# LSquarzoni/SNN_Event-based_Optical_Flow

Measured on AMD Instinct MI355X. Metric: events/sec (train step) LIFFireNet T=10 128x128, higher is better.
Workload: dtype fp32; 1 GPU; LIFFireNet train step: T=10 x 1000-event windows, 128x128, batch 8/GPU, base_num_channels 8, EventWarping + Adam; global_batch=8, parallelism=dp1, hip_graph=True, launch_order=wavefront

## Files before the change

### include/snnflow.h

```cpp
#ifndef SNNFLOW_H
#define SNNFLOW_H

#include <stdint.h>

#ifdef __cplusplus
extern "C" {
#endif

#define SNNFLOW_ABI_VERSION 41

#define SNNFLOW_E_ARG (-1)
#define SNNFLOW_E_CHANNELS (-2)

#define SNNFLOW_TILE_H 8
#define SNNFLOW_TILE_W 32

typedef struct snnflow_neuron {
    const float* bn_weight;
    const float* bn_bias;
    float* running_mean;
    float* running_var;
    int64_t* num_batches_tracked;
    const float* beta;
    const float* threshold;
    double momentum, eps;
    int bn_train;
    int zero_reset;
} snnflow_neuron;

int snnflow_prep_weights(const float* w, int c, int cin, float* wt_fwd, float* wt_bwd,
                         float* threshold, void* stream);

typedef struct snnflow_prep_desc {
    const float* w; int c, cin; float* wt_fwd; float* wt_bwd;
    float* threshold; int thr_n;
    uint16_t* frag_fwd; uint16_t* frag_bwd;
    double* zero; int64_t zero_n;
} snnflow_prep_desc;
int snnflow_frag_halfs(int c, int cin);
#define SNNFLOW_MAX_BATCH 16
int snnflow_prep_weights_batch(const snnflow_prep_desc* d, int n, void* stream);

#define SNNFLOW_ACC_SHARDS 32
#define SNNFLOW_ACC_STRIDE(n) ((((n) + 15) / 16) * 16)
#define SNNFLOW_ACC_LEN(n) (SNNFLOW_ACC_SHARDS * SNNFLOW_ACC_STRIDE(n))

typedef struct snnflow_conv_fwd_args {
    int B, H, W, cin, c;
    int lif_in;
    const float* x; int64_t xs_b, xs_c, xs_h, xs_w;
    const float* prev_y; const float* prev_mem;
    const double* prev_acc; float* prev_stats;
    snnflow_neuron prev; float* prev_state;
    const float* wt_ff;
    const float* wt_rec;
    const float* wt_ff_t; const float* wt_rec_t;
    const float* s_prev;
    float* y;
    double* acc;
    double* zero0; double* zero1; int zero_n;
    const uint16_t* wf_ff; const uint16_t* wf_rec;
    int state_spk_skip;
    uint8_t* prev_spk_bits; const uint8_t* s_prev_bits;
} snnflow_conv_fwd_args;
int snnflow_conv_fwd(const snnflow_conv_fwd_args* a, void* stream);
int snnflow_conv_blocks(int B, int H, int W);

typedef struct snnflow_lif_fwd_args {
    int B, H, W, c;
    const float* y; const float* mem;
    const double* acc;
    float* stats;
    snnflow_neuron n; float* state;
    const float* pred_w;
    const float* pred_b;
    float* flow;
    double* zero0; double* zero1; int zero_n;
    int state_spk_skip;
} snnflow_lif_fwd_args;
int snnflow_lif_fwd(const snnflow_lif_fwd_args* a, void* stream);

typedef struct snnflow_neuron_grad {
    float* bn_weight; float* bn_bias; float* beta; float* threshold;
} snnflow_neuron_grad;

#define SNNFLOW_SPK_BIT(c, ch) (((ch) % 4) * ((c) / 4) + (ch) / 4)

#define SNNFLOW_BWD_ACC(c) (5 * (c) + 2)

typedef struct snnflow_lif_bwd_args {
    int B, H, W, c;
    const float* y; const float* mem; const float* stats; snnflow_neuron n;
    const float* g_out;
    const float* g_state;
    const float* pred_w; const float* flow; const float* g_flow;
    int64_t gflow_sb, gflow_sc;
    float* g_cur;
    float* g_mem;
    double* acc;
    double* zero0; double* zero1; int zero_n;
    int mem_grad_in;
} snnflow_lif_bwd_args;
int snnflow_lif_bwd(const snnflow_lif_bwd_args* a, void* stream);

typedef struct snnflow_layer_bwd_args {
    int B, H, W, cin, c;
    const float* y; const float* stats; const float* g_cur;
    const double* acc_in;
    snnflow_neuron n;
    snnflow_neuron_grad ng;
    int has_pred; float* g_pred_w; float* g_pred_b;
    int accumulate;
    float* bnc_out;
    const float* wt_bwd_ff;
    const float* wt_bwd_rec;
    const float* wt_fwd_ff; const float* wt_fwd_rec;
    int lif_in;
    float* g_x; int64_t gxs_b, gxs_c, gxs_h, gxs_w;
    float* g_state_prev;
    int zero_mem_half;
    const float* prev_y; const float* prev_mem; const float* prev_stats; snnflow_neuron prev;
    const float* prev_g_state;
    float* prev_g_cur; float* prev_g_mem;
    double* acc_out;
    double* zero0; double* zero1; int zero_n;
    const uint16_t* wd_ff; const uint16_t* wd_rec;
    float* wslab_ff; float* wslab_rec; const float* s_prev; int wslab_accumulate;
    const float* x; int64_t xs_b, xs_c, xs_h, xs_w;
} snnflow_layer_bwd_args;
int snnflow_layer_bwd(const snnflow_layer_bwd_args* a, void* stream);

#define SNNFLOW_MAX_SLOT_TASKS 4
int snnflow_fwd_slot(const snnflow_conv_fwd_args* conv, int nconv, const snnflow_lif_fwd_args* lif,
                     void* stream);
int snnflow_bwd_slot(const snnflow_layer_bwd_args* layer, int nlayer, const snnflow_lif_bwd_args* lif,
                     void* stream);
int snnflow_slot_supported(int c, int cin0);
int snnflow_set_pipe(int fwd_tiles_per_block, int bwd_tiles_per_block);
int snnflow_get_pipe(int which);

#define SNNFLOW_MAX_LAYERS 8

typedef struct snnflow_wgrad_step {
    const float* g_cur;
    const float* y;
    const float* x; int64_t xs_b, xs_c, xs_h, xs_w;
    const float* s_prev;
    const float* stats;
    const float* bnc;
    const uint8_t* x_bits; const uint8_t* s_prev_bits;
} snnflow_wgrad_step;
#define SNNFLOW_MAX_WGRAD_STEPS 32
typedef struct snnflow_wgrad_args {
    int B, H, W, cin, c, nsteps, accumulate, rec;
    int exact_inputs;
    const float* bn_weight;
    float* slab_ff;
    float* slab_rec;
    snnflow_wgrad_step steps[SNNFLOW_MAX_WGRAD_STEPS];
} snnflow_wgrad_args;
int snnflow_wgrad(const snnflow_wgrad_args* a, void* stream);

typedef struct snnflow_convlif_params {
    const float* leak;
    const float* thresh;
    float act_width;
    int hard_reset;
} snnflow_convlif_params;

typedef struct snnflow_convlif_fwd_args {
    int B, H, W, cin, c;
    const float* x; int64_t xs_b, xs_c, xs_h, xs_w;
    const float* prev_state;
    const float* wt_ff;
    const float* wt_rec;
    snnflow_convlif_params p;
    const float* residual; int64_t rs_b, rs_c, rs_h, rs_w;
    float* out;
    float* state;
    float* current;
} snnflow_convlif_fwd_args;
int snnflow_convlif_fwd(const snnflow_convlif_fwd_args* a, void* stream);

typedef struct snnflow_convlif_bwd_args {
    int B, H, W, cin, c;
    const float* g_out; int64_t gs_b, gs_c, gs_h, gs_w;
    const float* g_state;
    const float* state;
    const float* prev_state;
    const float* current;
    const float* wt_bwd_ff;
    const float* wt_bwd_rec;
    snnflow_convlif_params p;
    float* g_x; int64_t gxs_b, gxs_c, gxs_h, gxs_w;
    float* g_prev;
    float* g_current;
    double* acc;
} snnflow_convlif_bwd_args;
int snnflow_convlif_bwd(const snnflow_convlif_bwd_args* a, void* stream);

int snnflow_convlif_param_grads(const double* acc, const float* leak, const float* thresh, int c, int accumulate,
                                float* g_leak, float* g_thresh, void* stream);

typedef struct snnflow_encode_args {
    int B, N, H, W;
    const float* ts; const float* ys; const float* xs; const float* ps;
    int64_t ev_stride, batch_stride;
    int num_bins, round_ts, accumulate;
    float* cnt; float* voxel; float* image; float* mask; float* pol_mask;
} snnflow_encode_args;
int snnflow_encode_events(const snnflow_encode_args* a, void* stream);

#define SNNFLOW_AUG_H 1
#define SNNFLOW_AUG_V 2
#define SNNFLOW_AUG_P 4
typedef struct snnflow_loader_args {
    int B, N;
    int H0, W0;
    int Ht, Wt;
    int num_bins, round_ts;
    int keep_gt_full_res;
    int hot_enabled, hot_max_px, hot_min_obvs;
    float hot_max_rate;
    float scale_y, scale_x;
    const float* xs; const float* ys; const float* ts; const float* ps;
    const int* counts;
    const int* flags;
    const float* gtflow_in;
    float* hot_events;
    int* hot_idx;
    float* event_cnt;
    float* event_voxel;
    float* event_mask;
    float* event_list;
    float* pol_mask;
    float* gtflow;
    float* scratch;
} snnflow_loader_args;
int snnflow_loader_prepare(const snnflow_loader_args* a, void* stream);
int64_t snnflow_loader_scratch_floats(int B, int N, int H0, int W0, int Ht, int Wt, int num_bins, int hot_enabled,
                                      int keep_gt_full_res);

typedef struct snnflow_slab_desc { const float* slab; float* out; int elems; } snnflow_slab_desc;
#define SNNFLOW_MAX_SLABS 16
int snnflow_slab_reduce(const snnflow_slab_desc* d, int n, int nblk, void* stream);

#define SNNFLOW_MAX_WINDOWS 64
typedef struct snnflow_iwe_loss_args {
    int B, M, T, H, W;
    int tf;
    const float* events[SNNFLOW_MAX_WINDOWS]; const float* pol[SNNFLOW_MAX_WINDOWS];
    const float* flows[SNNFLOW_MAX_WINDOWS]; const float* masks[SNNFLOW_MAX_WINDOWS];
    int32_t off[SNNFLOW_MAX_WINDOWS + 1];
    float flow_scaling, weight;
    int smoothing_mask, overwrite_intermediate, loss_scaling;
    float* images;
    double* acc;
    float* persample;
    float* smooth;
    float* loss;
} snnflow_iwe_loss_args;
int snnflow_iwe_loss_fwd(const snnflow_iwe_loss_args* a, void* stream);
int snnflow_iwe_loss_bwd(const snnflow_iwe_loss_args* a, const float* g_loss, float* g_flows, void* stream);
int snnflow_iwe_acc_doubles(int B, int H, int W, int tf);
int snnflow_device_errors(int clear);
int64_t snnflow_iwe_scratch_floats(int B, int M, int T, int tf, int H, int W);

int snnflow_iwe_corners(const float* events, const float* flow_ev, int B, int M, float tref,
                        int H, int W, float flow_scaling, int round_idx, int32_t* idx, float* w,
                        void* stream);
int snnflow_iwe_interpolate(const int32_t* idx, const float* w, const float* pol, int64_t pol_sb,
                            int B, int K, int H, int W, float* img, void* stream);
int snnflow_iwe_corners_bwd(const float* events, const float* flow_ev, int B, int M, float tref,
                            int H, int W, float flow_scaling, const float* g_w, float* g_flow_ev,
                            void* stream);
int snnflow_iwe_interpolate_bwd(const int32_t* idx, const float* pol, int64_t pol_sb, int B, int K,
                                int H, int W, const float* g_img, float* g_w, void* stream);

int snnflow_pol_iwe(const float* events, const float* flow, const float* pol, int64_t pol_stride, int nimg, int B,
                    int N, int H, int W, float tref, float flow_scaling, int round_idx, float* out, void* stream);

typedef struct snnflow_aee_args {
    int B, H, W;
    const float* flow;
    const float* gtflow;
    const float* event_mask;
    const float* dt_ratio;
    float flow_scaling;
    double* acc;
    float* aee; float* percent;
// ... 378 lines not shown
```

### snn_event-based_optical_flow_amd/csrc/lif_layers.hip

```cpp
#include <cmath>
#include <string>
#include <type_traits>

#include "snnflow_dev.h"
#include "snnflow_tile.h"

#ifndef SNNFLOW_PROBE
#define SNNFLOW_PROBE 0
#endif
#define PROBE_OFF(bit) ((SNNFLOW_PROBE & (bit)) != 0)

#ifndef SNNFLOW_SP32
#define SNNFLOW_SP32 2
#endif
#ifndef SNNFLOW_LATE_D_REC8
#define SNNFLOW_LATE_D_REC8 1
#endif
#ifndef SNNFLOW_LATE_D_FF8
#define SNNFLOW_LATE_D_FF8 1
#endif
#ifndef SNNFLOW_EARLY_G_REC8
#define SNNFLOW_EARLY_G_REC8 1
#endif
#ifndef SNNFLOW_L32_WAVES
// ... 1007 lines not shown
        float s = 0.0f;
        for (int k = qq; k < NT; k += Q) {
            const float4 v = lds[k];
            s += j == 0 ? v.x : (j == 1 ? v.y : (j == 2 ? v.z : v.w));
        }
        part[(int64_t)blockIdx.x * C + tid] = s;
    }
}

__global__ __launch_bounds__(64) void k_lif_theta_reduce(const float* __restrict__ part, int nblk, int c,
                                                      float* g_theta) {
    const int ch = threadIdx.x;
    if (ch >= c) return;
    double s = 0.0;
    for (int b = 0; b < nblk; ++b) s += (double)part[(int64_t)b * c + ch];
    g_theta[ch] -= (float)s;
}

struct BnBwdLds { float mean, inv, gm, k, w; };

__device__ inline float4 bn_bwd4(const float4& g, const float4& y, const BnBwdLds* bp) {
    const float gi[4] = {g.x, g.y, g.z, g.w}, yi[4] = {y.x, y.y, y.z, y.w};
    float o[4];
#pragma unroll
    for (int j = 0; j < 4; ++j) {
        const BnBwdLds c = bp[j];
        const float dx = (yi[j] - c.mean) * c.k;
        o[j] = (((gi[j] - c.gm) - dx) * c.inv) * c.w;
    }
    return make_float4(o[0], o[1], o[2], o[3]);
}

template <int CIN, int C, bool LIF_IN, bool REC, int SPLIT, bool BFG = false>
struct LayerBwdLds {
    static constexpr bool BF6 = kMfma<CIN, C> && (C == 8 || BFG);
    static constexpr bool WL = kWlds<CIN, C> && !BF6;
    static constexpr int FR = FragFloats<BF6 && C == 8, C, NT * SPLIT>::v;
    static constexpr int G = BF6 ? (3 * HN * C / 2 + 3) / 4 * 4 : HN * Pad<C>::v;
    static constexpr int WX = WL ? 9 * C * C : FR, WR = REC ? (WL ? 9 * C * C : FR) : 0;
    static constexpr int FLOATS = G + WX + WR;
    static_assert(!BF6 || G >= NT * Pad<CIN>::v, "output staging aliases the gradient tile");
};

typedef short s16x4w __attribute__((ext_vector_type(4)));
typedef __attribute__((address_space(3))) s16x4w lds_s16x4w;
__device__ inline bf16x8 tr8(const __bf16* r0, const __bf16* r1) {
    const s16x4w v0 = __builtin_amdgcn_ds_read_tr16_b64_v4i16((lds_s16x4w*)(r0));
    const s16x4w v1 = __builtin_amdgcn_ds_read_tr16_b64_v4i16((lds_s16x4w*)(r1));
    const short __attribute__((ext_vector_type(8))) v = __builtin_shufflevector(v0, v1, 0, 1, 2, 3, 4, 5, 6, 7);
    return __builtin_bit_cast(bf16x8, v);
}

constexpr int kWgfX = NT * 8 / 2, kWgfR = 8 * 8 * 9, kWgfP = 8 * 64;
constexpr int kWgfFloats = kWgfX + kWgfR + kWgfP;

template <bool REC>
__device__ void fused_wgrad_old(const snnflow_layer_bwd_args& a, const Grid& g, float (&wold)[4]) {
    const int tid = threadIdx.x;
    const bool acc_in = a.wslab_accumulate != 0;
    const bool has_s = REC && a.s_prev != nullptr && a.wslab_rec != nullptr;
    if (acc_in) {
        const float* sf = a.wslab_ff + (int64_t)g.bid * kWgfR;
        wold[0] = sf[tid];
        if (tid + 2 * NT < kWgfR) wold[1] = sf[tid + 2 * NT];
        if constexpr (REC) {
            if (has_s) {
                const float* sr = a.wslab_rec + (int64_t)g.bid * kWgfR;
                wold[2] = sr[tid];
                if (tid + 2 * NT < kWgfR) wold[3] = sr[tid + 2 * NT];
            }
        }
    }
}

template <bool REC>
__device__ void fused_wgrad_stage(const snnflow_layer_bwd_args& a, const float* G, float* wl_x, float* wl_r,
                                  const float (&xsp)[4], const float4& sp, int pt, int ci0) {
    constexpr int C = 8, PART = HN * C;
    const int tid = threadIdx.x;
    const bool has_s = REC && a.s_prev != nullptr && a.wslab_rec != nullptr;
    typedef __bf16 bf16x4 __attribute__((ext_vector_type(4)));
    __bf16* X = reinterpret_cast<__bf16*>(wl_x);
    __bf16* S = reinterpret_cast<__bf16*>(wl_r);
    const bf16x4 xs = {(__bf16)xsp[0], (__bf16)xsp[1], (__bf16)xsp[2], (__bf16)xsp[3]};
    __syncthreads();
    *reinterpret_cast<bf16x4*>(X + pt * C + ci0) = xs;
    if constexpr (REC) {
        if (has_s) *reinterpret_cast<bf16x4*>(S + pt * C + ci0) = bf16x4{(__bf16)sp.x, (__bf16)sp.y, (__bf16)sp.z, (__bf16)sp.w};
    }
    __syncthreads();

    const int lane = tid & 63, wv = __builtin_amdgcn_readfirstlane(tid >> 6);
    const int g4 = lane >> 4, qq = (lane & 15) >> 2, pp = lane & 3;
    const __bf16* G3 = reinterpret_cast<const __bf16*>(G);
    const int j0 = 8 * g4 + qq;
    f32x4 acc = {0.f, 0.f, 0.f, 0.f}, acc8 = acc, accr = acc, acc8r = acc;
    auto kstep = [&](int tap, int row, f32x4& d, f32x4& dr) {
        const int ky = tap / 3, kx = tap - 3 * ky;
        const int hp = (row + 2 - ky) * HWD + (j0 + 2 - kx);
        const __bf16* ga = G3 + hp * C + 4 * pp;
        const bf16x8 ah = tr8(ga, ga + 4 * C);
        const bf16x8 am = tr8(ga + PART, ga + PART + 4 * C);
        const bf16x8 al = tr8(ga + 2 * PART, ga + 2 * PART + 4 * C);
        const int q = row * TW + j0;
        const __bf16* xb = X + q * C + 4 * pp;
        const bf16x8 b = tr8(xb, xb + 4 * C);
        d = __builtin_amdgcn_mfma_f32_16x16x32_bf16(al, b, d, 0, 0, 0);
        d = __builtin_amdgcn_mfma_f32_16x16x32_bf16(am, b, d, 0, 0, 0);
        d = __builtin_amdgcn_mfma_f32_16x16x32_bf16(ah, b, d, 0, 0, 0);
        if constexpr (REC) {
            if (has_s) {
                const __bf16* sb = S + q * C + 4 * pp;
                const bf16x8 bs = tr8(sb, sb + 4 * C);
                dr = __builtin_amdgcn_mfma_f32_16x16x32_bf16(al, bs, dr, 0, 0, 0);
                dr = __builtin_amdgcn_mfma_f32_16x16x32_bf16(am, bs, dr, 0, 0, 0);
                dr = __builtin_amdgcn_mfma_f32_16x16x32_bf16(ah, bs, dr, 0, 0, 0);
            }
        }
    };
#pragma unroll 2
    for (int row = 0; row < TH; ++row) kstep(wv, row, acc, accr);
    kstep(8, wv, acc8, acc8r);
    const int ci = lane & 15;
    if (ci < C && g4 < 2) {
        float* R = wl_x + kWgfX;
        float* P8 = R + kWgfR;
#pragma unroll
        for (int j = 0; j < 4; ++j) {
            const int co = 4 * g4 + j;
            R[(co * C + ci) * 9 + wv] = acc[j];
            P8[wv * 64 + co * C + ci] = acc8[j];
        }
        if constexpr (REC) {
            if (has_s) {
                float* Rr = wl_r + kWgfX;
                float* P8r = Rr + kWgfR;
#pragma unroll
                for (int j = 0; j < 4; ++j) {
                    const int co = 4 * g4 + j;
                    Rr[(co * C + ci) * 9 + wv] = accr[j];
                    P8r[wv * 64 + co * C + ci] = acc8r[j];
                }
            }
        }
    }
}

__device__ inline int pk_slot(int q) { return SNNFLOW_SWZ ? q ^ (((q >> 3) & 1) << 2) : q; }
__device__ inline int pk_quad(int q, int quad) { return SNNFLOW_SWZ ? quad ^ ((q >> 3) & 1) : quad; }

constexpr int kPkRecOff = SNNFLOW_SWZ ? 16 : 0;

__device__ void fused_wgrad_stage_pk(const float* G, float* wl_x, float* wl_r, const float (&xsp)[4], const float4& sp,
                                     int pt, int ci0) {
    constexpr int C = 8, PART = HN * C, XS = 16;
    static_assert(FragFloats<true, 8, 2 * NT>::v >= NT * XS / 2 && FragFloats<true, 8, 2 * NT>::v >= 2 * (kWgfR + kWgfP) + kPkRecOff,
                  "packed x|s tile in wl_x, both result sets in wl_r");
    const int tid = threadIdx.x;
    typedef __bf16 bf16x4 __attribute__((ext_vector_type(4)));
    __bf16* X = reinterpret_cast<__bf16*>(wl_x);
    __syncthreads();
    const int ps = pk_slot(pt);
    *reinterpret_cast<bf16x4*>(X + ps * XS + ci0) = bf16x4{(__bf16)xsp[0], (__bf16)xsp[1], (__bf16)xsp[2], (__bf16)xsp[3]};
    *reinterpret_cast<bf16x4*>(X + ps * XS + C + ci0) = bf16x4{(__bf16)sp.x, (__bf16)sp.y, (__bf16)sp.z, (__bf16)sp.w};
    __syncthreads();

    const int lane = tid & 63, wv = __builtin_amdgcn_readfirstlane(tid >> 6);
    const int g4 = lane >> 4, qq = (lane & 15) >> 2, pp = lane & 3;
    const __bf16* G3 = reinterpret_cast<const __bf16*>(G);
    const int j0 = 8 * g4 + qq;
    f32x4 acc = {0.f, 0.f, 0.f, 0.f}, acc8 = acc;
    auto kstep = [&](int tap, int row, f32x4& d) {
        const int ky = tap / 3, kx = tap - 3 * ky;
        const int hp = (row + 2 - ky) * HWD + (j0 + 2 - kx);
        const __bf16* ga = G3 + hp * C + 4 * pp;
        const bf16x8 ah = tr8(ga, ga + 4 * C);
        const bf16x8 am = tr8(ga + PART, ga + PART + 4 * C);
        const bf16x8 al = tr8(ga + 2 * PART, ga + 2 * PART + 4 * C);
        const int q = row * TW + j0;
        const bf16x8 b = tr8(X + pk_slot(q) * XS + 4 * pp, X + pk_slot(q + 4) * XS + 4 * pp);
        d = __builtin_amdgcn_mfma_f32_16x16x32_bf16(al, b, d, 0, 0, 0);
        d = __builtin_amdgcn_mfma_f32_16x16x32_bf16(am, b, d, 0, 0, 0);
        d = __builtin_amdgcn_mfma_f32_16x16x32_bf16(ah, b, d, 0, 0, 0);
    };
#pragma unroll 2
    for (int row = 0; row < TH; ++row) kstep(wv, row, acc);
    kstep(8, wv, acc8);
    const int n = lane & 15;
    if (g4 < 2) {
        float* R = wl_r + (n < C ? 0 : kWgfR + kWgfP + kPkRecOff);
        float* P8 = R + kWgfR;
        const int ci = n & 7;
#pragma unroll
        for (int j = 0; j < 4; ++j) {
            const int co = 4 * g4 + j;
            R[(co * C + ci) * 9 + wv] = acc[j];
            P8[wv * 64 + co * C + ci] = acc8[j];
        }
    }
}

template <bool REC>
__device__ void fused_wgrad_store(const snnflow_layer_bwd_args& a, const Grid& g, const float* rx,
                                  const float* rr, const float (&wold)[4]) {
    const int tid = threadIdx.x;
    const bool acc_in = a.wslab_accumulate != 0;
    const bool has_s = REC && a.s_prev != nullptr && a.wslab_rec != nullptr;
    auto value = [&](const float* R, int e) {
        const int tap = e % 9;
        if (tap < 8) return R[e];
        const float* P8 = R + kWgfR;
        const int k = e / 9;
        float v = P8[k];
#pragma unroll
        for (int w = 1; w < 8; ++w) v += P8[w * 64 + k];
        return v;
    };
#pragma unroll
    for (int i = 0; i < 2; ++i) {
        const int e = tid + i * 2 * NT;
        if (e < kWgfR) {
            a.wslab_ff[(int64_t)g.bid * kWgfR + e] = acc_in ? wold[i] + value(rx, e) : value(rx, e);
            if constexpr (REC) {
                if (a.wslab_rec) {
                    if (has_s) a.wslab_rec[(int64_t)g.bid * kWgfR + e] = acc_in ? wold[2 + i] + value(rr, e) : value(rr, e);
                    else if (!acc_in) a.wslab_rec[(int64_t)g.bid * kWgfR + e] = 0.0f;
                }
            }
        }
    }
}

template <int CIN, int C, int NTH, int TOFF>
struct WAcc {
    static constexpr int VW = VecW<CIN>::v;
    static constexpr int Q = 9 * (C / 4) * (CIN / VW);
    static constexpr int GR0 = (Q >= NTH) ? 1 : NTH / Q;
    static constexpr int GR = GR0 > 16 ? 16 : GR0;
    static constexpr int NM = (GR > 1) ? 1 : (Q + NTH - 1) / NTH;
    static constexpr int SCRATCH = (GR > 1) ? GR * Q * 4 * VW : 1;
    float acc[NM][4][VW];
    __device__ void zero() {
#pragma unroll
        for (int m = 0; m < NM; ++m)
#pragma unroll
            for (int i = 0; i < 4; ++i)
#pragma unroll
                for (int j = 0; j < VW; ++j) acc[m][i][j] = 0.f;
    }
    template <bool HG = false>
    __device__ void step(const float* Gi, const float* X) {
        constexpr int PC = Pad<C>::v, PX = Pad<CIN>::v;
        const int tid = (int)threadIdx.x - TOFF;
        if (tid < 0 || tid >= NTH) return;
#pragma unroll
        for (int m = 0; m < NM; ++m) {
            const int q = (GR > 1) ? tid % Q : tid + m * NTH;
            const int g = (GR > 1) ? tid / Q : 0;
            if ((GR > 1) ? (g >= GR) : (q >= Q)) continue;
            const int kidx = q % 9, rest = q / 9, cob = rest % (C / 4), cib = rest / (C / 4);
            const int ky = kidx / 3, kx = kidx % 3;
#pragma unroll 4
            for (int p = g; p < NT; p += GR) {
                const int ty = p / TW, tx = p - ty * TW;
                const int gp = HG ? (ty + 1) * HWD + tx + 1 : p;
                const float4 gv4 = *reinterpret_cast<const float4*>(Gi + gp * PC + cob * 4);
                const float gv[4] = {gv4.x, gv4.y, gv4.z, gv4.w};
                const float* xp = X + ((ty + ky) * HWD + tx + kx) * PX + cib * VW;
                float xv[VW];
                if constexpr (VW == 4) {
                    const float4 v = *reinterpret_cast<const float4*>(xp);
                    xv[0] = v.x; xv[1] = v.y; xv[2] = v.z; xv[3] = v.w;
                } else if constexpr (VW == 2) {
                    const float2 v = *reinterpret_cast<const float2*>(xp);
                    xv[0] = v.x; xv[1] = v.y;
                } else {
                    xv[0] = xp[0];
                }
#pragma unroll
                for (int i = 0; i < 4; ++i)
#pragma unroll
                    for (int j = 0; j < VW; ++j) acc[m][i][j] = fmaf(gv[i], xv[j], acc[m][i][j]);
            }
        }
    }
    static __device__ int slab_index(int e) {
        const int qq = e / (4 * VW), ij = e - qq * 4 * VW, i = ij / VW, j = ij - i * VW;
        const int kk = qq % 9, rest = qq / 9, cb = rest % (C / 4), ib = rest / (C / 4);
        return ((cb * 4 + i) * CIN + ib * VW + j) * 9 + kk;
    }
    static constexpr int NOLD = (Q * 4 * VW + NTH - 1) / NTH;
    __device__ void flush_prefetched(float* __restrict__ slab, int accumulate, float* scratch, const float (&old)[NOLD]) {
        static_assert(GR > 1, "group-scratch form");
        const int tid = (int)threadIdx.x - TOFF;
        const bool mine = tid >= 0 && tid < NTH;
        const int q = tid % Q, g = tid / Q;
        if (mine && g < GR) {
#pragma unroll
            for (int i = 0; i < 4; ++i)
#pragma unroll
                for (int j = 0; j < VW; ++j) scratch[((g * Q + q) * 4 + i) * VW + j] = acc[0][i][j];
        }
        __syncthreads();
#pragma unroll
        for (int k = 0; k < NOLD; ++k) {
            const int e = tid + k * NTH;
            if (mine && e < Q * 4 * VW) {
                float sum = 0.f;
                for (int gg = 0; gg < GR; ++gg) sum += scratch[gg * Q * 4 * VW + e];
                slab[slab_index(e)] = accumulate ? old[k] + sum : sum;
            }
        }
    }
    __device__ void flush(float* __restrict__ slab, int accumulate, float* scratch) {
        const int tid = (int)threadIdx.x - TOFF;
        const bool mine = tid >= 0 && tid < NTH;
        if constexpr (GR > 1) {
            const int q = tid % Q, g = tid / Q;
            if (mine && g < GR) {
#pragma unroll
                for (int i = 0; i < 4; ++i)
#pragma unroll
                    for (int j = 0; j < VW; ++j) scratch[((g * Q + q) * 4 + i) * VW + j] = acc[0][i][j];
            }
            __syncthreads();
            for (int e = mine ? tid : Q * 4 * VW; e < Q * 4 * VW; e += NTH) {
                float sum = 0.f;
                for (int gg = 0; gg < GR; ++gg) sum += scratch[gg * Q * 4 * VW + e];
                const int qq = e / (4 * VW), ij = e - qq * 4 * VW, i = ij / VW, j = ij - i * VW;
                const int kk = qq % 9, rest = qq / 9, cb = rest % (C / 4), ib = rest / (C / 4);
                const int idx = ((cb * 4 + i) * CIN + ib * VW + j) * 9 + kk;
                slab[idx] = accumulate ? slab[idx] + sum : sum;
            }
            __syncthreads();
        } else {
#pragma unroll
            for (int m = 0; m < NM; ++m) {
                const int q = tid + m * NTH;
                if (!mine || q >= Q) continue;
                const int kk = q % 9, rest = q / 9, cb = rest % (C / 4), ib = rest / (C / 4);
#pragma unroll
                for (int i = 0; i < 4; ++i)
#pragma unroll
                    for (int j = 0; j < VW; ++j) {
                        const int idx = ((cb * 4 + i) * CIN + ib * VW + j) * 9 + kk;
                        slab[idx] = accumulate ? slab[idx] + acc[m][i][j] : acc[m][i][j];
                    }
            }
        }
    }
};

template <int CIN, int C, bool LIF_IN, bool REC, int SPLIT, bool BFG = false, bool WGF = false, bool HWG = false>
__device__ void layer_bwd_body(const snnflow_layer_bwd_args& a, const Grid g, float* lds) {
    using LB = LayerBwdLds<CIN, C, LIF_IN, REC, SPLIT, BFG>;
    static_assert(!HWG || (!LIF_IN && !REC && !kMfma<CIN, C>), "fused head weight gradient: feed-forward head tasks");
    static_assert(!WGF || (LIF_IN && C == 8 && CIN == 8 && SPLIT == 2 && LB::BF6 && LB::FR >= kWgfFloats),
                  "fused weight gradients: C = 8 LIF-fed layers with LDS weight fragments");
    constexpr int NTB = NT * SPLIT;
    constexpr int CI = CIN / SPLIT, CR = C / SPLIT;
    static_assert(CI * SPLIT == CIN && CR * SPLIT == C, "channel split");
    static_assert(!LIF_IN || CI % 4 == 0, "LIF backward group: multiple of 4 channels");
    constexpr int PC = Pad<C>::v;
    constexpr bool PF = Prefetch<C, NTB>::on;
    constexpr int NVP = LIF_IN ? 3 * CI : 1;
    constexpr int QI = CI / 4 > 0 ? CI / 4 : 1;
    float* G = lds;
    [[maybe_unused]] float* wl_x = lds + LB::G;
    [[maybe_unused]] float* wl_r = wl_x + LB::WX;
    __shared__ BnBwdLds bnp[C];
    __shared__ LifCoef pcoef[LIF_IN ? CIN : 1];
    __shared__ float pmean[LIF_IN ? CIN : 1];

    const int tid = threadIdx.x, pt = tid % NT, ty = pt / TW, tx = pt - ty * TW;
    const int part = thread_part(), ci0 = part * CI, cr0 = part * CR;
    const int H = a.H, W = a.W;
    const Tile tl = block_tile(H, W, g);
    const double N = (double)a.B * H * W;
    const float nf = (float)N;
    const int h = tl.h0 + ty, w = tl.w0 + tx;
    const bool in = (h < H) && (w < W);
    const int64_t pix = ((int64_t)tl.b * H + h) * W + w;
    const float4 z4 = make_float4(0.f, 0.f, 0.f, 0.f);
    [[maybe_unused]] constexpr bool TR = LIF_IN && CIN == C && SNNFLOW_TRACE_LAYER;
    [[maybe_unused]] constexpr int TK = REC ? 3 : 2;
    TRACE_AT(TR, TK, 0);

    constexpr bool EARLY_G = C <= 16 && !(REC && C == 8 && !SNNFLOW_EARLY_G_REC8);
    constexpr int NSUM = SNNFLOW_BWD_ACC(C), NBN = (C <= 16 || SNNFLOW_BWD_GATHER32) ? 2 * C : NSUM;
    const bool lead = g.bid == 0;
    constexpr int NL = NSUM - NBN > 0 ? NSUM - NBN : 1;
    AccGather<NBN> gat;
    AccGather<NL> gat_l;
    if constexpr (EARLY_G) {
        acc_gather_load<NBN>(a.acc_in, NSUM, gat);
        if (NBN < NSUM && lead) acc_gather_load<NL>(a.acc_in + NBN, NSUM, gat_l);
    }
    float st_mean = 0.f, st_inv = 0.f, gamma = 0.f;
    if (tid < C) {
        st_mean = a.stats[tid];
        st_inv = a.stats[C + tid];
        gamma = a.n.bn_weight[tid];
    }
    const NeuronGradRegs ngr =
        load_neuron_grad(a.n, a.stats, C, a.ng, a.accumulate, a.has_pred, a.g_pred_w, a.g_pred_b, g.bid == 0);
    float praw[6] = {0.f, 0.f, 0.f, 0.f, 0.f, 0.f};
    if constexpr (LIF_IN) {
        const int c = tid < CIN ? tid : 0;
        praw[0] = a.prev_stats[c];
        praw[1] = a.prev_stats[CIN + c];
        praw[2] = a.prev.bn_weight[c];
        praw[3] = a.prev.bn_bias[c];
        praw[4] = a.prev.beta[c];
        praw[5] = a.prev.threshold[c];
    }

    constexpr bool WL = LB::WL, BF6 = LB::BF6, FLDS = BF6 && C == 8;
    WStage<WL ? 9 * C * C : 1, NTB> sw_x, sw_r;
    FragStage<FLDS ? C : 8, FLDS ? CIN : 8, FLDS ? NTB : 64> fs_x, fs_r;
    static_assert(!BF6 || PF, "bf16 gradient tile: register-prefetched halo");
    if constexpr (WL) {
        if (a.wt_bwd_ff) sw_x.load(a.wt_fwd_ff);
        if constexpr (REC) {
            if (a.g_state_prev) sw_r.load(a.wt_fwd_rec);
        }
    }
    constexpr bool PKC = FLDS && REC && CIN == 8 && C == 8;
    [[maybe_unused]] const bool pkr = PKC && a.wt_bwd_ff != nullptr && a.g_state_prev != nullptr;
    if constexpr (FLDS) {
        if constexpr (PKC) {
            if (pkr) fs_x.load2(a.wt_fwd_ff, a.wt_fwd_rec);
            else if (a.wt_bwd_ff) fs_x.load(a.wt_fwd_ff);
            if (!pkr && a.g_state_prev) fs_r.load(a.wt_fwd_rec);
        } else {
            if (a.wt_bwd_ff) fs_x.load(a.wt_fwd_ff);
            if constexpr (REC) {
                if (a.g_state_prev) fs_r.load(a.wt_fwd_rec);
            }
        }
    }
    using HAF = WAcc<HWG ? CIN : 4, HWG ? C : 4, NTB, 0>;
    constexpr int HXR = HWG ? (HN * CIN + NTB - 1) / NTB : 1;
    [[maybe_unused]] const bool hwg = HWG && a.wslab_ff != nullptr && a.x != nullptr;
    [[maybe_unused]] float hx[HXR], hold[HAF::NOLD];
    if constexpr (HWG) {
        if (hwg) {
            const float* xb = a.x + (int64_t)tl.b * a.xs_b;
#pragma unroll
            for (int i = 0; i < HXR; ++i) {
                const int e = tid + i * NTB;
                const int ci = e / HN, p = e - ci * HN;
                const int r = p / HWD, cc = p - r * HWD;
                const int hh = tl.h0 + r - 1, ww = tl.w0 + cc - 1;
                hx[i] = (e < HN * CIN && in_image(hh, ww, H, W)) ? xb[ci * a.xs_c + hh * a.xs_h + ww * a.xs_w] : 0.0f;
            }
            const float* srow = a.wslab_ff + (int64_t)g.bid * (C * CIN * 9);
#pragma unroll
            for (int k = 0; k < HAF::NOLD; ++k) {
                const int e = tid + k * NTB;
                hold[k] = (a.wslab_accumulate && e < C * CIN * 9) ? srow[HAF::slab_index(e < C * CIN * 9 ? e : 0)] : 0.0f;
            }
        }
    }
    float4 rg[PF ? Halo4<C, NTB>::R : 1], ry[PF ? Halo4<C, NTB>::R : 1];
    float4 dy[LIF_IN ? QI : 1], dm[LIF_IN ? QI : 1], dg[LIF_IN ? QI : 1];
    if constexpr (PF) {
        halo_load<C, NTB>(a.g_cur, tl, H, W, rg);
        halo_load<C, NTB>(a.y, tl, H, W, ry);
    }
    constexpr bool LATE_D = C >= 32 || (C == 8 && (REC ? SNNFLOW_LATE_D_REC8 : SNNFLOW_LATE_D_FF8));
    [[maybe_unused]] float wold[4] = {0.f, 0.f, 0.f, 0.f};
    [[maybe_unused]] float4 wsp = z4;
    [[maybe_unused]] const bool wgf = WGF && a.wslab_ff != nullptr;
    auto load_prev = [&]() {
        if constexpr (LIF_IN) {
            constexpr int Q4 = CIN / 4;
            const int64_t plane4 = (int64_t)a.B * H * W * Q4;
            const float4* py4 = reinterpret_cast<const float4*>(a.prev_y);
            const float4* pm4 = reinterpret_cast<const float4*>(a.prev_mem);
            const float4* pg4 = reinterpret_cast<const float4*>(a.prev_g_state);
            const int64_t pc = ((int64_t)tl.b * H + (h < H ? h : H - 1)) * W + (w < W ? w : W - 1);
            const int64_t base = pc * Q4 + ci0 / 4;
#pragma unroll
            for (int q = 0; q < QI; ++q) {
                dy[q] = py4[base + q];
                dm[q] = ld4_or_zero(pm4, py4, base + q);
                dg[q] = ld4_or_zero(pg4 ? pg4 + plane4 : nullptr, py4, base + q);
            }
        }
        if constexpr (WGF && REC) {
            if (wgf && a.s_prev && a.wslab_rec && in) wsp = reinterpret_cast<const float4*>(a.s_prev)[pix * 2 + ci0 / 4];
        }
    };
    if constexpr (!LATE_D) load_prev();


    __shared__ double sums[NSUM];
    if constexpr (EARLY_G) {
        acc_gather_reduce<NBN>(gat, sums);
        if (NBN < NSUM && lead) acc_gather_reduce<NL>(gat_l, sums + NBN);
    } else if constexpr (SNNFLOW_BWD_GATHER32) {
        double* red = reinterpret_cast<double*>(lds);
        acc_gather_pool<NBN, NTB>(a.acc_in, NSUM, sums, red);
        if (NBN < NSUM && lead) acc_gather_pool<NL, NTB>(a.acc_in + NBN, NSUM, sums + NBN, red);
    } else {
        acc_gather<NBN>(a.acc_in, NSUM, sums);
        if (NBN < NSUM && lead) acc_gather<NL>(a.acc_in + NBN, NSUM, sums + NBN);
    }
    neuron_grads(ngr, sums, C, a.ng, a.has_pred, a.g_pred_w, a.g_pred_b, lead);
    if (tid < C) {
        const float mean = st_mean, inv = st_inv;
        BnBwdLds c;
        c.mean = mean;
        c.inv = inv;
        c.w = gamma;
        if (a.n.bn_train) {
            c.k = (float)sums[C + tid] * inv * inv / nf;
            c.gm = (float)(sums[tid] / N);
        } else {
            c.k = 0.0f;
            c.gm = 0.0f;
        }
        bnp[tid] = c;
        if (g.bid == 0 && a.bnc_out) {
            a.bnc_out[tid] = c.gm;
            a.bnc_out[C + tid] = c.k;
        }
    }
    if constexpr (LIF_IN) {
        if (tid < CIN) {
            LifCoef pk;
            pk.alpha = praw[1] * praw[2];
            pk.shift = praw[3] - praw[0] * pk.alpha;
            pk.beta = fminf(fmaxf(praw[4], 0.0f), 1.0f);
            pk.theta = praw[5];
            pcoef[tid] = pk;
            pmean[tid] = praw[0];
        }
    }
    __syncthreads();
    TRACE_AT(TR, TK, 1);
    zero_consumed(a.zero0, a.zero1, a.zero_n, g);

    if constexpr (PF) {
        constexpr int Q = C / 4;
        static_assert(NTB % Q == 0, "constant channel quad per thread");
        const int qt = tid % Q;
        const BnBwdLds kb[4] = {bnp[4 * qt], bnp[4 * qt + 1], bnp[4 * qt + 2], bnp[4 * qt + 3]};
#pragma unroll
        for (int i = 0; i < Halo4<C, NTB>::R; ++i) {
            const int e = tid + i * NTB;
            if (e < Halo4<C, NTB>::E) {
                const int p = e / Q;
                const int r = p / HWD, cc = p - r * HWD;
                const bool img = in_image(tl.h0 + r - 1, tl.w0 + cc - 1, H, W);
                const float4 gv = img ? bn_bwd4(rg[i], ry[i], kb) : z4;
                if constexpr (BF6) split3_store4(reinterpret_cast<__bf16*>(G) + p * C + 4 * qt, HN * C, gv);
                else *reinterpret_cast<float4*>(G + p * PC + 4 * qt) = gv;
            }
        }
    } else {
        constexpr int Q = C / 4;
        for (int e = tid; e < Halo4<C>::E; e += NTB) {
            const int p = e / Q, q = e - p * Q;
            const int64_t k = halo_idx4<C>(e, tl, H, W);
            float4 out = z4;
            if (k >= 0)
                out = bn_bwd4(reinterpret_cast<const float4*>(a.g_cur)[k], reinterpret_cast<const float4*>(a.y)[k],
                              bnp + 4 * q);
            *reinterpret_cast<float4*>(G + p * PC + 4 * q) = out;
        }
    }
    if constexpr (WL) {
        if (a.wt_bwd_ff) sw_x.store(wl_x);
        if constexpr (REC) {
            if (a.g_state_prev) sw_r.store(wl_r);
        }
    }
    if constexpr (FLDS) {
        if (a.wt_bwd_ff) fs_x.store(reinterpret_cast<__bf16*>(wl_x));
        if constexpr (REC) {
            if (a.g_state_prev && !pkr) fs_r.store(reinterpret_cast<__bf16*>(wl_r));
        }
    }
    __syncthreads();
    TRACE_AT(TR, TK, 2);

    float gx[CI];
#pragma unroll
    for (int ci = 0; ci < CI; ++ci) gx[ci] = 0.0f;
    if constexpr (kMfma<CIN, C>) {
        constexpr int NW = NTB / 64;
        const bool do_x = a.wt_bwd_ff != nullptr;
        const bool do_r = REC && a.g_state_prev != nullptr;
        constexpr int NG = (C >= 32 && BF6) ? 2 : 1;
        MfmaAcc<C, CIN, NW, NG> ax;
        MfmaAcc<C, C, NW, NG> arr;
        const __bf16* g3 = reinterpret_cast<const __bf16*>(G);
        if (do_x) {
            ax.zero();
            if constexpr (FLDS) {
                if (!PROBE_OFF(1)) mfma_dgrad_bf6<C, CIN, NW>(g3, reinterpret_cast<const __bf16*>(wl_x), ax);
            } else if constexpr (BF6) {
                if (!PROBE_OFF(1)) mfma_dgrad_bf6g<C, CIN, NW, NG>(g3, reinterpret_cast<const __bf16*>(a.wd_ff), ax);
            } else {
                if (!PROBE_OFF(1)) mfma_conv3x3<C, CIN, true, NW, NG>(G, WL ? wl_x : a.wt_fwd_ff, ax);
            }
        }
        if constexpr (REC) {
            if (do_r && !pkr) {
                arr.zero();
                if constexpr (FLDS) {
                    if (!PROBE_OFF(1)) mfma_dgrad_bf6<C, C, NW>(g3, reinterpret_cast<const __bf16*>(wl_r), arr);
                } else if constexpr (BF6) {
                    if (!PROBE_OFF(1)) mfma_dgrad_bf6g<C, C, NW, NG>(g3, reinterpret_cast<const __bf16*>(a.wd_rec), arr);
                } else {
                    if (!PROBE_OFF(1)) mfma_conv3x3<C, C, true, NW, NG>(G, WL ? wl_r : a.wt_fwd_rec, arr);
                }
            }
        }
        if constexpr (LATE_D) load_prev();
        __syncthreads();
        float* const dgo = (WGF && wgf) ? wl_x : G;
        if constexpr (PKC) {
            if (pkr) {
                const int lane = tid & 63, n = lane & 15, g4 = lane >> 4;
                const int wv = __builtin_amdgcn_readfirstlane(tid >> 6);
                float* out = (n < 8 ? wl_x : wl_r + kPkRecOff) + (n & 3);
#pragma unroll
                for (int mt = 0; mt < MfmaAcc<C, CIN, NW, NG>::MT; ++mt) {
                    const int T = MfmaAcc<C, CIN, NW, NG>::mt0(wv) + mt, row = T >> 1, c0 = (T & 1) * 16;
#pragma unroll
                    for (int r = 0; r < 4; ++r) {
                        const int q = row * TW + c0 + g4 * 4 + r;
                        out[q * 8 + 4 * pk_quad(q, (n >> 2) & 1)] = ax.v[mt][0][r];
                    }
                }
                __syncthreads();
                const float4 gv4 = *reinterpret_cast<const float4*>(wl_x + pt * 8 + 4 * pk_quad(pt, ci0 >> 2));
                gx[0] = gv4.x; gx[1] = gv4.y; gx[2] = gv4.z; gx[3] = gv4.w;
                if (in) {
                    const int64_t plane = (int64_t)a.B * H * W * C;
                    float* gsp = a.g_state_prev + pix * C + cr0;
                    if (a.zero_mem_half) *reinterpret_cast<float4*>(gsp) = z4;
                    *reinterpret_cast<float4*>(gsp + plane) =
                        *reinterpret_cast<const float4*>(wl_r + kPkRecOff + pt * 8 + 4 * pk_quad(pt, cr0 >> 2));
                }
            }
        }
        if (do_x && !pkr) {
            mfma_store<false>(ax, ax, dgo);
            __syncthreads();
            const float* gl = dgo + pt * Pad<CIN>::v + ci0;
#pragma unroll
            for (int ci = 0; ci < CI; ++ci) gx[ci] = gl[ci];
        }
        if constexpr (REC) {
            if (do_r && !pkr) {
                __syncthreads();
                mfma_store<false>(arr, arr, dgo);
                __syncthreads();
                if (in) {
                    const float* rl = dgo + pt * PC + cr0;
                    const int64_t plane = (int64_t)a.B * H * W * C;
                    float* gsp = a.g_state_prev + pix * C + cr0;
#pragma unroll
                    for (int c = 0; c < CR; c += 4) {
                        if (a.zero_mem_half) *reinterpret_cast<float4*>(gsp + c) = z4;
                        *reinterpret_cast<float4*>(gsp + plane + c) = *reinterpret_cast<const float4*>(rl + c);
                    }
                }
            }
        }
    } else {
        if (!PROBE_OFF(1) && a.wt_bwd_ff) dgrad_acc<C, CIN, CI>(G, a.wt_bwd_ff, ty, tx, ci0, gx);
        if constexpr (REC) {
            if (a.g_state_prev) {
                float gr[CR];
#pragma unroll
                for (int c = 0; c < CR; ++c) gr[c] = 0.0f;
                if (!PROBE_OFF(1)) dgrad_acc<C, C, CR>(G, a.wt_bwd_rec, ty, tx, cr0, gr);
                pin(gr);
                if (in) {
                    const int64_t plane = (int64_t)a.B * H * W * C;
                    float* gsp = a.g_state_prev + pix * C + cr0;
#pragma unroll
                    for (int c = 0; c < CR; c += 4) {
                        if (a.zero_mem_half) *reinterpret_cast<float4*>(gsp + c) = z4;
                        *reinterpret_cast<float4*>(gsp + plane + c) = make_float4(gr[c], gr[c + 1], gr[c + 2], gr[c + 3]);
                    }
                }
            }
        }
    }

    TRACE_AT(TR, TK, 3);
    if constexpr (LIF_IN) {
        float vd[NVP];
#pragma unroll
        for (int j = 0; j < NVP; ++j) vd[j] = 0.0f;
        [[maybe_unused]] float xsp[4] = {0.f, 0.f, 0.f, 0.f};
        if constexpr (WGF) {
            if (wgf) fused_wgrad_old<REC>(a, g, wold);
        }
        if (in && !PROBE_OFF(8)) {
            const bool zr = a.prev.zero_reset != 0;
            float4* gc4 = reinterpret_cast<float4*>(a.prev_g_cur) + pix * (CIN / 4) + ci0 / 4;
            float4* gm4 = a.prev_g_mem ? reinterpret_cast<float4*>(a.prev_g_mem) + pix * (CIN / 4) + ci0 / 4 : nullptr;
#pragma unroll
            for (int q = 0; q < QI; ++q) {
                const float yi[4] = {dy[q].x, dy[q].y, dy[q].z, dy[q].w};
                const float mi[4] = {dm[q].x, dm[q].y, dm[q].z, dm[q].w};
                const float gi[4] = {dg[q].x, dg[q].y, dg[q].z, dg[q].w};
                float go[4], gmo[4];
#pragma unroll
                for (int j = 0; j < 4; ++j) {
                    const int cl = 4 * q + j, ci = ci0 + cl;
                    const float gs = gx[cl] + gi[j];
                    const LifOut o = lif_step(yi[j], mi[j], pcoef[ci], zr);
                    const float gv = atan_sg(o.v - pcoef[ci].theta) * gs;
                    if constexpr (WGF) xsp[cl & 3] = o.s;
                    go[j] = gv;
                    gmo[j] = mem_grad(gv, mi[j], pcoef[ci], zr);
                    vd[cl] = gv;
                    vd[CI + cl] = (yi[j] - pmean[ci]) * gv;
                    vd[2 * CI + cl] = gv * o.mprime;
                }
                gc4[q] = make_float4(go[0], go[1], go[2], go[3]);
                if (gm4) gm4[q] = make_float4(gmo[0], gmo[1], gmo[2], gmo[3]);
            }
        }
        TRACE_AT(TR, TK, 4);
        double* acc = acc_shard(a.acc_out, SNNFLOW_BWD_ACC(CIN), g.bid);
        if (!PROBE_OFF(4))
            block_atomic_sum_parts<NVP, SPLIT>(vd, [acc](int pp, int j) {
                const int k = j / CI, jj = j - k * CI;
                return acc + k * CIN + pp * CI + jj;
            });
        TRACE_AT(TR, TK, 5);
        if constexpr (WGF) {
            if (wgf) {
                if (REC && a.s_prev != nullptr && a.wslab_rec != nullptr) {
                    fused_wgrad_stage_pk(G, wl_x, wl_r, xsp, wsp, pt, ci0);
                    __syncthreads();
                    fused_wgrad_store<REC>(a, g, wl_r, wl_r + kWgfR + kWgfP + kPkRecOff, wold);
                } else {
                    fused_wgrad_stage<REC>(a, G, wl_x, wl_r, xsp, wsp, pt, ci0);
                    __syncthreads();
                    fused_wgrad_store<REC>(a, g, wl_x + kWgfX, wl_r + kWgfX, wold);
                }
            }
        }
        TRACE_AT(TR, TK, 6);
    } else {
        if (a.g_x && a.wt_bwd_ff && in) {
            float* gb = a.g_x + (int64_t)tl.b * a.gxs_b + h * a.gxs_h + w * a.gxs_w;
#pragma unroll
            for (int ci = 0; ci < CI; ++ci) gb[(ci0 + ci) * a.gxs_c] = gx[ci];
        }
        if constexpr (HWG) {
            if (hwg) {
                float* X = lds + LB::G;
#pragma unroll
                for (int i = 0; i < HXR; ++i) {
                    const int e = tid + i * NTB;
                    if (e < HN * CIN) {
                        const int ci = e / HN, p = e - ci * HN;
                        X[p * Pad<CIN>::v + ci] = hx[i];
                    }
                }
                HAF af;
                af.zero();
                __syncthreads();
                af.template step<true>(G, X);
                __syncthreads();
                af.flush_prefetched(a.wslab_ff + (int64_t)g.bid * (C * CIN * 9), a.wslab_accumulate, lds, hold);
            }
        }
    }
}

template <int CIN, int C, bool LIF_IN, bool REC, int SPLIT, bool BFG = false>
__global__ __launch_bounds__(NT * SPLIT, (C == 32 && LIF_IN && SPLIT == 2) ? SNNFLOW_L32_WAVES : 1)
void k_layer_bwd(snnflow_layer_bwd_args a) {
    __shared__ __attribute__((aligned(16))) float pool[LayerBwdLds<CIN, C, LIF_IN, REC, SPLIT, BFG>::FLOATS];
    layer_bwd_body<CIN, C, LIF_IN, REC, SPLIT, BFG>(a, hw_grid(), pool);
}

typedef const __attribute__((address_space(4))) snnflow_wgrad_args* cwgrad_ptr;

template <int CIN, int C, bool REC, int NW>
struct WgradMfma {
    static constexpr int MTc = (C + 15) / 16, NTF = (CIN + 15) / 16, NTR = (C + 15) / 16;
    static constexpr int NFF = 9 * MTc * NTF, NREC = REC ? 9 * MTc * NTR : 0, NTOT = NFF + NREC;
    static constexpr int J = (NTOT + NW - 1) / NW;
    static_assert(C % 8 == 0 && CIN % 8 == 0, "MFMA wgrad: 8-channel multiples (C = 8 pads the 16-wide tiles)");
    f32x4 acc[J];
    int off[J], mt[J], nt[J], tap[J];
    bool rec[J], live[J];
    __device__ void init() {
        const int wv = __builtin_amdgcn_readfirstlane((int)threadIdx.x >> 6);
#pragma unroll
        for (int j = 0; j < J; ++j) {
            acc[j] = f32x4{0.f, 0.f, 0.f, 0.f};
            const int i = wv + NW * j;
            live[j] = i < NTOT;
            rec[j] = i >= NFF;
            const int ii = rec[j] ? i - NFF : i, ntx = rec[j] ? NTR : NTF;
            tap[j] = live[j] ? ii / (MTc * ntx) : 0;
            const int rem = ii - tap[j] * (MTc * ntx);
            mt[j] = live[j] ? rem / ntx : 0;
            nt[j] = live[j] ? rem - mt[j] * ntx : 0;
            off[j] = (tap[j] / 3) * HWD + (tap[j] % 3);
        }
    }
    __device__ void step(const float* Gi, const float* X, const float* S, bool has_s) {
        constexpr int PC = Pad<C>::v, PX = Pad<CIN>::v;
        const int lane = threadIdx.x & 63, m = lane & 15, g = lane >> 4;
#pragma unroll 8
        for (int s = 0; s < NT / 4; ++s) {
            const int p = 4 * s + g, ty = p / TW, tx = p - ty * TW;
            const int hb = ty * HWD + tx;
            float a[MTc];
#pragma unroll
            for (int q = 0; q < MTc; ++q) a[q] = (q * 16 + m < C) ? Gi[p * PC + q * 16 + m] : 0.0f;
#pragma unroll
            for (int j = 0; j < J; ++j) {
                if (!live[j] || (rec[j] && !has_s)) continue;
                float av = a[0];
#pragma unroll
                for (int q = 1; q < MTc; ++q)
                    if (mt[j] == q) av = a[q];
                const int n = nt[j] * 16 + m;
                float b = 0.0f;
                if (rec[j]) {
                    if (n < C) b = S[(hb + off[j]) * PC + n];
                } else if (n < CIN) {
                    b = X[(hb + off[j]) * PX + n];
                }
                acc[j] = __builtin_amdgcn_mfma_f32_16x16x4f32(av, b, acc[j], 0, 0, 0);
            }
        }
    }
    __device__ void flush(float* __restrict__ slab_ff, float* __restrict__ slab_rec, int accumulate) {
        const int lane = threadIdx.x & 63, m = lane & 15, g = lane >> 4;
#pragma unroll
        for (int j = 0; j < J; ++j) {
            if (!live[j] || (rec[j] && !slab_rec)) continue;
            const int ci = nt[j] * 16 + m, cin = rec[j] ? C : CIN;
            if (ci >= cin) continue;
            float* base = rec[j] ? slab_rec : slab_ff;
#pragma unroll
            for (int r = 0; r < 4; ++r) {
                const int co = mt[j] * 16 + g * 4 + r;
                if (co >= C) continue;
                float* d = base + ((int64_t)co * cin + ci) * 9 + tap[j];
                *d = accumulate ? *d + acc[j][r] : acc[j][r];
            }
        }
    }
};

template <int CH, int NTH>
struct Own4 {
    static constexpr int Q = CH / 4, E = NT * Q, R = (E + NTH - 1) / NTH;
};

template <int CIN, int C, bool REC, int SPLIT>
__global__ __launch_bounds__(NT * SPLIT) void k_wgrad(snnflow_wgrad_args) {
    constexpr int NTB = NT * SPLIT;
    constexpr int PC = Pad<C>::v, PI_ = Pad<CIN>::v;
    constexpr bool XV = CIN % 4 == 0;
    constexpr bool HALVES = REC && SPLIT == 2;
    using AF = WAcc<CIN, C, HALVES ? NT : NTB, 0>;
    using AR = WAcc<C, C, HALVES ? NT : NTB, HALVES ? NT : 0>;
    constexpr bool MF = C >= 16 && CIN % 16 == 0;
    using O = Own4<C, NTB>;
    constexpr int RX = XV ? Halo4<CIN, NTB>::R : 1, RS = REC ? Halo4<C, NTB>::R : 1;
    constexpr int SCR = MF ? 4 : ((REC && AR::SCRATCH > AF::SCRATCH) ? AR::SCRATCH : AF::SCRATCH);
    __shared__ __attribute__((aligned(16))) float Gi[NT * PC];
    __shared__ __attribute__((aligned(16))) float X[HN * PI_];
    __shared__ __attribute__((aligned(16))) float S[REC ? HN * PC : 4];
    __shared__ __attribute__((aligned(16))) float scratch[SCR];
    __shared__ BnBwdLds coef[SNNFLOW_MAX_WGRAD_STEPS][C];

    const cwgrad_ptr ap = (cwgrad_ptr)__builtin_amdgcn_kernarg_segment_ptr();
    const int tid = threadIdx.x;
    const int H = ap->H, W = ap->W, nsteps = ap->nsteps;
    const Tile tl = block_tile(H, W);
    const float4 z4 = make_float4(0.f, 0.f, 0.f, 0.f);

    for (int e = tid; e < nsteps * C; e += NTB) {
        const int t = e / C, c = e - t * C;
        const float* st = ap->steps[t].stats;
        const float* bc = ap->steps[t].bnc;
        BnBwdLds k = {0.f, 1.f, 0.f, 0.f, 1.f};
        if (st) {
            k.mean = st[c];
// ... 862 lines not shown
    const float c = coef_s;
    for (int64_t j = threadIdx.x; j < n; j += 8 * CLIP_NT) {
        float v[8];
#pragma unroll
        for (int k = 0; k < 8; ++k) v[k] = j + k * CLIP_NT < n ? g[j + k * CLIP_NT] : 0.0f;
#pragma unroll
        for (int k = 0; k < 8; ++k)
            if (j + k * CLIP_NT < n) g[j + k * CLIP_NT] = v[k] * c;
    }
}

constexpr int CLIP_PER = 8, CLIP_SLICE = CLIP_PER * CLIP_NT;
static_assert(CLIP_SLICE == SNNFLOW_CLIP_ADAM_ONE_BLOCK, "one-block size");

__device__ inline double clip_sq_slice(const float* g, int64_t n, int64_t i0, int64_t i1) {
    double s = 0.0;
    for (int64_t i = i0 + threadIdx.x; i < i1; i += (int64_t)CLIP_SLICE) {
        float v[CLIP_PER];
#pragma unroll
        for (int k = 0; k < CLIP_PER; ++k) v[k] = i + k * CLIP_NT < i1 ? g[i + k * CLIP_NT] : 0.0f;
#pragma unroll
        for (int k = 0; k < CLIP_PER; ++k) s += (double)v[k] * (double)v[k];
    }
    return s;
}

__device__ inline double clip_block_sum(double s, double* part) {
#pragma unroll
    for (int off = 32; off > 0; off >>= 1) s += __shfl_xor(s, off, 64);
    if ((threadIdx.x & 63) == 0) part[threadIdx.x >> 6] = s;
    __syncthreads();
    double t = 0.0;
    if (threadIdx.x == 0)
        for (int w = 0; w < CLIP_NT / 64; ++w) t += part[w];
    return t;
}

__global__ __launch_bounds__(CLIP_NT) void k_clip_adam_norm(snnflow_clip_adam_args a) {
    __shared__ double part[CLIP_NT / 64];
    const int64_t i0 = (int64_t)blockIdx.x * CLIP_SLICE, i1 = i0 + CLIP_SLICE < a.n ? i0 + CLIP_SLICE : a.n;
    const double t = clip_block_sum(a.max_norm > 0.0f ? clip_sq_slice(a.grad, a.n, i0, i1) : 0.0, part);
    if (threadIdx.x == 0) {
        a.scratch[blockIdx.x] = t;
        if (blockIdx.x == 0) a.step[0] = a.step[0] + 1.0f;
    }
}

__global__ __launch_bounds__(CLIP_NT) void k_clip_adam(snnflow_clip_adam_args a, int nparts) {
    __shared__ double part[CLIP_NT / 64];
    __shared__ float coef_s;
    __shared__ snnflow_adam_tensor tab[SNNFLOW_ADAM_MAX_TENSORS];
    if (threadIdx.x < a.ntensors) tab[threadIdx.x] = a.t[threadIdx.x];
    const bool clip = a.max_norm > 0.0f;
    const float st_in = a.step[0];
    __syncthreads();
    const int64_t lo_i = nparts ? (int64_t)blockIdx.x * CLIP_SLICE : 0;
    const int64_t hi_i = lo_i + CLIP_SLICE < a.n ? lo_i + CLIP_SLICE : a.n;
    float gv[CLIP_PER], pv[CLIP_PER], mv[CLIP_PER], vv[CLIP_PER];
    float *pp[CLIP_PER], *mp[CLIP_PER], *vp[CLIP_PER];
#pragma unroll
    for (int u = 0; u < CLIP_PER; ++u) {
        const int64_t i = lo_i + threadIdx.x + (int64_t)u * CLIP_NT;
        gv[u] = i < hi_i ? a.grad[i] : 0.0f;
    }
#pragma unroll
    for (int u = 0; u < CLIP_PER; ++u) {
        const int64_t i = lo_i + threadIdx.x + (int64_t)u * CLIP_NT;
        pp[u] = nullptr;
        if (i >= hi_i) continue;
        int lo = 0, hi = a.ntensors - 1;
        while (lo < hi) {
            const int mid = (lo + hi + 1) >> 1;
            if (tab[mid].offset <= i) lo = mid;
            else hi = mid - 1;
        }
        const int64_t j = i - tab[lo].offset;
        if (j < 0 || j >= tab[lo].numel) continue;
        pp[u] = tab[lo].param + j;
        mp[u] = a.exp_avg + tab[lo].state_offset + j;
        vp[u] = a.exp_avg_sq + tab[lo].state_offset + j;
        pv[u] = *pp[u];
        mv[u] = *mp[u];
        vv[u] = *vp[u];
    }
    double tot = 0.0;
    if (nparts == 0) {
        double sq = 0.0;
        if (clip) {
#pragma unroll
            for (int u = 0; u < CLIP_PER; ++u) sq += (double)gv[u] * (double)gv[u];
        }
        tot = clip_block_sum(sq, part);
    } else if (threadIdx.x == 0 && clip) {
        for (int j = 0; j < nparts; ++j) tot += a.scratch[j];
    }
    const float st = nparts == 0 ? st_in + 1.0f : st_in;
    if (threadIdx.x == 0) {
        if (clip) {
            const float total = (float)sqrt(tot);
            const float cc = a.max_norm / (total + a.clip_eps);
            coef_s = cc < 1.0f ? cc : 1.0f;
            if (a.total_out && blockIdx.x == 0) a.total_out[0] = total;
        } else {
            coef_s = 1.0f;
        }
        if (nparts == 0) a.step[0] = st;
    }
    const double step = (double)st;
    const double bc1 = 1.0 - pow(a.beta1, step), bc2 = 1.0 - pow(a.beta2, step);
    __syncthreads();
    const float c = coef_s;
    const float neg_step_size = (float)(-(a.lr / bc1));
    const float bc2_sqrt = (float)sqrt(bc2);
    const float w1 = (float)(1.0 - a.beta1), b2 = (float)a.beta2, w2 = (float)(1.0 - a.beta2);
    const float eps = (float)a.eps, wd = (float)a.weight_decay;
#pragma unroll
    for (int u = 0; u < CLIP_PER; ++u) {
        if (!pp[u]) continue;
        float g = gv[u];
        if (clip) {
            g = g * c;
            a.grad[lo_i + threadIdx.x + (int64_t)u * CLIP_NT] = g;
        }
        float p = pv[u];
        if (wd != 0.0f) g = g + wd * p;
        const float m = mv[u] + w1 * (g - mv[u]);
        const float v = vv[u] * b2 + w2 * g * g;
        const float denom = sqrtf(v) / bc2_sqrt + eps;
        p = p + neg_step_size * (m / denom);
        *mp[u] = m;
        *vp[u] = v;
        *pp[u] = p;
    }
}

__global__ void k_lif_export(const float* __restrict__ x, const float* __restrict__ mem, const float* __restrict__ beta,
                             const float* __restrict__ thr, int64_t total, int C, int HW, float* spk, float* mout) {
    for (int64_t i = (int64_t)blockIdx.x * blockDim.x + threadIdx.x; i < total; i += (int64_t)gridDim.x * blockDim.x) {
        const int c = (int)((i / HW) % C);
        const float m = beta[c] * mem[i] + x[i];
        const bool s = m >= thr[c];
        spk[i] = s ? 1.0f : 0.0f;
        mout[i] = s ? 0.0f : m;
    }
}

constexpr int kSlotTasks = SNNFLOW_MAX_SLOT_TASKS;

enum SlotKind : int {
    SK_HEAD1, SK_HEAD2, SK_HEAD4, SK_HEAD5,
    SK_PLAIN, SK_PLAIN_REC,
    SK_LIF, SK_LIF_REC,
    SK_TOP, SK_TOP_PRED,
    SK_LIF_P, SK_LIF_REC_P
};

struct FwdSlotParams {
    snnflow_conv_fwd_args conv[kSlotTasks];
    snnflow_lif_fwd_args lif;
    int kind[kSlotTasks], blk0[kSlotTasks], nblk[kSlotTasks];
    int ntask;
};
struct BwdSlotParams {
    snnflow_layer_bwd_args layer[kSlotTasks];
    snnflow_lif_bwd_args lif;
    int kind[kSlotTasks], blk0[kSlotTasks], nblk[kSlotTasks];
    int ntask;
};

constexpr int cmax(int a, int b) { return a > b ? a : b; }

template <int C>
constexpr bool kSlotAllKinds = C == 8;

constexpr int kFragC8 = 3 * 3 * 256;
constexpr int kPipeRaw = 2 * HN * 16, kPipeSpk = HN * 8 * 2, kPipeFrag = kFragC8 * 2;
template <bool REC>
struct PipeFwdLds {
    static constexpr int RAWY = 0, RAWM = kPipeRaw, SPK = 2 * kPipeRaw, RSPK = SPK + kPipeSpk;
    static constexpr int FF = RSPK + (REC ? kPipeSpk : 0), FR = FF + kPipeFrag;
    static constexpr int BYTES = FR + (REC ? kPipeFrag : 0);
    static constexpr int FLOATS = BYTES / 4;
};

template <int C>
struct SlotLds {
    static constexpr int FWD_ALL = cmax(cmax(ConvFwdLds<1, C, false, false, 2>::FLOATS, ConvFwdLds<5, C, false, false, 2>::FLOATS),
                                        cmax(ConvFwdLds<C, C, false, false, 2>::FLOATS, ConvFwdLds<C, C, false, true, 2>::FLOATS));
    static constexpr int FWD_P = C == 8 ? PipeFwdLds<true>::FLOATS : 0;
    static constexpr int FWD = cmax(cmax(cmax(kSlotAllKinds<C> ? FWD_ALL : 0, kLifQFwdLds<C>), FWD_P),
                                    cmax(cmax(ConvFwdLds<2, C, false, false, 2>::FLOATS, ConvFwdLds<4, C, false, false, 2>::FLOATS),
                                         cmax(ConvFwdLds<C, C, true, false, 2>::FLOATS, ConvFwdLds<C, C, true, true, 2>::FLOATS)));
    static constexpr bool BFG = C >= 16;
    static constexpr int BWD_ALL = cmax(LayerBwdLds<C, C, false, false, 2>::FLOATS, LayerBwdLds<C, C, false, true, 2>::FLOATS);
    static constexpr int BWD = cmax(cmax(cmax(kSlotAllKinds<C> ? BWD_ALL : 0, kLifQBwdLds<C, true>),
                                         cmax(LayerBwdLds<2, C, false, false, 2>::FLOATS, LayerBwdLds<4, C, false, false, 2>::FLOATS)),
                                    cmax(LayerBwdLds<C, C, true, false, 2, BFG>::FLOATS,
                                         LayerBwdLds<C, C, true, true, 2, BFG>::FLOATS));
};

template <typename T>
__device__ inline T kernarg_copy(const __attribute__((address_space(4))) T* p) {
    static_assert(sizeof(T) % 4 == 0, "dword-sized struct");
    T r;
    const __attribute__((address_space(4))) int* src = (const __attribute__((address_space(4))) int*)p;
    int* dst = reinterpret_cast<int*>(&r);
#pragma unroll
    for (int i = 0; i < (int)(sizeof(T) / 4); ++i) dst[i] = src[i];
    return r;
}

template <typename T>
__device__ inline T* as_global_ptr(T* p) {
    __attribute__((address_space(1))) T* g;
    asm("" : "=s"(g) : "0"(p));
    return (T*)g;
}
#define SNN_G(x) (x) = as_global_ptr(x)

__device__ inline void globalize(snnflow_neuron& n) {
    SNN_G(n.bn_weight); SNN_G(n.bn_bias); SNN_G(n.running_mean); SNN_G(n.running_var);
    SNN_G(n.num_batches_tracked); SNN_G(n.beta); SNN_G(n.threshold);
}
__device__ inline void globalize(snnflow_neuron_grad& n) {
    SNN_G(n.bn_weight); SNN_G(n.bn_bias); SNN_G(n.beta); SNN_G(n.threshold);
}
__device__ inline void globalize(snnflow_conv_fwd_args& a) {
    SNN_G(a.x); SNN_G(a.prev_y); SNN_G(a.prev_mem); SNN_G(a.prev_acc); SNN_G(a.prev_stats);
    globalize(a.prev);
    SNN_G(a.prev_state); SNN_G(a.wt_ff); SNN_G(a.wt_rec); SNN_G(a.wt_ff_t); SNN_G(a.wt_rec_t); SNN_G(a.s_prev);
    SNN_G(a.prev_spk_bits); SNN_G(a.s_prev_bits);
    SNN_G(a.y); SNN_G(a.acc); SNN_G(a.zero0); SNN_G(a.zero1); SNN_G(a.wf_ff); SNN_G(a.wf_rec);
}
__device__ inline void globalize(snnflow_lif_fwd_args& a) {
    SNN_G(a.y); SNN_G(a.mem); SNN_G(a.acc); SNN_G(a.stats);
    globalize(a.n);
    SNN_G(a.state); SNN_G(a.pred_w); SNN_G(a.pred_b); SNN_G(a.flow); SNN_G(a.zero0); SNN_G(a.zero1);
}
__device__ inline void globalize(snnflow_lif_bwd_args& a) {
    SNN_G(a.y); SNN_G(a.mem); SNN_G(a.stats);
    globalize(a.n);
    SNN_G(a.g_out); SNN_G(a.g_state); SNN_G(a.pred_w); SNN_G(a.flow); SNN_G(a.g_flow); SNN_G(a.g_cur);
    SNN_G(a.g_mem); SNN_G(a.acc); SNN_G(a.zero0); SNN_G(a.zero1);
}
__device__ inline void globalize(snnflow_layer_bwd_args& a) {
    SNN_G(a.y); SNN_G(a.stats); SNN_G(a.g_cur); SNN_G(a.acc_in);
    globalize(a.n);
    globalize(a.ng);
    SNN_G(a.g_pred_w); SNN_G(a.g_pred_b); SNN_G(a.bnc_out); SNN_G(a.wt_bwd_ff); SNN_G(a.wt_bwd_rec);
    SNN_G(a.wt_fwd_ff); SNN_G(a.wt_fwd_rec); SNN_G(a.g_x); SNN_G(a.g_state_prev); SNN_G(a.prev_y);
    SNN_G(a.prev_mem); SNN_G(a.prev_stats);
    globalize(a.prev);
    SNN_G(a.prev_g_state); SNN_G(a.prev_g_cur); SNN_G(a.prev_g_mem); SNN_G(a.acc_out); SNN_G(a.zero0);
    SNN_G(a.zero1); SNN_G(a.wd_ff); SNN_G(a.wd_rec); SNN_G(a.wslab_ff); SNN_G(a.wslab_rec); SNN_G(a.s_prev);
    SNN_G(a.x);
}
__device__ inline void globalize(snnflow_eval_fwd_args& a) {
    SNN_G(a.x); SNN_G(a.s_in); SNN_G(a.mem_prev); SNN_G(a.s_prev); SNN_G(a.wt_ff); SNN_G(a.wt_rec);
    SNN_G(a.wt_ff_t); SNN_G(a.wt_rec_t);
    globalize(a.n);
    SNN_G(a.state); SNN_G(a.pred_w); SNN_G(a.pred_b); SNN_G(a.flow);
}
#undef SNN_G

template <typename T>
__device__ inline T task_args(const __attribute__((address_space(4))) T* p) {
    T r = kernarg_copy(p);
    globalize(r);
    return r;
}

template <typename P>
__device__ inline int slot_task(const __attribute__((address_space(4))) P* pp, Grid& g) {
    const int bid = blockIdx.x, nt = pp->ntask;
    int k = 0;
#pragma unroll
    for (int i = 1; i < kSlotTasks; ++i)
        if (i < nt && bid >= pp->blk0[i]) k = i;
    g.bid = bid - pp->blk0[k];
    g.nb = pp->nblk[k];
    return k;
}

typedef __attribute__((address_space(3))) void lds_void;

template <int N>
__device__ inline void vm_wait() {
    static_assert(N >= 0 && N < 64, "vmcnt");
    __builtin_amdgcn_s_waitcnt((N & 15) | ((N >> 4) << 14) | (7 << 4) | (15 << 8));
}

__device__ inline int opaque_int(int v) {
    asm volatile("" : "+v"(v));
    return v;
}

struct FragC8 {
    float r[2];
    __device__ inline void load(const float* __restrict__ wB) {
#pragma unroll
        for (int i = 0; i < 2; ++i) {
            const int e = (int)threadIdx.x + i * 2 * NT;
            const int j = e & 7, co = (e >> 3) & 7, g = (e >> 6) & 3, ch = e >> 8, tap = 4 * ch + g;
            r[i] = (e < 768 && tap < 9) ? wB[(tap * 8 + co) * 8 + j] : 0.0f;
        }
    }
    __device__ inline void store(__bf16* f) const {
#pragma unroll
        for (int i = 0; i < 2; ++i) {
            const int e = (int)threadIdx.x + i * 2 * NT;
            if (e < 768) {
                const float w = r[i];
                const __bf16 h = (__bf16)w;
                const float r1 = w - (float)h;
                const __bf16 md = (__bf16)r1;
                __bf16* d = f + (e >> 8) * 3 * 256 + (e & 255);
                d[0] = h;
                d[256] = md;
                d[512] = (__bf16)(r1 - (float)md);
            }
        }
    }
};

__host__ __device__ inline int pipe_tiles(const Grid& g, int ntiles) {
    return g.bid < ntiles ? (ntiles - 1 - g.bid) / g.nb + 1 : 0;
}

__device__ inline int* pipe_slot() {
    __shared__ int slot[4];
    return slot;
}

template <bool REC>
__device__ void fwd_lif8_pipe(const snnflow_conv_fwd_args& a, const Grid g, float* pool) {
    constexpr int C = 8, NTB = 2 * NT, R = Halo4<C, NTB>::R;
    using L = PipeFwdLds<REC>;
    char* const lds = reinterpret_cast<char*>(pool);
    __shared__ LifCoef coef[C];
    __shared__ double sums[2 * C];
    const int tid = threadIdx.x, lane = tid & 63;
    const int wv = __builtin_amdgcn_readfirstlane(tid >> 6);
    const int H = a.H, W = a.W, ntiles = a.B * tiles_per_image(H, W);
    int* const slot = pipe_slot();
    int v_cur = g.bid < ntiles ? g.bid : -1;
    if (v_cur < 0) return;
    const bool lead = g.bid == 0;
    const bool has_mem = a.prev_mem != nullptr;
    const bool has_rec = REC && a.s_prev != nullptr;
    TRACE_AT(true, REC ? 1 : 0, 0);

    AccGather<2 * C> gat;
    if (a.prev.bn_train) acc_gather_load<2 * C>(a.prev_acc, 2 * C, gat);
    const NeuronRegs nr = load_neuron(a.prev, C, lead);
    FragC8 fz_ff, fz_rec;
    fz_ff.load(a.wt_ff_t);
    if (has_rec) fz_rec.load(a.wt_rec_t);

    const uint32_t nbytes = (uint32_t)a.B * H * W * C * 4;
    const __amdgpu_buffer_rsrc_t rs_y = __builtin_amdgcn_make_buffer_rsrc(const_cast<float*>(a.prev_y), (short)0, (int)nbytes, 0x00020000);
    const __amdgpu_buffer_rsrc_t rs_m =
        __builtin_amdgcn_make_buffer_rsrc(const_cast<float*>(has_mem ? a.prev_mem : a.prev_y), (short)0, (int)nbytes, 0x00020000);
    auto issue = [&](const Tile& t, int lane) {
        const int base = ((t.b * H + t.h0 - 1) * W + (t.w0 - 1)) * (C * 4);
#pragma unroll
        for (int j = 0; j < 3; ++j) {
            const int k = wv + 8 * j;
            if (k >= 22) break;
            const bool mem = k >= 11;
            if (mem && !has_mem) continue;
            const int kk = mem ? k - 11 : k, ee = kk * 64 + lane, p = ee >> 1, r = p / HWD, cc = p - r * HWD;
            const bool ok = in_image(t.h0 + r - 1, t.w0 + cc - 1, H, W);
            const uint32_t off = ok ? (uint32_t)(base + (r * W + cc) * (C * 4) + (ee & 1) * 16) : 0x80000000u;
            if (ee < 2 * HN)
                __builtin_amdgcn_raw_ptr_buffer_load_lds(mem ? rs_m : rs_y, (lds_void*)(lds + (mem ? L::RAWM : L::RAWY) + kk * 1024),
                                                         16, off, 0, 0, 0);
        }
    };
    float4 rs[R];
    auto load_sprev = [&](const Tile& t, int tid) {
        const float4* base = reinterpret_cast<const float4*>(a.s_prev) + (((int64_t)t.b * H + (t.h0 - 1)) * W + (t.w0 - 1)) * 2;
#pragma unroll
        for (int i = 0; i < R; ++i) {
            const int e = tid + i * NTB, p = e >> 1, r = p / HWD, cc = p - r * HWD;
            const bool ok = e < 2 * HN && in_image(t.h0 + r - 1, t.w0 + cc - 1, H, W);
            rs[i] = ok ? base[(r * W + cc) * 2 + (e & 1)] : make_float4(0.f, 0.f, 0.f, 0.f);
        }
    };
    Tile tl = block_tile(H, W, Grid{v_cur, ntiles});
    issue(tl, lane);
    if (has_rec) load_sprev(tl, tid);
    if (a.prev.bn_train) acc_gather_reduce<2 * C>(gat, sums);
    TRACE_AT(true, REC ? 1 : 0, 1);
    lif_prologue(a.prev, nr, sums, C, (double)a.B * H * W, a.prev_stats, coef, nullptr, lead);
    TRACE_AT(true, REC ? 1 : 0, 2);
    fz_ff.store(reinterpret_cast<__bf16*>(lds + L::FF));
    if (has_rec) fz_rec.store(reinterpret_cast<__bf16*>(lds + L::FR));
    zero_consumed(a.zero0, a.zero1, a.zero_n, g);
    if (tid == 0) slot[2] = 0;

    const bool zr = a.prev.zero_reset != 0, spk_skip = a.state_spk_skip != 0;
    const int64_t plane4 = (int64_t)a.B * H * W * 2;
    float4* st4 = reinterpret_cast<float4*>(a.prev_state);
    float bs[4] = {0.f, 0.f, 0.f, 0.f}, bq[4] = {0.f, 0.f, 0.f, 0.f};
    const __bf16* spk = reinterpret_cast<const __bf16*>(lds + L::SPK);
    const __bf16* rspk = reinterpret_cast<const __bf16*>(lds + L::RSPK);
    TRACE_AT(true, REC ? 1 : 0, 3);

    for ([[maybe_unused]] int k = 0; v_cur >= 0; ++k) {
        vm_wait<0>();
        __syncthreads();
        TRACE_AT(k < 2, REC ? 1 : 0, 4 + 3 * k);
        const int tid = opaque_int(threadIdx.x), lane = tid & 63, jj = lane & 15, gg = lane >> 4, qt = tid & 1;
        const LifCoef kc[4] = {coef[4 * qt], coef[4 * qt + 1], coef[4 * qt + 2], coef[4 * qt + 3]};
        bool ok = true;
#pragma unroll
        for (int i = 0; i < R; ++i) {
            const int e = tid + i * NTB;
            if (e < 2 * HN) {
                const int p = e >> 1, r = p / HWD, cc = p - r * HWD;
                const int h = tl.h0 + r - 1, w = tl.w0 + cc - 1;
                const float4 yv = *reinterpret_cast<const float4*>(lds + L::RAWY + e * 16);
                const float4 mv = has_mem ? *reinterpret_cast<const float4*>(lds + L::RAWM + e * 16) : make_float4(0.f, 0.f, 0.f, 0.f);
                float4 sv = make_float4(0.f, 0.f, 0.f, 0.f);
                if (in_image(h, w, H, W)) {
                    const Lif4 o = zr ? lif_step4(yv, mv, kc, true) : lif_step4(yv, mv, kc, false);
                    sv = o.s;
                    if (r >= 1 && r <= TH && cc >= 1 && cc <= TW) {
                        const int64_t q = (((int64_t)tl.b * H + h) * W + w) * 2 + qt;
                        st_state4(st4, q, o.mout);
// ... 283 lines not shown
    const int64_t HWp = (int64_t)H * W;

    for (int k = 0; v_cur >= 0; ++k) {
        vm_wait<0>();
        __syncthreads();
        const int tid = opaque_int(threadIdx.x), lane = tid & 63, jj = lane & 15, gg = lane >> 4, qt = tid & 1;
        bool ok = true;
#pragma unroll
        for (int i = 0; i < R; ++i) {
            const int e = tid + i * NTB;
            if (e < 2 * HN) {
                const int p = e >> 1;
                const float4 sv = *reinterpret_cast<const float4*>(lds + L::RAW + e * 16);
                typedef __bf16 bf16x4 __attribute__((ext_vector_type(4)));
                *reinterpret_cast<bf16x4*>(const_cast<__bf16*>(spk) + p * 8 + 4 * qt) =
                    bf16x4{(__bf16)sv.x, (__bf16)sv.y, (__bf16)sv.z, (__bf16)sv.w};
                if (has_rec) {
                    const float4 s = rs[i];
                    ok = ok && exact_bf16(s.x) && exact_bf16(s.y) && exact_bf16(s.z) && exact_bf16(s.w);
                    *reinterpret_cast<bf16x4*>(const_cast<__bf16*>(rspk) + p * 8 + 4 * qt) =
                        bf16x4{(__bf16)s.x, (__bf16)s.y, (__bf16)s.z, (__bf16)s.w};
                }
            }
        }
        if (has_rec && __builtin_amdgcn_ballot_w64(!ok) != 0 && lane == 0) bad[k & 1] = 1;
        if (threadIdx.x == 0) bad[(k + 1) & 1] = 0;
        __syncthreads();
        const bool rec_bf = has_rec && bad[k & 1] == 0;
        const int v_nxt = v_cur + g.nb < ntiles ? v_cur + g.nb : -1;
        const Tile cur = tl;
        if (v_nxt >= 0) {
            tl = block_tile(H, W, Grid{v_nxt, ntiles});
            issue(tl, lane);
            if (has_rec) load_sprev(tl, tid);
        }
        const int qd = (lane >> 4) & 1, h = cur.h0 + wv, w = cur.w0 + (lane >> 5) * 16 + jj;
        const bool in = h < H && w < W;
        const int64_t pix = ((int64_t)cur.b * H + (in ? h : 0)) * W + (in ? w : 0);
        const float4 mv = (has_mem && in) ? mem4[pix * 2 + qd] : make_float4(0.f, 0.f, 0.f, 0.f);

        const bf16x8* fff = reinterpret_cast<const bf16x8*>(lds + L::FF) + gg * 8 + (jj & 7);
        const bf16x8* ffr = reinterpret_cast<const bf16x8*>(lds + L::FR) + gg * 8 + (jj & 7);
        f32x4 af[2] = {{0.f, 0.f, 0.f, 0.f}, {0.f, 0.f, 0.f, 0.f}}, ar[2] = {{0.f, 0.f, 0.f, 0.f}, {0.f, 0.f, 0.f, 0.f}};
#pragma unroll
        for (int ch = 0; ch < 3; ++ch) {
            const int tap = 4 * ch + gg, ky = tap / 3, kx = tap - 3 * ky;
            const bf16x8 fh = fff[ch * 96], fm = fff[ch * 96 + 32], fl = fff[ch * 96 + 64];
#pragma unroll
            for (int mt = 0; mt < 2; ++mt) {
                const int off = ((wv + ky) * HWD + mt * 16 + jj + kx) * 8;
                bf16x8 b = {};
                if (tap < 9) b = *reinterpret_cast<const bf16x8*>(spk + off);
                af[mt] = __builtin_amdgcn_mfma_f32_16x16x32_bf16(fl, b, af[mt], 0, 0, 0);
                af[mt] = __builtin_amdgcn_mfma_f32_16x16x32_bf16(fm, b, af[mt], 0, 0, 0);
                af[mt] = __builtin_amdgcn_mfma_f32_16x16x32_bf16(fh, b, af[mt], 0, 0, 0);
            }
            if (rec_bf) {
                const bf16x8 rh = ffr[ch * 96], rm = ffr[ch * 96 + 32], rl = ffr[ch * 96 + 64];
#pragma unroll
                for (int mt = 0; mt < 2; ++mt) {
                    const int off = ((wv + ky) * HWD + mt * 16 + jj + kx) * 8;
                    bf16x8 b = {};
                    if (tap < 9) b = *reinterpret_cast<const bf16x8*>(rspk + off);
                    ar[mt] = __builtin_amdgcn_mfma_f32_16x16x32_bf16(rl, b, ar[mt], 0, 0, 0);
                    ar[mt] = __builtin_amdgcn_mfma_f32_16x16x32_bf16(rm, b, ar[mt], 0, 0, 0);
                    ar[mt] = __builtin_amdgcn_mfma_f32_16x16x32_bf16(rh, b, ar[mt], 0, 0, 0);
                }
            }
        }
        f32x4 yv;
#pragma unroll
        for (int r = 0; r < 4; ++r) {
            const float y0 = rec_bf ? af[0][r] + ar[0][r] : af[0][r];
            const float y1 = rec_bf ? af[1][r] + ar[1][r] : af[1][r];
            const auto sw = __builtin_amdgcn_permlane32_swap(__builtin_bit_cast(unsigned, y0), __builtin_bit_cast(unsigned, y1),
                                                             false, false);
            yv[r] = __builtin_bit_cast(float, sw[0]);
        }
        if (has_rec && !rec_bf && in) {
            const float* wr = a.wt_rec;
#pragma unroll 1
            for (int tp = 0; tp < 9; ++tp) {
                const int hh = h + tp / 3 - 1, ww = w + tp % 3 - 1;
                if (!in_image(hh, ww, H, W)) continue;
                const float* sp = a.s_prev + (((int64_t)cur.b * H + hh) * W + ww) * C;
                for (int ci = 0; ci < C; ++ci) {
                    const float s = sp[ci];
#pragma unroll
                    for (int r = 0; r < 4; ++r) yv[r] = fmaf(wr[(tp * C + ci) * C + 4 * qd + r], s, yv[r]);
                }
            }
        }
        const LifCoef kc[4] = {coef[4 * qd], coef[4 * qd + 1], coef[4 * qd + 2], coef[4 * qd + 3]};
        const Lif4 o = zr ? lif_step4(make_float4(yv[0], yv[1], yv[2], yv[3]), mv, kc, true)
                          : lif_step4(make_float4(yv[0], yv[1], yv[2], yv[3]), mv, kc, false);
        if (in) {
            st_state4(st4, pix * 2 + qd, o.mout);
            st_state4(st4, plane4 + pix * 2 + qd, o.s);
        }
        if (pred) {
            const float p0 = __shfl_xor(o.s.x, 16, 64), p1 = __shfl_xor(o.s.y, 16, 64);
            const float p2 = __shfl_xor(o.s.z, 16, 64), p3 = __shfl_xor(o.s.w, 16, 64);
            const float s8[8] = {qd ? p0 : o.s.x, qd ? p1 : o.s.y, qd ? p2 : o.s.z, qd ? p3 : o.s.w,
                                 qd ? o.s.x : p0, qd ? o.s.y : p1, qd ? o.s.z : p2, qd ? o.s.w : p3};
            if (in) {
                const float* pw = a.pred_w + qd * C;
                float acc = 0.0f;
#pragma unroll
                for (int c = 0; c < C; ++c) acc = fmaf(pw[c], s8[c], acc);
                a.flow[((int64_t)cur.b * 2 + qd) * HWp + (int64_t)h * W + w] = tanhf(acc + a.pred_b[qd]);
            }
        }
        v_cur = v_nxt;
    }
}

__global__ __launch_bounds__(NT * 2, 6) void k_eval_slot(EvalSlotParams) {
    typedef const __attribute__((address_space(4))) EvalSlotParams* cptr;
    const cptr pp = (cptr)__builtin_amdgcn_kernarg_segment_ptr();
    const int bid = blockIdx.x, nt = pp->ntask;
    int k = 0;
#pragma unroll
    for (int i = 1; i < kEvalTasks; ++i)
        if (i < nt && bid >= pp->blk0[i]) k = i;
    Grid g;
    g.bid = bid - pp->blk0[k];
    g.nb = pp->nblk[k];
    if (g.bid >= g.nb) return;
    __shared__ __attribute__((aligned(16))) float pool[kEvalLdsFloats];
    const snnflow_eval_fwd_args a = task_args(&pp->t[k]);
    switch (pp->kind[k]) {
        case EK_HEAD2: eval_head_body<2>(a, g, pool); break;
        case EK_HEAD4: eval_head_body<4>(a, g, pool); break;
        case EK_FF: eval8_pipe<false>(a, g, pool); break;
        case EK_REC: eval8_pipe<true>(a, g, pool); break;
        default: break;
    }
}

#ifndef SNNFLOW_BWD_SLOT_WAVES
#define SNNFLOW_BWD_SLOT_WAVES 6
#endif
template <int C>
__global__ __launch_bounds__(NT * 2, C == 8 ? SNNFLOW_BWD_SLOT_WAVES : SNNFLOW_L32_WAVES) void k_bwd_slot(BwdSlotParams) {
    static_assert(C != 8 || SlotLds<C>::BWD >= LayerBwdLds<C, C, true, true, 2>::FLOATS, "fused wgrad staging");
    static_assert(C != 8 || 2 * LayerBwdLds<C, C, true, true, 2>::FR >= NT * Pad<C>::v, "dgrad staging size");
    static_assert(SlotLds<C>::BWD >= LayerBwdLds<2, C, false, false, 2>::G + HN * Pad<2>::v &&
                      SlotLds<C>::BWD >= LayerBwdLds<4, C, false, false, 2>::G + HN * Pad<4>::v &&
                      SlotLds<C>::BWD >= WAcc<2, C, 2 * NT, 0>::SCRATCH && SlotLds<C>::BWD >= WAcc<4, C, 2 * NT, 0>::SCRATCH,
                  "fused head weight gradient staging");
    typedef const __attribute__((address_space(4))) BwdSlotParams* cptr;
    const cptr pp = (cptr)__builtin_amdgcn_kernarg_segment_ptr();
    Grid g;
    const int k = slot_task(pp, g);
    if (g.bid >= g.nb) return;
    __shared__ __attribute__((aligned(16))) float pool[SlotLds<C>::BWD];
    switch (pp->kind[k]) {
#define BWD_LAYER(ALL, KIND, ...)                             \
    case KIND: {                                              \
        if constexpr (ALL || kSlotAllKinds<C>) {              \
            const snnflow_layer_bwd_args a = task_args(&pp->layer[k]);       \
            layer_bwd_body<__VA_ARGS__>(a, g, pool);          \
        }                                                     \
        break;                                                \
    }
        BWD_LAYER(true, SK_HEAD2, 2, C, false, false, 2, false, false, true)
        BWD_LAYER(true, SK_HEAD4, 4, C, false, false, 2, false, false, true)
        BWD_LAYER(false, SK_PLAIN, C, C, false, false, 2)
        BWD_LAYER(false, SK_PLAIN_REC, C, C, false, true, 2)
        BWD_LAYER(true, SK_LIF, C, C, true, false, 2, SlotLds<C>::BFG, C == 8)
        BWD_LAYER(true, SK_LIF_REC, C, C, true, true, 2, SlotLds<C>::BFG, C == 8)
#undef BWD_LAYER
        case SK_TOP: {
            if constexpr (kSlotAllKinds<C>) {
                const snnflow_lif_bwd_args a = task_args(&pp->lif);
                lif_bwd_body<C, false, NT * 2>(a, g);
            }
            break;
        }
        case SK_TOP_PRED: {
            const snnflow_lif_bwd_args a = task_args(&pp->lif);
            if constexpr (C >= 16) lif_bwd_q_body<C, true, NT * 2>(a, g, pool);
            else lif_bwd_body<C, true, NT * 2>(a, g);
            break;
        }
        default: break;
    }
}

bool valid_c(int c) { return c == 4 || c == 8 || c == 16 || c == 32; }

template <int C>
int conv_fwd_c(const snnflow_conv_fwd_args& a, hipStream_t s) {
    constexpr int SP = C == 32 ? SNNFLOW_SP32 : ((C == 8 || C == 16) ? 2 : 1);
    const dim3 grid(snnflow_conv_blocks(a.B, a.H, a.W)), block(NT * SP);
    if (a.lif_in) {
        if (a.cin != C) SNN_FAIL(SNNFLOW_E_CHANNELS, "conv_fwd: lif_in requires cin == c");
        if (a.wt_rec) hipLaunchKernelGGL((k_conv_fwd<C, C, true, true, SP>), grid, block, 0, s, a);
        else hipLaunchKernelGGL((k_conv_fwd<C, C, true, false, SP>), grid, block, 0, s, a);
    } else if (a.wt_rec) {
        if (a.cin == C) hipLaunchKernelGGL((k_conv_fwd<C, C, false, true, SP>), grid, block, 0, s, a);
        else if (a.cin == 1) hipLaunchKernelGGL((k_conv_fwd<1, C, false, true, SP>), grid, block, 0, s, a);
        else if (a.cin == 2) hipLaunchKernelGGL((k_conv_fwd<2, C, false, true, SP>), grid, block, 0, s, a);
        else if (a.cin == 4) hipLaunchKernelGGL((k_conv_fwd<4, C, false, true, SP>), grid, block, 0, s, a);
        else if (a.cin == 5) hipLaunchKernelGGL((k_conv_fwd<5, C, false, true, SP>), grid, block, 0, s, a);
        else SNN_FAIL(SNNFLOW_E_CHANNELS, "conv_fwd: recurrent cell with unsupported cin (1, 2, 4, 5 or c)");
    } else {
        if (a.cin == 1) hipLaunchKernelGGL((k_conv_fwd<1, C, false, false, SP>), grid, block, 0, s, a);
        else if (a.cin == 2) hipLaunchKernelGGL((k_conv_fwd<2, C, false, false, SP>), grid, block, 0, s, a);
        else if (a.cin == 4) hipLaunchKernelGGL((k_conv_fwd<4, C, false, false, SP>), grid, block, 0, s, a);
        else if (a.cin == 5) hipLaunchKernelGGL((k_conv_fwd<5, C, false, false, SP>), grid, block, 0, s, a);
        else if (a.cin == C) hipLaunchKernelGGL((k_conv_fwd<C, C, false, false, SP>), grid, block, 0, s, a);
        else SNN_FAIL(SNNFLOW_E_CHANNELS, "conv_fwd: unsupported cin");
    }
    SNN_CHECK_LAUNCH();
    return 0;
}

int layer_bwd_blocks(const snnflow_layer_bwd_args& a) {
    const bool pixels = a.lif_in || (a.g_x && a.wt_bwd_ff) || (a.wt_bwd_rec && a.g_state_prev) || (a.wslab_ff && a.x);
    return pixels ? snnflow_conv_blocks(a.B, a.H, a.W) : 1;
}

template <int C>
int layer_bwd_c(const snnflow_layer_bwd_args& a, hipStream_t s) {
    constexpr int SP = C == 32 ? SNNFLOW_SP32 : ((C == 8 || C == 16) ? 2 : 1);
    const dim3 grid(layer_bwd_blocks(a)), block(NT * SP), block1(NT);
    if (a.lif_in) {
        if (a.cin != C) SNN_FAIL(SNNFLOW_E_CHANNELS, "layer_bwd: lif_in requires cin == c");
        const bool bfg = C >= 16 && a.wd_ff && (!a.wt_bwd_rec || !a.g_state_prev || a.wd_rec);
        if (bfg) {
            if (a.wt_bwd_rec) hipLaunchKernelGGL((k_layer_bwd<C, C, true, true, SP, C >= 16>), grid, block, 0, s, a);
            else hipLaunchKernelGGL((k_layer_bwd<C, C, true, false, SP, C >= 16>), grid, block, 0, s, a);
        } else if (a.wt_bwd_rec) hipLaunchKernelGGL((k_layer_bwd<C, C, true, true, SP>), grid, block, 0, s, a);
        else hipLaunchKernelGGL((k_layer_bwd<C, C, true, false, SP>), grid, block, 0, s, a);
    } else if (a.wt_bwd_rec) {
        if (a.cin == C) hipLaunchKernelGGL((k_layer_bwd<C, C, false, true, SP>), grid, block, 0, s, a);
        else if (a.cin == 1) hipLaunchKernelGGL((k_layer_bwd<1, C, false, true, 1>), grid, block1, 0, s, a);
        else if (a.cin == 2) hipLaunchKernelGGL((k_layer_bwd<2, C, false, true, 1>), grid, block1, 0, s, a);
        else if (a.cin == 4) hipLaunchKernelGGL((k_layer_bwd<4, C, false, true, 1>), grid, block1, 0, s, a);
        else if (a.cin == 5) hipLaunchKernelGGL((k_layer_bwd<5, C, false, true, 1>), grid, block1, 0, s, a);
        else SNN_FAIL(SNNFLOW_E_CHANNELS, "layer_bwd: recurrent cell with unsupported cin (1, 2, 4, 5 or c)");
    } else {
        if (a.cin == 1) hipLaunchKernelGGL((k_layer_bwd<1, C, false, false, 1>), grid, block1, 0, s, a);
        else if (a.cin == 2) hipLaunchKernelGGL((k_layer_bwd<2, C, false, false, 1>), grid, block1, 0, s, a);
        else if (a.cin == 4) hipLaunchKernelGGL((k_layer_bwd<4, C, false, false, 1>), grid, block1, 0, s, a);
        else if (a.cin == 5) hipLaunchKernelGGL((k_layer_bwd<5, C, false, false, 1>), grid, block1, 0, s, a);
        else if (a.cin == C) hipLaunchKernelGGL((k_layer_bwd<C, C, false, false, SP>), grid, block, 0, s, a);
        else SNN_FAIL(SNNFLOW_E_CHANNELS, "layer_bwd: unsupported cin");
    }
    SNN_CHECK_LAUNCH();
    return 0;
}

int elem_grid(int64_t n) {
    int64_t g = (n + NT - 1) / NT;
    return (int)(g < 1 ? 1 : g);
}

}

extern "C" {

int snnflow_abi_version(void) { return SNNFLOW_ABI_VERSION; }

#if SNNFLOW_TRACE
int snnflow_trace_copy(void* host, size_t bytes) {
    return (int)hipMemcpyFromSymbol(host, HIP_SYMBOL(g_trace), bytes < sizeof(g_trace) ? bytes : sizeof(g_trace), 0,
                                    hipMemcpyDeviceToHost);
}
#endif
const char* snnflow_last_error(void) { return g_err.c_str(); }

int snnflow_conv_blocks(int B, int H, int W) { return B * tiles_per_image(H, W); }

int snnflow_frag_halfs(int c, int cin) {
    if (cin != c || c <= 0 || c % 8 != 0 || c > 64) return 0;
    return FragGeo(c, c).halfs();
}

int snnflow_prep_weights_batch(const snnflow_prep_desc* d, int n, void* stream) {
    if (!d || n <= 0 || n > SNNFLOW_MAX_BATCH) SNN_FAIL(SNNFLOW_E_ARG, "prep_weights_batch: bad count");
    DescBatch<snnflow_prep_desc> batch = {};
    int maxe = 1;
    for (int i = 0; i < n; ++i) {
        const snnflow_prep_desc& x = d[i];
        if ((x.w && (x.c <= 0 || x.cin <= 0 || !x.wt_fwd || !x.wt_bwd)) || (!x.w && !x.threshold && !x.zero) ||
            (x.threshold && x.thr_n <= 0) || (x.zero && x.zero_n < 0))
            SNN_FAIL(SNNFLOW_E_ARG, "prep_weights_batch: bad descriptor");
        if ((x.frag_fwd || x.frag_bwd) && (!x.w || snnflow_frag_halfs(x.c, x.cin) == 0))
            SNN_FAIL(SNNFLOW_E_ARG, "prep_weights_batch: fragments need cin == c, c % 8 == 0");
        batch.d[i] = x;
        if (x.w && x.c * x.cin * 9 > maxe) maxe = x.c * x.cin * 9;
        if (x.frag_fwd || x.frag_bwd) {
            const int fe = snnflow_frag_halfs(x.c, x.cin) / 3;
            if (fe > maxe) maxe = fe;
        }
        if (x.threshold && x.thr_n > maxe) maxe = x.thr_n;
        if (x.zero) maxe = std::max(maxe, (int)std::min<int64_t>(x.zero_n, 65536));
    }
    hipLaunchKernelGGL(k_prep_weights, dim3((maxe + 255) / 256, n), dim3(256), 0, (hipStream_t)stream, batch);
    SNN_CHECK_LAUNCH();
    return 0;
}

int snnflow_prep_weights(const float* w, int c, int cin, float* wt_fwd, float* wt_bwd, float* threshold,
                         void* stream) {
    if (c <= 0 || cin <= 0 || (w && (!wt_fwd || !wt_bwd)) || (!w && !threshold))
        SNN_FAIL(SNNFLOW_E_ARG, "prep_weights: bad args");
    snnflow_prep_desc d = {w, c, cin, wt_fwd, wt_bwd, threshold, c, nullptr, nullptr, nullptr, 0};
    return snnflow_prep_weights_batch(&d, 1, stream);
}

static int conv_fwd_check(const snnflow_conv_fwd_args* a) {
    if (!a || a->B <= 0 || a->H <= 0 || a->W <= 0 || !a->wt_ff || !a->y)
        SNN_FAIL(SNNFLOW_E_ARG, "conv_fwd: bad args");
    if (a->cin == a->c && a->c % 8 == 0 && (!a->wt_ff_t || (a->wt_rec && !a->wt_rec_t)))
        SNN_FAIL(SNNFLOW_E_ARG, "conv_fwd: cin == c needs the backward-layout weights wt_ff_t / wt_rec_t");
    if (a->lif_in ? (!a->prev_y || !a->prev_state || (a->prev.bn_train && !a->prev_acc)) : !a->x)
        SNN_FAIL(SNNFLOW_E_ARG, "conv_fwd: missing input");
    const bool bits_ok = a->cin == a->c && (a->c == 8 || a->c == 16 || a->c == 32);
    if ((a->prev_spk_bits && !(bits_ok && a->lif_in)) || (a->s_prev_bits && !(bits_ok && a->wt_rec)))
        SNN_FAIL(SNNFLOW_E_ARG, "conv_fwd: spike bit planes need cin == c in {8, 16, 32} (and lif_in / a recurrent conv)");
    return 0;
}
// ... 136 lines not shown
        case SK_LIF_REC: case SK_PLAIN_REC: return 0;
        case SK_LIF: case SK_PLAIN: return 1;
        default: return 2;
    }
}

#ifndef SNNFLOW_SLOT_ORDER8
#define SNNFLOW_SLOT_ORDER8 0
#endif
extern "C++" template <typename A>
static void slot_sort(A* args, int* kind, int* nblk, int n, bool reverse = false) {
    if (!SNNFLOW_SLOT_ORDER) return;
    const int sg = reverse ? -1 : 1;
    for (int i = 1; i < n; ++i)
        for (int j = i; j > 0 && sg * slot_rank(kind[j]) < sg * slot_rank(kind[j - 1]); --j) {
            const A ta = args[j]; args[j] = args[j - 1]; args[j - 1] = ta;
            const int tk = kind[j]; kind[j] = kind[j - 1]; kind[j - 1] = tk;
            const int tn = nblk[j]; nblk[j] = nblk[j - 1]; nblk[j - 1] = tn;
        }
}

static int slot_top_blocks(int c, int B, int H, int W) {
    const int64_t npix = (int64_t)B * H * W;
    if (c < 16) return (int)((npix + 2 * NT - 1) / (2 * NT));
    const int64_t ppb = 2 * NT / (c / 4), target = snnflow_conv_blocks(B, H, W);
    const int64_t items = (npix + ppb * target - 1) / (ppb * target);
    return (int)((npix + ppb * items - 1) / (ppb * items));
}

static int env_int(const char* name, int dflt) {
    const char* v = getenv(name);
    return v && *v ? atoi(v) : dflt;
}
static int g_pipe_fwd = env_int("SNNFLOW_PIPE_FWD", 2);
static int g_pipe_order = env_int("SNNFLOW_PIPE_ORDER", 1);

static int pipe_blocks(int ntiles, int tpb) {
    const int nb = (ntiles + tpb - 1) / tpb;
    return (nb + 7) / 8 * 8;
}
static bool pipe_fits(int B, int H, int W, int c) { return (int64_t)B * H * W * c * 4 < ((int64_t)1 << 31); }

int snnflow_slot_supported(int c, int cin0) { return slot_c(c) && (cin0 == 2 || cin0 == 4) ? 1 : 0; }

static int slot_ranges(const int* nblk, int n, int* blk0) {
    int b = 0;
    for (int i = 0; i < n; ++i) {
        blk0[i] = b;
        b += (nblk[i] + 7) / 8 * 8;
    }
    return b;
}

int snnflow_fwd_slot(const snnflow_conv_fwd_args* conv, int nconv, const snnflow_lif_fwd_args* lif, void* stream) {
    const int nt = nconv + (lif ? 1 : 0);
    if (nconv < 0 || nt <= 0 || nt > kSlotTasks || (nconv && !conv)) SNN_FAIL(SNNFLOW_E_ARG, "fwd_slot: task count");
    FwdSlotParams p = {};
    const int c = nconv ? conv[0].c : lif->c;
    const int B = nconv ? conv[0].B : lif->B, H = nconv ? conv[0].H : lif->H, W = nconv ? conv[0].W : lif->W;
    if (!slot_c(c)) SNN_FAIL(SNNFLOW_E_CHANNELS, "fwd_slot: c must be 8, 16 or 32");
    for (int i = 0; i < nconv; ++i) {
        const snnflow_conv_fwd_args& a = conv[i];
        if (const int e = conv_fwd_check(&a)) return e;
        if (a.c != c || a.B != B || a.H != H || a.W != W) SNN_FAIL(SNNFLOW_E_ARG, "fwd_slot: tasks of different shapes");
        int kind;
        if (a.lif_in) {
            if (a.cin != c) SNN_FAIL(SNNFLOW_E_CHANNELS, "fwd_slot: lif_in requires cin == c");
            kind = a.wt_rec ? SK_LIF_REC : SK_LIF;
        } else if (a.wt_rec) {
            if (a.cin != c) SNN_FAIL(SNNFLOW_E_CHANNELS, "fwd_slot: recurrent cell requires cin == c");
            kind = SK_PLAIN_REC;
        } else if (a.cin == c) {
            kind = SK_PLAIN;
        } else if (a.cin == 1 || a.cin == 2 || a.cin == 4 || a.cin == 5) {
            kind = a.cin == 1 ? SK_HEAD1 : a.cin == 2 ? SK_HEAD2 : a.cin == 4 ? SK_HEAD4 : SK_HEAD5;
        } else {
            SNN_FAIL(SNNFLOW_E_CHANNELS, "fwd_slot: unsupported cin");
        }
        if (c != 8 && !(kind == SK_HEAD2 || kind == SK_HEAD4 || kind == SK_LIF || kind == SK_LIF_REC))
            SNN_FAIL(SNNFLOW_E_CHANNELS, "fwd_slot: c = 16 / 32 runs the LIFFireNet task kinds only");
        p.conv[i] = a;
        p.nblk[i] = snnflow_conv_blocks(B, H, W);
        if (c == 8 && g_pipe_fwd > 0 && (kind == SK_LIF || kind == SK_LIF_REC) && pipe_fits(B, H, W, c) &&
            !a.prev_spk_bits && !a.s_prev_bits)
            kind = kind == SK_LIF ? SK_LIF_P : SK_LIF_REC_P;
        p.kind[i] = kind;
    }
    const int tpb = g_pipe_fwd;
    for (int i = 0; i < nconv; ++i) {
        if (p.kind[i] != SK_LIF_P && p.kind[i] != SK_LIF_REC_P) continue;
        const int nt = p.nblk[i];
        p.nblk[i] = pipe_blocks(nt, tpb);
        if (p.nblk[i] > (nt + 7) / 8 * 8) p.nblk[i] = (nt + 7) / 8 * 8;
    }
    if (lif) {
        if (const int e = lif_fwd_check(lif)) return e;
        if (lif->c != c || lif->B != B || lif->H != H || lif->W != W)
            SNN_FAIL(SNNFLOW_E_ARG, "fwd_slot: tasks of different shapes");
        if (c != 8 && !lif->pred_w) SNN_FAIL(SNNFLOW_E_CHANNELS, "fwd_slot: c = 16 / 32 top task needs the prediction");
        p.lif = *lif;
        p.kind[nconv] = lif->pred_w ? SK_TOP_PRED : SK_TOP;
        p.nblk[nconv] = slot_top_blocks(c, B, H, W);
    }
    if (c != 8) slot_sort(p.conv, p.kind, p.nblk, nconv);
    else if (SNNFLOW_SLOT_ORDER8) slot_sort(p.conv, p.kind, p.nblk, nconv, SNNFLOW_SLOT_ORDER8 == 2);
    else if (g_pipe_fwd > 0 && g_pipe_order) slot_sort(p.conv, p.kind, p.nblk, nconv, g_pipe_order == 2);
    p.ntask = nt;
    const int nb = slot_ranges(p.nblk, nt, p.blk0);
    const hipStream_t s = (hipStream_t)stream;
    if (c == 8) hipLaunchKernelGGL(k_fwd_slot<8>, dim3(nb), dim3(2 * NT), 0, s, p);
    else if (c == 16) hipLaunchKernelGGL(k_fwd_slot<16>, dim3(nb), dim3(2 * NT), 0, s, p);
    else hipLaunchKernelGGL(k_fwd_slot<32>, dim3(nb), dim3(2 * NT), 0, s, p);
    SNN_CHECK_LAUNCH();
    return 0;
}

int snnflow_eval_slot(const snnflow_eval_fwd_args* tasks, int n, void* stream) {
    if (!tasks || n <= 0 || n > kEvalTasks) SNN_FAIL(SNNFLOW_E_ARG, "eval_slot: task count");
    EvalSlotParams p = {};
    const int B = tasks[0].B, H = tasks[0].H, W = tasks[0].W;
    for (int i = 0; i < n; ++i) {
        const snnflow_eval_fwd_args& a = tasks[i];
        if (a.c != 8) SNN_FAIL(SNNFLOW_E_CHANNELS, "eval_slot: c must be 8");
        if (a.B != B || a.H != H || a.W != W || B <= 0 || H <= 0 || W <= 0)
            SNN_FAIL(SNNFLOW_E_ARG, "eval_slot: tasks of different or empty shapes");
        if (a.n.bn_train) SNN_FAIL(SNNFLOW_E_ARG, "eval_slot: BatchNorm in train mode needs batch statistics (snnflow_fwd_slot)");
        if (!a.state || !a.wt_ff || !a.n.bn_weight || !a.n.bn_bias || !a.n.running_mean || !a.n.running_var ||
            !a.n.beta || !a.n.threshold)
            SNN_FAIL(SNNFLOW_E_ARG, "eval_slot: missing state, weights or neuron parameters");
        if (a.flow && (!a.pred_w || !a.pred_b)) SNN_FAIL(SNNFLOW_E_ARG, "eval_slot: prediction without weights");
        if (!pipe_fits(B, H, W, 8)) SNN_FAIL(SNNFLOW_E_ARG, "eval_slot: tensors of 2^31 bytes or more");
        const int ntiles = snnflow_conv_blocks(B, H, W);
        if (a.cin == a.c) {
            if (!a.s_in || !a.wt_ff_t) SNN_FAIL(SNNFLOW_E_ARG, "eval_slot: spike input / fragment weights missing");
            if (a.s_prev && (!a.wt_rec || !a.wt_rec_t)) SNN_FAIL(SNNFLOW_E_ARG, "eval_slot: recurrent weights missing");
            p.kind[i] = a.s_prev ? EK_REC : EK_FF;
            p.nblk[i] = pipe_blocks(ntiles, 2);
        } else if (a.cin == 2 || a.cin == 4) {
            if (!a.x || a.s_prev || a.flow) SNN_FAIL(SNNFLOW_E_ARG, "eval_slot: head task takes the event tensor only");
            p.kind[i] = a.cin == 2 ? EK_HEAD2 : EK_HEAD4;
            p.nblk[i] = ntiles;
        } else {
            SNN_FAIL(SNNFLOW_E_CHANNELS, "eval_slot: cin must be 2, 4 or c");
        }
        p.t[i] = a;
    }
    p.ntask = n;
    const int nb = slot_ranges(p.nblk, n, p.blk0);
    hipLaunchKernelGGL(k_eval_slot, dim3(nb), dim3(2 * NT), 0, (hipStream_t)stream, p);
    SNN_CHECK_LAUNCH();
    return 0;
}

int snnflow_bwd_slot(const snnflow_layer_bwd_args* layer, int nlayer, const snnflow_lif_bwd_args* lif,
                     void* stream) {
    const int nt = nlayer + (lif ? 1 : 0);
    if (nlayer < 0 || nt <= 0 || nt > kSlotTasks || (nlayer && !layer)) SNN_FAIL(SNNFLOW_E_ARG, "bwd_slot: task count");
    BwdSlotParams p = {};
    const int c = nlayer ? layer[0].c : lif->c;
    const int B = nlayer ? layer[0].B : lif->B, H = nlayer ? layer[0].H : lif->H, W = nlayer ? layer[0].W : lif->W;
    if (!slot_c(c)) SNN_FAIL(SNNFLOW_E_CHANNELS, "bwd_slot: c must be 8, 16 or 32");
    for (int i = 0; i < nlayer; ++i) {
        const snnflow_layer_bwd_args& a = layer[i];
        if (const int e = layer_bwd_check(&a)) return e;
        if (a.c != c || a.B != B || a.H != H || a.W != W) SNN_FAIL(SNNFLOW_E_ARG, "bwd_slot: tasks of different shapes");
        int kind;
        if (a.lif_in) {
            if (a.cin != c) SNN_FAIL(SNNFLOW_E_CHANNELS, "bwd_slot: lif_in requires cin == c");
            if (c >= 16 && (!a.wd_ff || (a.wt_bwd_rec && a.g_state_prev && !a.wd_rec)))
                SNN_FAIL(SNNFLOW_E_ARG, "bwd_slot: c >= 16 needs the pre-split input-gradient fragments wd_ff / wd_rec");
            kind = a.wt_bwd_rec ? SK_LIF_REC : SK_LIF;
        } else if (a.wt_bwd_rec) {
            if (a.cin != c) SNN_FAIL(SNNFLOW_E_CHANNELS, "bwd_slot: recurrent cell requires cin == c");
            kind = SK_PLAIN_REC;
        } else if (a.cin == c) {
            kind = SK_PLAIN;
        } else if (a.cin == 2 || a.cin == 4) {
            kind = a.cin == 2 ? SK_HEAD2 : SK_HEAD4;
        } else {
            SNN_FAIL(SNNFLOW_E_CHANNELS, "bwd_slot: unsupported cin (2, 4 or c)");
        }
        if (c != 8 && !(kind == SK_HEAD2 || kind == SK_HEAD4 || kind == SK_LIF || kind == SK_LIF_REC))
            SNN_FAIL(SNNFLOW_E_CHANNELS, "bwd_slot: c = 16 / 32 runs the LIFFireNet task kinds only");
        const bool head_wg = (kind == SK_HEAD2 || kind == SK_HEAD4) && a.x != nullptr && !a.wslab_rec && !a.wt_bwd_rec;
        if ((a.wslab_ff || a.wslab_rec) && !(c == 8 && (kind == SK_LIF || kind == SK_LIF_REC)) && !head_wg)
            SNN_FAIL(SNNFLOW_E_ARG, "bwd_slot: wslab_ff / wslab_rec need a c = 8 LIF-fed task or a head task with x");
        p.layer[i] = a;
        p.kind[i] = kind;
        p.nblk[i] = layer_bwd_blocks(a);
    }
    if (lif) {
        if (const int e = lif_bwd_check(lif)) return e;
        if (lif->c != c || lif->B != B || lif->H != H || lif->W != W)
            SNN_FAIL(SNNFLOW_E_ARG, "bwd_slot: tasks of different shapes");
        if (lif->mem_grad_in) SNN_FAIL(SNNFLOW_E_ARG, "bwd_slot: mem_grad_in is a standalone-cell option");
        if (c != 8 && !lif->pred_w) SNN_FAIL(SNNFLOW_E_CHANNELS, "bwd_slot: c = 16 / 32 top task needs the prediction");
        p.lif = *lif;
        p.kind[nlayer] = lif->pred_w ? SK_TOP_PRED : SK_TOP;
        p.nblk[nlayer] = slot_top_blocks(c, B, H, W);
    }
    if (c != 8) {
        slot_sort(p.layer, p.kind, p.nblk, nlayer);
    } else if (SNNFLOW_SLOT_ORDER8) {
        slot_sort(p.layer, p.kind, p.nblk, nlayer, SNNFLOW_SLOT_ORDER8 == 2);
    }
    p.ntask = nt;
    const int nb = slot_ranges(p.nblk, nt, p.blk0);
    const hipStream_t s = (hipStream_t)stream;
    if (c == 8) hipLaunchKernelGGL(k_bwd_slot<8>, dim3(nb), dim3(2 * NT), 0, s, p);
    else if (c == 16) hipLaunchKernelGGL(k_bwd_slot<16>, dim3(nb), dim3(2 * NT), 0, s, p);
    else hipLaunchKernelGGL(k_bwd_slot<32>, dim3(nb), dim3(2 * NT), 0, s, p);
    SNN_CHECK_LAUNCH();
    return 0;
}

int snnflow_set_pipe(int fwd_tiles_per_block, int bwd_tiles_per_block) {
    if (fwd_tiles_per_block < 0) SNN_FAIL(SNNFLOW_E_ARG, "set_pipe: negative tiles per block");
    if (bwd_tiles_per_block != 0) SNN_FAIL(SNNFLOW_E_ARG, "set_pipe: the backward runs one tile per block (ABI 38)");
    g_pipe_fwd = fwd_tiles_per_block;
    return 0;
}
int snnflow_get_pipe(int which) { return which == 0 ? g_pipe_fwd : 0; }

static int g_wg_bits = env_int("SNNFLOW_WG_BITS", 1);
static int g_wg_head_sp2 = env_int("SNNFLOW_WG_HEAD_SP2", 1);
static bool wgrad_all_x_bits(const snnflow_wgrad_args* a) {
    for (int t = 0; t < a->nsteps; ++t)
        if (!a->steps[t].x_bits) return false;
    return true;
}

int snnflow_wgrad(const snnflow_wgrad_args* a, void* stream) {
    if (!a || a->B <= 0 || a->H <= 0 || a->W <= 0 || a->nsteps <= 0 || a->nsteps > SNNFLOW_MAX_WGRAD_STEPS ||
        !a->slab_ff || (a->rec && !a->slab_rec))
        SNN_FAIL(SNNFLOW_E_ARG, "wgrad: bad args");
    for (int t = 0; t < a->nsteps; ++t) {
        const snnflow_wgrad_step& st = a->steps[t];
        if (!st.g_cur || !st.y || !(st.x || st.x_bits) || (st.stats && !st.bnc)) SNN_FAIL(SNNFLOW_E_ARG, "wgrad: incomplete step");
        if ((st.x_bits || st.s_prev_bits) && !(a->exact_inputs && a->cin == a->c && (a->c == 8 || a->c == 16 || a->c == 32)))
            SNN_FAIL(SNNFLOW_E_ARG, "wgrad: spike bit planes need exact_inputs and cin == c in {8, 16, 32}");
        if (st.stats && !a->bn_weight) SNN_FAIL(SNNFLOW_E_ARG, "wgrad: BatchNorm step needs bn_weight");
    }
    const hipStream_t s = (hipStream_t)stream;
    const dim3 grid(snnflow_conv_blocks(a->B, a->H, a->W));
    const int c = a->c, cin = a->cin;
    if (!valid_c(c)) SNN_FAIL(SNNFLOW_E_CHANNELS, "wgrad: c must be 4, 8, 16 or 32");
#define WG_LAUNCH(CI_, CC_, REC_)                                                                          \
    do {                                                                                                   \
        constexpr int SP_ = (CC_ == 8 || CC_ == 16 || (CC_ == 32 && CI_ % 16 == 0)) ? 2 : 1;              \
        constexpr int SP2_ = (CC_ == 32 && CI_ == 2 && !REC_) ? 2 : SP_;                                  \
        if (SP2_ != SP_ && !g_wg_head_sp2)                                                                \
            hipLaunchKernelGGL((k_wgrad<CI_, CC_, REC_, SP_>), grid, dim3(NT * SP_), 0, s, *a);           \
        else                                                                                              \
            hipLaunchKernelGGL((k_wgrad<CI_, CC_, REC_, SP2_>), grid, dim3(NT * SP2_), 0, s, *a);         \
    } while (0)
#define WG_PICK(CI_, CC_)                                                                                  \
    do {                                                                                                   \
        if (a->rec) WG_LAUNCH(CI_, CC_, true);                                                             \
        else WG_LAUNCH(CI_, CC_, false);                                                                   \
    } while (0)
#define WG_CASE(CC_)                                                                                       \
    case CC_:                                                                                              \
        if (cin == CC_) WG_PICK(CC_, CC_);                                                                 \
        else if (cin == 1) WG_PICK(1, CC_);                                                                \
        else if (cin == 2) WG_PICK(2, CC_);                                                                \
        else if (cin == 3) WG_PICK(3, CC_);                                                                \
        else if (cin == 4) WG_PICK(4, CC_);                                                                \
        else if (cin == 5) WG_PICK(5, CC_);                                                                \
        else SNN_FAIL(SNNFLOW_E_CHANNELS, "wgrad: unsupported cin");                                       \
        break;
    if (a->exact_inputs && cin == c && (c == 8 || c == 16 || c == 32)) {
        const dim3 blk(NT * 2);
        if (c == 8) {
            if (a->rec) hipLaunchKernelGGL((k_wgrad_bf<8, true>), grid, blk, 0, s, *a);
            else hipLaunchKernelGGL((k_wgrad_bf<8, false>), grid, blk, 0, s, *a);
        } else if (c == 16) {
            if (a->rec) hipLaunchKernelGGL((k_wgrad_bf<16, true>), grid, blk, 0, s, *a);
            else hipLaunchKernelGGL((k_wgrad_bf<16, false>), grid, blk, 0, s, *a);
        } else if (g_wg_bits && wgrad_all_x_bits(a)) {
            hipLaunchKernelGGL(k_wgrad_b32, dim3(a->rec ? 2 * ((grid.x + 7) / 8 * 8) : grid.x), blk, 0, s, *a);
        } else {
            if (a->rec) {
                if (SNNFLOW_WG32_SPLIT > 1) hipLaunchKernelGGL((k_wgrad_bf32<true>), grid, blk, 0, s, *a);
                else hipLaunchKernelGGL((k_wgrad_bf<32, true>), grid, blk, 0, s, *a);
            } else if (SNNFLOW_WG32_SPLIT) {
                hipLaunchKernelGGL((k_wgrad_bf32<false>), grid, blk, 0, s, *a);
            } else {
                hipLaunchKernelGGL((k_wgrad_bf<32, false>), grid, blk, 0, s, *a);
            }
        }
        SNN_CHECK_LAUNCH();
        return 0;
    }
    switch (c) {
        WG_CASE(4) WG_CASE(8) WG_CASE(16) WG_CASE(32)
        default: break;
    }
#undef WG_CASE
#undef WG_PICK
#undef WG_LAUNCH
    SNN_CHECK_LAUNCH();
    return 0;
}

int snnflow_slab_reduce(const snnflow_slab_desc* d, int n, int nblk, void* stream) {
    if (!d || n <= 0 || n > SNNFLOW_MAX_SLABS || nblk <= 0) SNN_FAIL(SNNFLOW_E_ARG, "slab_reduce: bad args");
    DescBatch<snnflow_slab_desc> batch = {};
    int maxe = 0;
    for (int i = 0; i < n; ++i) {
        batch.d[i] = d[i];
        if (!d[i].slab || !d[i].out || d[i].elems <= 0) SNN_FAIL(SNNFLOW_E_ARG, "slab_reduce: bad descriptor");
        maxe = d[i].elems > maxe ? d[i].elems : maxe;
    }
    hipLaunchKernelGGL(k_slab_reduce, dim3((maxe + SR_E - 1) / SR_E, n), dim3(SR_E * SR_G), 0, (hipStream_t)stream,
                       batch, nblk);
    SNN_CHECK_LAUNCH();
    return 0;
}

}

namespace {
constexpr int CLIP2_NB = 512;

__global__ __launch_bounds__(256) void k_clip_partial(const float* __restrict__ g, int64_t n, double* partials) {
    __shared__ double part[4];
    double s = 0.0;
    for (int64_t i = (int64_t)blockIdx.x * 256 + threadIdx.x; i < n; i += (int64_t)gridDim.x * 256) {
        const double v = g[i];
        s += v * v;
    }
#pragma unroll
    for (int off = 32; off > 0; off >>= 1) s += __shfl_xor(s, off, 64);
    if ((threadIdx.x & 63) == 0) part[threadIdx.x >> 6] = s;
    __syncthreads();
    if (threadIdx.x == 0) partials[blockIdx.x] = (part[0] + part[1]) + (part[2] + part[3]);
}

__global__ void k_clip_coef(const double* partials, int nb, float max_norm, float eps, float* total_out, float* coef) {
    if (threadIdx.x != 0) return;
    double t = 0.0;
    for (int i = 0; i < nb; ++i) t += partials[i];
    const float total = (float)sqrt(t);
    const float c = max_norm / (total + eps);
    coef[0] = c < 1.0f ? c : 1.0f;
    if (total_out) total_out[0] = total;
}

__global__ __launch_bounds__(256) void k_clip_scale(float* __restrict__ g, int64_t n, const float* coef) {
    const float c = coef[0];
    for (int64_t i = (int64_t)blockIdx.x * 256 + threadIdx.x; i < n; i += (int64_t)gridDim.x * 256) g[i] = g[i] * c;
}
}

extern "C" {

int snnflow_clip_grad_norm_large(float* g, int64_t n, float max_norm, float eps, float* total_out, double* scratch,
                                 void* stream) {
    if (!g || n < 0 || !scratch) SNN_FAIL(SNNFLOW_E_ARG, "clip_grad_norm_large: bad args");
    const hipStream_t s = (hipStream_t)stream;
    int64_t nb = (n + 255) / 256;
    if (nb > CLIP2_NB) nb = CLIP2_NB;
    if (nb < 1) nb = 1;
    float* coef = reinterpret_cast<float*>(scratch + CLIP2_NB);
    hipLaunchKernelGGL(k_clip_partial, dim3((unsigned)nb), dim3(256), 0, s, g, n, scratch);
    hipLaunchKernelGGL(k_clip_coef, dim3(1), dim3(64), 0, s, scratch, (int)nb, max_norm, eps, total_out, coef);
// ... 55 lines not shown
```

### snn_event-based_optical_flow_amd/snnflow/_lib.py

```python
import ctypes
import os

import torch

_HERE = os.path.dirname(os.path.abspath(__file__))
LIB_PATH = os.environ.get("SNNFLOW_LIB", os.path.join(_HERE, "libsnnflow.so"))

P = ctypes.c_void_p
I32 = ctypes.c_int
I64 = ctypes.c_int64
F32 = ctypes.c_float
F64 = ctypes.c_double

TILE_H, TILE_W = 8, 32
ABI_VERSION = 41
THETA_SCRATCH = 1024 * 32


class Neuron(ctypes.Structure):
    _fields_ = [("bn_weight", P), ("bn_bias", P), ("running_mean", P), ("running_var", P),
                ("num_batches_tracked", P), ("beta", P), ("threshold", P),
                ("momentum", F64), ("eps", F64), ("bn_train", I32), ("zero_reset", I32)]


# ... 192 lines not shown

class IweLossArgs(ctypes.Structure):
    _fields_ = [("B", I32), ("M", I32), ("T", I32), ("H", I32), ("W", I32), ("tf", I32),
                ("events", P * MAX_WINDOWS), ("pol", P * MAX_WINDOWS), ("flows", P * MAX_WINDOWS),
                ("masks", P * MAX_WINDOWS), ("off", ctypes.c_int32 * (MAX_WINDOWS + 1)),
                ("flow_scaling", F32), ("weight", F32),
                ("smoothing_mask", I32), ("overwrite_intermediate", I32), ("loss_scaling", I32),
                ("images", P), ("acc", P), ("persample", P), ("smooth", P), ("loss", P)]


UNET_MAX_SEGS = 4
UNET_MODE_S1, UNET_MODE_S2, UNET_MODE_T2 = 0, 1, 2
UNET_EPI_STORE, UNET_EPI_LIF = 0, 1
SURROGATES = {"arctanspike": 0, "superspike": 1, "mgspike": 2, "trianglespike": 3}


class UNetSeg(ctypes.Structure):
    _fields_ = [("x", P), ("H", I32), ("W", I32), ("cpitch", I32), ("mode", I32), ("kc0", I32), ("nparts", I32)]


class UNetConvArgs(ctypes.Structure):
    _fields_ = [("B", I32), ("Ho", I32), ("Wo", I32), ("M", I32), ("ksize", I32), ("nseg", I32),
                ("seg", UNetSeg * UNET_MAX_SEGS), ("w", P), ("kct", I32), ("mpad", I32), ("xparts", I32),
                ("xpart", I64), ("pclass", I32), ("epi", I32),
                ("out", P), ("ld", I32), ("accumulate", I32),
                ("leak", P), ("thresh", P), ("hard_reset", I32), ("prev_state", P), ("residual", P),
                ("res_pitch", I32), ("state", P), ("current", P), ("act", P), ("act_pitch", I32),
                ("ksplit", I32), ("partial", P)]


class UNetWgradArgs(ctypes.Structure):
    _fields_ = [("B", I32), ("Ho", I32), ("Wo", I32), ("M", I32), ("ksize", I32),
                ("g3", P), ("gpitch", I32), ("gpart", I64), ("seg", UNetSeg), ("k0", I32), ("ktot", I32),
                ("dwk", P), ("partial", P)]


class UNetLifBwdArgs(ctypes.Structure):
    _fields_ = [("P", I32), ("C", I32), ("leak", P), ("thresh", P), ("width", F32), ("hard_reset", I32),
                ("detach", I32), ("surrogate", I32), ("g_out", P), ("g_pitch", I32), ("g_state", P),
                ("state", P), ("prev_state", P), ("current", P), ("g_cur3", P), ("gc_pitch", I32),
                ("gc_part", I64), ("g_prev", P), ("g_res", P), ("gres_pitch", I32), ("acc", P), ("partial", P),
                ("res_assign", I32)]


MAX_LAYERS = 8
PL = P * MAX_LAYERS


class FireNetPlan(ctypes.Structure):
    _fields_ = [("L", I32), ("B", I32), ("H", I32), ("W", I32), ("c", I32), ("cin0", I32),
                ("rec", I32 * MAX_LAYERS), ("train", I32 * MAX_LAYERS), ("n", Neuron * MAX_LAYERS),
                ("wt_fwd_ff", PL), ("wt_fwd_rec", PL), ("wt_bwd_ff", PL), ("wt_bwd_rec", PL),
                ("wf_ff", PL), ("wf_rec", PL), ("wd_ff", PL), ("wd_rec", PL),
                ("fwd_acc", P), ("fwd_acc_stride", I64), ("bwd_acc", P), ("bwd_acc_stride", I64),
                ("pred_w", P), ("pred_b", P), ("slab_ff", PL), ("slab_rec", PL), ("nblk", I32)]


class FireNetFwdIo(ctypes.Structure):
    _fields_ = [("x", P), ("xs", I64 * 4), ("ys", P), ("stats", P), ("states", P), ("flow", P),
                ("mem_in", PL), ("s_prev", PL)]


class FireNetBwdIo(ctypes.Structure):
    _fields_ = [("ys", P), ("stats", P), ("flow", P), ("mem_in", PL), ("g_state", PL),
                ("g_flow", P), ("gflow_sb", I64), ("gflow_sc", I64), ("g_cur", P), ("bnc", P),
                ("g_prev", PL), ("ext", I32 * MAX_LAYERS), ("g_x", P), ("gxs", I64 * 4),
                ("ng", NeuronGrad * MAX_LAYERS), ("g_pred_w", P), ("g_pred_b", P), ("accumulate", I32)]


class FireNetSeqBwd(ctypes.Structure):
    _fields_ = [("T", I32), ("fresh", I32), ("fused", I32),
                ("ys", P * MAX_WINDOWS), ("stats", P * MAX_WINDOWS), ("flow", P * MAX_WINDOWS),
                ("states", P * MAX_WINDOWS), ("g_flow", P * MAX_WINDOWS),
                ("gflow_sb", I64 * MAX_WINDOWS), ("gflow_sc", I64 * MAX_WINDOWS),
                ("mem_in0", PL), ("s_prev0", PL), ("g_prev0", PL), ("ext0", I32 * MAX_LAYERS), ("g_state_last", PL),
                ("g_out", P), ("g_cur", P), ("bnc", P), ("bwd_acc", P), ("acc_stride", I64),
                ("ng", NeuronGrad * MAX_LAYERS), ("g_pred_w", P), ("g_pred_b", P),
                ("fuse_head", I32), ("x", P * MAX_WINDOWS), ("xs", (I64 * 4) * MAX_WINDOWS)]


class FireNetWgradStep(ctypes.Structure):
    _fields_ = [("g_cur", P), ("bnc", P), ("ys", P), ("stats", P), ("x", P), ("xs", I64 * 4), ("states", P),
                ("s_prev", PL)]


BN_PARTS = 256
ACT = {None: 0, "tanh": 1, "relu": 2, "sigmoid": 3}
PW_MAX_CIN, PW_MAX_COUT = 256, 4


class BnFwdArgs(ctypes.Structure):
    _fields_ = [("P", I64), ("C", I32), ("train", I32), ("x", P), ("y", P), ("weight", P), ("bias", P),
                ("running_mean", P), ("running_var", P), ("num_batches_tracked", P), ("momentum", F32), ("eps", F32),
                ("save_mean", P), ("save_invstd", P), ("scratch", P)]


class BnBwdArgs(ctypes.Structure):
    _fields_ = [("P", I64), ("C", I32), ("train", I32), ("x", P), ("g", P), ("weight", P), ("save_mean", P),
                ("save_invstd", P), ("g_x", P), ("g_weight", P), ("g_bias", P), ("scratch", P)]


class PointwiseArgs(ctypes.Structure):
    _fields_ = [("B", I32), ("H", I32), ("W", I32), ("cin", I32), ("cout", I32), ("act", I32), ("x", P),
                ("xs", I64 * 4), ("w", P), ("b", P), ("out", P), ("g_x", P), ("gxs", I64 * 4)]


EXPORTS = {
    "snnflow_abi_version": (I32, []),
    "snnflow_last_error": (ctypes.c_char_p, []),
    "snnflow_conv_blocks": (I32, [I32, I32, I32]),
    "snnflow_prep_weights": (I32, [P, I32, I32, P, P, P, P]),
    "snnflow_prep_weights_batch": (I32, [ctypes.POINTER(PrepDesc), I32, P]),
    "snnflow_conv_fwd": (I32, [ctypes.POINTER(ConvFwdArgs), P]),
    "snnflow_lif_fwd": (I32, [ctypes.POINTER(LifFwdArgs), P]),
    "snnflow_lif_bwd": (I32, [ctypes.POINTER(LifBwdArgs), P]),
    "snnflow_layer_bwd": (I32, [ctypes.POINTER(LayerBwdArgs), P]),
    "snnflow_wgrad": (I32, [ctypes.POINTER(WgradArgs), P]),
    "snnflow_convlif_fwd": (I32, [ctypes.POINTER(ConvLifFwdArgs), P]),
    "snnflow_encode_events": (I32, [ctypes.POINTER(EncodeArgs), P]),
    "snnflow_loader_prepare": (I32, [ctypes.POINTER(LoaderArgs), P]),
    "snnflow_loader_scratch_floats": (I64, [I32, I32, I32, I32, I32, I32, I32, I32, I32]),
    "snnflow_pol_iwe":(I32, [P, P, P, I64, I32, I32, I32, I32, I32, F32, F32, I32, P, P]),
    "snnflow_aee": (I32, [ctypes.POINTER(AeeArgs), P]),
    "snnflow_aee_acc_doubles": (I32, [I32, I32, I32]),
    "snnflow_flow_metrics": (I32, [ctypes.POINTER(FlowMetricsArgs), P]),
    "snnflow_flow_metrics_rows": (I32, [I32, I32, I32]),
    "snnflow_percentiles": (I32, [ctypes.POINTER(PercentilesArgs), P]),
    "snnflow_flow_to_image": (I32, [ctypes.POINTER(FlowToImageArgs), P]),
    "snnflow_events_to_image": (I32, [ctypes.POINTER(EventsToImageArgs), P]),
    "snnflow_minmax_norm": (I32, [ctypes.POINTER(MinmaxNormArgs), P]),
    "snnflow_error_to_image": (I32, [P, I64, P, P]),
    "snnflow_error_maps": (I32, [ctypes.POINTER(ErrorMapsArgs), P]),
    "snnflow_convlif_bwd": (I32, [ctypes.POINTER(ConvLifBwdArgs), P]),
    "snnflow_convlif_param_grads": (I32, [P, P, P, I32, I32, P, P, P]),
    "snnflow_slab_reduce": (I32, [ctypes.POINTER(SlabDesc), I32, I32, P]),
    "snnflow_iwe_loss_fwd": (I32, [ctypes.POINTER(IweLossArgs), P]),
    "snnflow_iwe_loss_bwd": (I32, [ctypes.POINTER(IweLossArgs), P, P, P]),
    "snnflow_device_errors": (I32, [I32]),
    "snnflow_iwe_scratch_floats": (I64, [I32, I32, I32, I32, I32, I32]),
    "snnflow_iwe_acc_doubles": (I32, [I32, I32, I32, I32]),
    "snnflow_iwe_corners": (I32, [P, P, I32, I32, F32, I32, I32, F32, I32, P, P, P]),
    "snnflow_iwe_interpolate": (I32, [P, P, P, I64, I32, I32, I32, I32, P, P]),
    "snnflow_iwe_corners_bwd": (I32, [P, P, I32, I32, F32, I32, I32, F32, P, P, P]),
    "snnflow_iwe_interpolate_bwd": (I32, [P, P, I64, I32, I32, I32, I32, P, P, P]),
    "snnflow_lif_export": (I32, [P, P, P, P, I32, I32, I32, P, P, P]),
    "snnflow_lif_theta_subtract": (I32, [P, P, P, I64, I32, P, P, P]),
    "snnflow_clip_grad_norm": (I32, [P, I64, F32, F32, P, P]),
    "snnflow_clip_grad_norm_large": (I32, [P, I64, F32, F32, P, P, P]),
    "snnflow_clip_adam": (I32, [P, P]),
    "snnflow_eval_slot": (I32, [P, I32, P]),
    "snnflow_count_nonzero": (I32, [P, P, I32, P, P]),
    "snnflow_fwd_slot": (I32, [ctypes.POINTER(ConvFwdArgs), I32, ctypes.POINTER(LifFwdArgs), P]),
    "snnflow_bwd_slot": (I32, [ctypes.POINTER(LayerBwdArgs), I32, ctypes.POINTER(LifBwdArgs), P]),
    "snnflow_slot_supported": (I32, [I32, I32]),
    "snnflow_set_pipe": (I32, [I32, I32]),
    "snnflow_get_pipe": (I32, [I32]),
    "snnflow_frag_halfs": (I32, [I32, I32]),
    "snnflow_unet_conv": (I32, [ctypes.POINTER(UNetConvArgs), P]),
    "snnflow_unet_conv_ksplit": (I32, [ctypes.POINTER(UNetConvArgs)]),
    "snnflow_unet_prep_weights": (I32, [P, I32, I32, I32, P, I32, I32, I32, I32, I32, I32, I32, P, P]),
    "snnflow_unet_wgrad": (I32, [ctypes.POINTER(UNetWgradArgs), P]),
    "snnflow_unet_wgrad_partial_floats": (I64, [ctypes.POINTER(UNetWgradArgs)]),
    "snnflow_unet_wgrad_finalize": (I32, [P, I32, P, I32, I32, I32, I32, I32, I32, P, P]),
    "snnflow_unet_lif_bwd": (I32, [ctypes.POINTER(UNetLifBwdArgs), P]),
    "snnflow_unet_lif_bwd_partial_doubles": (I32, [I32, I32, I32]),
    "snnflow_unet_cell_param_grads": (I32, [P, P, P, I32, I32, P, P, P]),
    "snnflow_unet_pack": (I32, [P, I32, I32, I32, I32, I64, I64, I64, I64, I32, P, I32, P]),
    "snnflow_unet_dec_in": (I32, [P, I32, I32, P, I32, I32, P, I32, I32, I32, P, I32, P]),
    "snnflow_unet_dec_in_bwd": (I32, [P, I32, I32, I32, I32, I32, I32, I32, P, I32, P, I32, P, I32, P]),
    "snnflow_unet_pred_fwd": (I32, [P, I32, I32, P, P, I32, I32, I32, I32, P, P, P]),
    "snnflow_unet_pred_bwd": (I32, [P, I32, I32, P, P, P, P, I32, I32, I32, I32, P, P, I32, P, I32, P, P]),
    "snnflow_unet_pred_bwd_partial_doubles": (I32, [I32, I32, I32, I32]),
    "snnflow_unet_pred_param_grads": (I32, [P, I32, I32, P, P, P]),
    "snnflow_firenet_fwd": (I32, [ctypes.POINTER(FireNetPlan), ctypes.POINTER(FireNetFwdIo), P]),
    "snnflow_firenet_bwd": (I32, [ctypes.POINTER(FireNetPlan), ctypes.POINTER(FireNetBwdIo), P]),
    "snnflow_firenet_bwd_seq": (I32, [ctypes.POINTER(FireNetPlan), ctypes.POINTER(FireNetSeqBwd), ctypes.POINTER(I32), P]),
    "snnflow_firenet_wgrad": (I32, [ctypes.POINTER(FireNetPlan), ctypes.POINTER(FireNetWgradStep), I32, P, P, P]),
    "snnflow_bn_fwd": (I32, [ctypes.POINTER(BnFwdArgs), P]),
    "snnflow_bn_bwd": (I32, [ctypes.POINTER(BnBwdArgs), P]),
    "snnflow_bn_scratch_doubles": (I32, [I32]),
    "snnflow_pointwise_fwd": (I32, [ctypes.POINTER(PointwiseArgs), P]),
    "snnflow_pointwise_bwd": (I32, [ctypes.POINTER(PointwiseArgs), P, I64, I64, P, P, P, P]),
}
MAX_SLOT_TASKS = 4
MAX_COUNT_TENSORS = 16


def _load():
    if not os.path.exists(LIB_PATH):
        raise ImportError(
            f"snnflow HIP library not found at {LIB_PATH}; build it with "
            "`make -C snn_event-based_optical_flow_amd/csrc` (or __graft_entry__.build()). "
            "There is no CPU fallback.")
    lib = ctypes.CDLL(LIB_PATH)
    for name, (res, args) in EXPORTS.items():
        fn = getattr(lib, name)
        fn.restype = res
        fn.argtypes = args
    if lib.snnflow_abi_version() != ABI_VERSION:
        raise ImportError("snnflow ABI version mismatch; rebuild libsnnflow.so")
    return lib


lib = _load()


class SnnflowError(RuntimeError):
    pass


def check(rc, what):
    if rc != 0:
        raise SnnflowError(f"{what} failed ({rc}): {lib.snnflow_last_error().decode(errors='replace')}")


_DEVICE_FAULTS = {1: "event-warping forward: a bin segment outside its window's records (k_iwe_splat)",
                  2: "event-warping backward: a bin segment outside its window's records (k_iwe_bwd_band)"}


def check_device_errors(clear=True):
    rc = lib.snnflow_device_errors(1 if clear else 0)
    if rc < 0 or rc > 0xFFFF:
        check(rc, "device_errors")
    if rc:
        what = "; ".join(v for k, v in _DEVICE_FAULTS.items() if rc & k) or f"flags {rc:#x}"
        raise SnnflowError(f"device-side fault detected and skipped: {what}")


class KernelTimer:

    GROUPED = ("fwd_slot", "bwd_slot")

    def __init__(self):
        self.records = []
        self.open = None

    def close(self):
        if self.open is not None:
            name, a, n, work = self.open
            b = torch.cuda.Event(enable_timing=True)
            b.record()
            self.records.append((name, a, b, work, n))
            self.open = None

    def summary(self):
        self.close()
        torch.cuda.synchronize()
        out = {}
        for name, a, b, work, cnt in self.records:
            ms = a.elapsed_time(b)
            n, tot, w = out.get(name, (0, 0.0, 0.0))
            out[name] = (n + cnt, tot + ms, w + (work or 0.0))
        return {k: {"launches": n, "total_ms": tot, "avg_us": 1000.0 * tot / n, "work": w}
                for k, (n, tot, w) in out.items()}


TIMER = None


def timer_close():
    if TIMER is not None:
        TIMER.close()


def call(name, fn, *args, work=None):
    if TIMER is None:
        check(fn(*args), name)
        return
    if name in TIMER.GROUPED:
        if TIMER.open is None or TIMER.open[0] != name:
            TIMER.close()
            a = torch.cuda.Event(enable_timing=True)
            a.record()
            TIMER.open = [name, a, 0, 0.0]
        check(fn(*args), name)
        TIMER.open[2] += 1
        TIMER.open[3] += work or 0.0
        return
    TIMER.close()
    a = torch.cuda.Event(enable_timing=True)
    b = torch.cuda.Event(enable_timing=True)
    a.record()
    check(fn(*args), name)
    b.record()
    TIMER.records.append((name, a, b, work, 1))


def ptr(t):
    if t is None:
        return None
    return t.data_ptr()


_HIP_SEEN = False


def stream_ptr(device=None):
    global _HIP_SEEN
    if not _HIP_SEEN:
        if not torch.cuda.is_available():
            raise SnnflowError("snnflow kernels need a HIP device (none visible); there is no CPU fallback")
        _HIP_SEEN = True
    if isinstance(device, str):
        device = torch.device(device)
    idx = device.index if isinstance(device, torch.device) else device
    if idx is None:
        idx = torch.cuda.current_device()
    return torch._C._cuda_getCurrentRawStream(idx)


def require_device(t, name):
    if not t.is_cuda:
        raise SnnflowError(f"{name} must be a HIP device tensor (got {t.device}); there is no CPU fallback")
    if t.dtype != torch.float32:
        raise SnnflowError(f"{name} must be float32 (got {t.dtype})")
```

### snn_event-based_optical_flow_amd/snnflow/engine.py

```python
import ctypes
import operator
import os

import torch

from . import _lib
from ._lib import check, lib, ptr



def nhwc_state_strides(B, C, H, W):
    return (B * H * W * C, H * W * C, 1, W * C, C)


def empty_state(B, C, H, W, device):
    return torch.empty_strided((2, B, C, H, W), nhwc_state_strides(B, C, H, W), device=device, dtype=torch.float32)


def as_nhwc_state(s):
    two, B, C, H, W = s.shape
    if s.stride() == nhwc_state_strides(B, C, H, W) and s.dtype == torch.float32:
        return s
    out = empty_state(B, C, H, W, s.device)
    out.copy_(s)
    return out


def as_nhwc(t):
    B, C, H, W = t.shape
    if t.stride() == (H * W * C, 1, W * C, C) and t.dtype == torch.float32:
        return t
    return t.contiguous(memory_format=torch.channels_last).float()


def neuron_struct(cell, weight=None, bias=None):
    bn, lif = getattr(cell, "batch_norm", cell.bn), cell.lif
    train = bn.training or not bn.track_running_stats
    return _lib.Neuron(
        ptr(bn.weight if weight is None else weight), ptr(bn.bias if bias is None else bias),
        ptr(bn.running_mean) if bn.track_running_stats else None,
        ptr(bn.running_var) if bn.track_running_stats else None,
        ptr(bn.num_batches_tracked) if (bn.training and bn.track_running_stats) else None,
        ptr(lif.beta), ptr(lif.threshold),
        float(bn.momentum if bn.momentum is not None else 0.0), float(bn.eps),
        1 if train else 0, 1 if cell.hard_reset else 0)


class Workspace:

    def __init__(self, B, H, W, C, layers, device):
        self.key = (B, H, W, C, device)
        self.B, self.H, self.W, self.C = B, H, W, C
        self.nblk = lib.snnflow_conv_blocks(B, H, W)
        self.fwd_acc = torch.zeros(max(layers, 1), _lib.acc_storage(2 * C), dtype=torch.float64, device=device)
        self.bwd_acc = torch.zeros(max(layers, 1), _lib.acc_storage(_lib.bwd_acc_len(C)), dtype=torch.float64,
                                   device=device)
        self.slab_ff = []
        self.slab_rec = []
        self.device = device

    def reset_acc(self):
        self.fwd_acc.zero_()
        self.bwd_acc.zero_()

    def slabs(self, layer_shapes):
        if len(self.slab_ff) != len(layer_shapes):
            dev = self.device
            self.slab_ff = [torch.empty(self.nblk, self.C * cin * 9, device=dev) for cin, _ in layer_shapes]
            self.slab_rec = [torch.empty(self.nblk, self.C * self.C * 9, device=dev) if rec else None
                             for _, rec in layer_shapes]
        return self.slab_ff, self.slab_rec


class PreppedWeights:

    def __init__(self):
        self.fwd = {}
        self.bwd = {}
        self.frag = {}
        self.fragb = {}
        self.key = None
        self.gen = 0

    def weight_version(self):
        src = self.__dict__.get("src")
        if src is None:
            return -1
        return sum(w._version for w in src) + sum(t._version for t in self.__dict__.get("th", ()))

    def ensure(self, weights, thresholds, stream, refresh=True, zero=None):
        ver = sum(w._version for w in weights) + sum(t._version for t in thresholds)
        same = self.__dict__.get("src") is weights
        if not same:
            key = tuple((w.data_ptr(), w._version) for w in weights) + tuple((t.data_ptr(), t._version) for t in thresholds)
            if key != self.key:
                refresh = True
            self.key = key
            self.src = weights
            self.th = thresholds
        elif ver != self.__dict__.get("ver"):
            refresh = True
        self.ver = ver
        fresh = False
        shapes = tuple((w.data_ptr(), w.numel()) for w in weights) if not same else self.shapes
        for i, w in enumerate(weights if shapes != self.__dict__.get("shapes") else ()):
            f = self.fwd.get(i)
            if f is None or f.numel() != w.numel() or f.device != w.device:
                self.fwd[i] = torch.empty(w.numel(), device=w.device)
                self.bwd[i] = torch.empty(w.numel(), device=w.device)
                c, cin = w.shape[0], w.shape[1]
                nf = lib.snnflow_frag_halfs(c, cin) if c >= 16 else 0
                self.frag[i] = torch.empty(nf, dtype=torch.int16, device=w.device) if nf else None
                self.fragb[i] = torch.empty(nf, dtype=torch.int16, device=w.device) if nf else None
                fresh = True
        self.shapes = shapes
        if fresh:
            self.gen += 1
        if not (refresh or fresh):
            if zero is not None:
                d = _lib.PrepDesc()
                d.zero, d.zero_n = zero.data_ptr(), zero.numel()
                _lib.call("prep_weights", lib.snnflow_prep_weights_batch, (_lib.PrepDesc * 1)(d), 1, stream)
            return
        descs = []
        for i, w in enumerate(weights):
            c, cin = w.shape[0], w.shape[1]
            if not w.is_contiguous():
                raise _lib.SnnflowError("conv weight must be contiguous")
            descs.append(_lib.PrepDesc(ptr(w), c, cin, ptr(self.fwd[i]), ptr(self.bwd[i]), None, 0,
                                       _ptr_t(self.frag.get(i)), _ptr_t(self.fragb.get(i))))
        for i, t in enumerate(thresholds):
            if i < len(descs):
                descs[i].threshold, descs[i].thr_n = ptr(t), t.numel()
            else:
                descs.append(_lib.PrepDesc(None, 0, 0, None, None, ptr(t), t.numel()))
        if zero is not None:
            if not descs:
                descs.append(_lib.PrepDesc())
            descs[0].zero, descs[0].zero_n = zero.data_ptr(), zero.numel()
        for i0 in range(0, len(descs), _lib.MAX_BATCH):
            chunk = descs[i0:i0 + _lib.MAX_BATCH]
            _lib.call("prep_weights", lib.snnflow_prep_weights_batch, (_lib.PrepDesc * len(chunk))(*chunk),
                      len(chunk), stream)


class FireNetEngine:

    def __init__(self, model):
        self.cells = [getattr(model, name) for name, _ in model.layer_spec]
        self.rec = [rec for _, rec in model.layer_spec]
        self.pred = model.pred.conv2d
        self.L = len(self.cells)
        self.C = self.cells[0].hidden_size
        self.ws = None
        self.prep = PreppedWeights()
        self.bwd_open = False
        self.flat = None
        self.flat_views = None
        self.pending = []
        self.pending_layers = []
        self.slab_live = [False] * self.L
        self.fuse_wgrad = self.C == 8
        fh = os.environ.get("SNNFLOW_FUSE_HEAD")
        self.fuse_head = (self.C >= 16) if fh is None else fh != "0"
        self.spk_bits = os.environ.get("SNNFLOW_SPK_BITS", "1") != "0"
        self.defer_backward = os.environ.get("SNNFLOW_DEFER_BWD", "1") != "0"
        self.keep_seq_states = False
        self.capture_states = False
        self.final_state_out = None
        self.seq_states = None
        self.prep_stale = True
        self.lifs = [c.lif for c in self.cells]
        self.bns = [getattr(c, "batch_norm", c.bn) for c in self.cells]
        self._plist = None
        self._neurons = None
        self._gen = 0

    def __deepcopy__(self, memo):
        import copy
        new = self.__class__.__new__(self.__class__)
        memo[id(self)] = new
        for k, v in self.__dict__.items():
            new.__dict__[k] = None if k in ("_neurons", "_nk_src", "_plist", "_prep_ws", "_prep_map", "_plan", "_gviews", "_layout",
                                            "_anchor") \
                else copy.deepcopy(v, memo)
        return new

    def invalidate(self):
        self._plist = None
        self._neurons = None
        self._prep_ws = None
        self._prep_map = None
        self._plan = None
        self._gen = self.__dict__.get("_gen", 0) + 1

    def _neuron_key(self):
        src = self.__dict__.get("_nk_src")
        if src is None:
            src = [(c, bn, bn._parameters, bn._buffers, lif._parameters, lif._buffers)
                   for c, bn, lif in zip(self.cells, self.bns, self.lifs)]
            self._nk_src = src
        tens, scal = [], []
        for c, bn, bp, bb, lp, lb in src:
            tens += (bp.get("weight"), bp.get("bias"), bb.get("running_mean"), bb.get("running_var"),
                     bb.get("num_batches_tracked"), lp["beta"] if "beta" in lp else lb.get("beta"),
                     lp["threshold"] if "threshold" in lp else lb.get("threshold"))
            scal += (bn.training, bn.track_running_stats, bn.momentum, bn.eps, c.hard_reset)
        return tens, scal

    def neurons(self):
        tens, scal = self._neuron_key()
        n = self._neurons
        if n is None or n[1] != scal or not all(map(operator.is_, n[0], tens)):
            self._neurons = (tens, scal, [neuron_struct(c) for c in self.cells])
            self._gen = self.__dict__.get("_gen", 0) + 1
        return self._neurons[2]

    def any_subtract(self):
        return any(lif.reset_mechanism == "subtract" for lif in self.lifs)

    def sequence_ok(self, cin0):
        return bool(lib.snnflow_slot_supported(self.C, cin0))

    def param_list(self):
        pl = self._plist
        if pl is not None and all(d.get(k) is v for d, k, v in pl[1]):
            return pl[0]
        ps = self._param_list()
        checks = []
        for cell, rec in zip(self.cells, self.rec):
            checks.append((cell.ff._parameters, "weight", cell.ff.weight))
            if rec:
                checks.append((cell.rec._parameters, "weight", cell.rec.weight))
            bn = getattr(cell, "batch_norm", cell.bn)
            checks += [(bn._parameters, "weight", bn.weight), (bn._parameters, "bias", bn.bias),
                       (cell.lif._parameters, "beta", cell.lif._parameters.get("beta")),
                       (cell.lif._parameters, "threshold", cell.lif._parameters.get("threshold"))]
        checks += [(self.pred._parameters, "weight", self.pred.weight), (self.pred._parameters, "bias", self.pred.bias)]
        self._plist = (tuple(ps), checks)
        self._neurons = None
        self._prep_ws = None
        return self._plist[0]

    def _param_list(self):
        ps = []
        for cell, rec in zip(self.cells, self.rec):
            ps.append(cell.ff.weight)
            if rec:
                ps.append(cell.rec.weight)
            ps += [cell.bn.weight, cell.bn.bias, cell.lif.beta, cell.lif.threshold]
        ps += [self.pred.weight, self.pred.bias]
        return ps

    def workspace(self, B, H, W, device):
        key = (B, H, W, self.C, device)
        if self.ws is None or self.ws.key != key:
            self.ws = Workspace(B, H, W, self.C, self.L, device)
            self.ws.slabs([(c.input_size, r) for c, r in zip(self.cells, self.rec)])
        return self.ws

    def prep_weights(self, stream, refresh=True, zero=None):
        ws = self.__dict__.get("_prep_ws")
        if ws is None or self._plist is None:
            ws = []
            for cell, rec in zip(self.cells, self.rec):
                ws.append(cell.ff.weight)
                if rec:
                    ws.append(cell.rec.weight)
            self._prep_ws = ws
            self._prep_th = [c.lif.threshold for c in self.cells]
            self._prep_map = None
        self.prep.ensure(ws, self._prep_th, stream, refresh, zero)
        m = self._prep_map
        if m is not None and m[0] == self.prep.gen:
            return m[1], m[2]
        fwd, bwd, frag, fragb, i = [], [], [], [], 0
        for rec in self.rec:
            ff = (self.prep.fwd[i], self.prep.bwd[i], self.prep.frag.get(i), self.prep.fragb.get(i))
            i += 1
            rc = (None, None, None, None)
            if rec:
                rc = (self.prep.fwd[i], self.prep.bwd[i], self.prep.frag.get(i), self.prep.fragb.get(i))
                i += 1
            fwd.append((ff[0], rc[0]))
            bwd.append((ff[1], rc[1]))
            frag.append((ff[2], rc[2]))
            fragb.append((ff[3], rc[3]))
        self.frags, self.fragsb = frag, fragb
        self._prep_map = (self.prep.gen, fwd, bwd)
        return fwd, bwd

    def flat_layout_for(self, params):
        layout = self.__dict__.get("_layout")
        if layout is None or layout[0] != [id(p) for p in params]:
            lay, off = [], 0
            for p in params:
                lay.append((off, p.numel(), p.shape))
                off += p.numel()
            layout = ([id(p) for p in params], lay, off)
            self._layout = layout
        return layout[1]

    def anchor(self, states):
        params = self.param_list()
        if not torch.is_grad_enabled() or not any(p.requires_grad for p in params):
            return None
        cont = False
        for p, rec in zip(states, self.rec):
            if rec and p is not None and p.requires_grad and getattr(p.grad_fn, "eng", None) is self:
                cont = True
                break
        a = self.__dict__.get("_anchor")
        if not cont or a is None or a[0] is not params:
            self._anchor = (params, ParamAnchor.apply(self, *params))
        return self._anchor[1]

    def prepped(self):
# ... 530 lines not shown
    gl = [as_nhwc_state(g) if g is not None else None for g in steps[-1].g_states]
    for l in range(L):
        q.mem_in0[l], q.s_prev0[l], q.g_prev0[l] = mem0[l], sp0[l], _ptr_t(g0[l])
        q.ext0[l] = 1 if first.ext[l] else 0
        q.g_state_last[l] = _ptr_t(gl[l])
        q.ng[l] = glayers[l][2]
    q.g_out = buf.data_ptr() + 4 * (ng_ + nb_) if no_ else None
    q.g_cur, q.bnc = gcur.data_ptr(), bnc.data_ptr()
    q.bwd_acc, q.acc_stride = bacc.data_ptr(), nacc
    q.g_pred_w, q.g_pred_b = gpw, gpb
    live = (ctypes.c_int * L)(*[1 if v else 0 for v in eng.slab_live])
    try:
        _lib.call("firenet_bwd_seq", lib.snnflow_firenet_bwd_seq, ctypes.byref(plan), ctypes.byref(q), live, s)
        eng.slab_live = [bool(v) for v in live]
        if eng.any_subtract():
            for t, st in enumerate(steps):
                for l in range(L):
                    theta_subtract(eng.cells[l], gcur[t][l].data_ptr(), st.ptrs[0][l], B * H * W,
                                   glayers[l][2].threshold, s)
        for t in range(T - 1, -1, -1):
            st = steps[t]
            x, ys, stats = st.saved[:3]
            eng.pending.append((_Rows(gcur[t]), _Rows(bnc[t]), _Rows(ys), _Rows(stats), x, st.saved[4:4 + L],
                                st.ptrs[1], (st.saved, buf), None))
            eng.pending_layers.append(tuple(l for l in range(L) if not ((fuse and l > 0) or (fuse_head and l == 0))))
        eng.flush_weight_grads(B, H, W, cin0, ws, glayers, s, plan)
    except Exception:
        eng.ws.reset_acc()
        eng.bwd_open = False
        eng.pending, eng.pending_layers = [], []
        eng.prep_stale = True
        raise
    g_anchor = eng.flat if first.needs[2 + L] else None
    eng.flat_views = None
    eng.bwd_open = False
    eng.last_flat = eng.flat
    eng.prep_stale = True
    del gfl
    return (None, None, *g0, g_anchor)


def _step_backward(eng, ctx, g_states=None):
    g_flow = ctx.g_flow
    if g_states is None:
        g_states = ctx.g_states
    L, C = eng.L, eng.C
    B, H, W, cin0 = ctx.shape
    saved = ctx.saved
    x, ys, stats, flow = saved[:4]
    states = saved[4:4 + L]
    keep = saved[4 + L:]
    mem_in, s_prev = ctx.ptrs

    dev = x.device
    s = _lib.stream_ptr(dev)
    ws = eng.workspace(B, H, W, dev)
    wfwd, wbwd = eng.prepped()
    if not eng.bwd_open:
        eng.open_chain(dev)
        acc = 0
    else:
        acc = 1
    glayers, gpw, gpb = eng.grad_views()
    neurons = eng.neurons()
    bacc = _Rows(ws.bwd_acc)
    zn = ws.bwd_acc.shape[1]
    gst = [as_nhwc_state(g) if g is not None else None for g in g_states]
    g_prev = [None] * L
    for l in range(L):
        if not (ctx.has_prev[l] and ctx.needs[2 + l]):
            continue
        if ctx.ext[l]:
            g_prev[l] = torch.zeros((2, B, C, H, W), device=dev).as_strided(
                (2, B, C, H, W), (B * H * W * C, H * W * C, 1, W * C, C))
        elif eng.rec[l]:
            g_prev[l] = empty_state(B, C, H, W, dev)
    gmem = [g_prev[l] if (g_prev[l] is not None and ctx.ext[l]) else None for l in range(L)]

    gcur_t = torch.empty(L, B, H, W, C, device=dev)
    bnc_t = torch.empty(L, 2, C, device=dev)
    gcur, bnc, ys, stats = _Rows(gcur_t), _Rows(bnc_t), _Rows(ys), _Rows(stats)
    eng.pending.append((gcur, bnc, ys, stats, x, states, s_prev, (keep, gcur_t, bnc_t, saved), None))
    eng.pending_layers.append(tuple(range(L)))
    try:
        if g_flow is not None and (g_flow.stride(3) != 1 or g_flow.stride(2) != W or g_flow.dtype != torch.float32):
            g_flow = g_flow.contiguous().float()
        gx = None
        if ctx.needs[1]:
            gx = torch.empty_like(x)
        plan = None if _lib.TIMER is not None else eng.plan(B, H, W, cin0, ws, wfwd, wbwd)
        if plan is not None:
            io = _lib.FireNetBwdIo()
            io.ys, io.stats, io.flow = ys.base, stats.base, flow.data_ptr()
            for l in range(L):
                io.mem_in[l] = mem_in[l]
                io.g_state[l] = _ptr_t(gst[l])
                io.g_prev[l] = _ptr_t(g_prev[l])
                io.ext[l] = 1 if ctx.ext[l] else 0
                io.ng[l] = glayers[l][2]
            if g_flow is not None:
                io.g_flow, io.gflow_sb, io.gflow_sc = g_flow.data_ptr(), g_flow.stride(0), g_flow.stride(1)
            io.g_cur, io.bnc = gcur.base, bnc.base
            if gx is not None:
                io.g_x = gx.data_ptr()
                io.gxs[0], io.gxs[1], io.gxs[2], io.gxs[3] = gx.stride()
            io.g_pred_w, io.g_pred_b, io.accumulate = gpw, gpb, acc
            _lib.call("firenet_bwd", lib.snnflow_firenet_bwd, ctypes.byref(plan), ctypes.byref(io), s)
        else:
            b = _bwd_top_args(eng, B, H, W, ys, stats, mem_in, neurons, gst, g_flow, flow, gcur, gmem, bacc)
            b.zero0, b.zero_n = bacc[0], zn
            _lib.call("lif_bwd", lib.snnflow_lif_bwd, ctypes.byref(b), s)
            for l in range(L - 1, -1, -1):
                a = _bwd_layer_args(eng, l, B, H, W, cin0, ys, stats, mem_in, neurons, gst, gcur, gmem, bacc, bnc,
                                    glayers, gpw, gpb, acc, wfwd, wbwd, g_prev, ctx.ext, gx)
                if l + 1 <= L - 1:
                    a.zero0, a.zero_n = bacc[l + 1], zn
                _lib.call(f"layer_bwd[{l}]", lib.snnflow_layer_bwd, ctypes.byref(a), s)
        if eng.any_subtract():
            for l in range(L):
                theta_subtract(eng.cells[l], gcur[l], mem_in[l], B * H * W, glayers[l][2].threshold, s)
        if ctx.root:
            eng.flush_weight_grads(B, H, W, cin0, ws, glayers, s, plan)
    except Exception:
        ws.reset_acc()
        eng.bwd_open = False
        eng.pending, eng.pending_layers = [], []
        eng.prep_stale = True
        raise

    g_anchor = None
    if ctx.root:
        g_anchor = eng.flat if ctx.needs[2 + L] else None
        eng.flat_views = None
        eng.bwd_open = False
        eng.last_flat = eng.flat
        eng.prep_stale = True
    return (None, gx, *g_prev, g_anchor)


def _ptr_t(t):
    if t is None or isinstance(t, int):
        return t
    return t.data_ptr()


def wavefront_slots(T, K):
    slots = [[] for _ in range(K + 2 * (T - 1))]
    for t in range(T):
        for k in range(K):
            slots[k + 2 * t].append((k, t))
    return slots


def _state_rows(st_all, fin, T):
    rows = [st_all[t] for t in range(st_all.shape[0])]
    return rows + [fin] if fin is not None else rows


class FireNetSequence(torch.autograd.Function):

    @staticmethod
    def forward(ctx, eng, T, *rest):
        L, C = eng.L, eng.C
        xs = list(rest[:T])
        prev = list(rest[T:T + L])
        B, cin0, H, W = xs[0].shape
        dev = xs[0].device
        for x in xs:
            _lib.require_device(x, "event tensor")
            if tuple(x.shape) != (B, cin0, H, W):
                raise _lib.SnnflowError("forward_sequence: every step's input must have the same shape")
        s = _lib.stream_ptr(dev)
        ws = eng.workspace(B, H, W, dev)
        nf, nb = T * L * _lib.acc_storage(2 * C), T * L * _lib.acc_storage(_lib.bwd_acc_len(C))
        accs = torch.empty(nf + nb, dtype=torch.float64, device=dev)
        facc = accs[:nf].view(T, L, -1)
        ctx.bacc = accs[nf:].view(T, L, -1)
        wfwd, wbwd = eng.prep_weights(s, refresh=eng.prep_stale, zero=accs)
        eng.prep_stale = False
        cells = eng.cells

        ys = torch.empty(T, L, B, H, W, C, device=dev)
        stats = torch.empty(T, L, 2, C, device=dev)
        n1 = 2 * B * H * W * C
        fin = eng.final_state_out
        eng.final_state_out = None
        if fin is not None:
            if (fin.device != dev or fin.dtype != torch.float32 or fin.numel() != L * n1 or not fin.is_contiguous()
                    or any(p is not None and p.untyped_storage().data_ptr() == fin.untyped_storage().data_ptr()
                           for p in prev)):
                raise _lib.SnnflowError("final_state_out: a contiguous fp32 buffer of L*2*B*H*W*C floats on the "
                                        "input's device, not aliasing the initial states")
            fin = fin.view(L * n1)
        st_all = torch.empty(T - (fin is not None), L * n1, device=dev)
        rows = _state_rows(st_all, fin, T)
        states = [[rows[t][l * n1:(l + 1) * n1].as_strided((2, B, C, H, W), nhwc_state_strides(B, C, H, W))
                   for l in range(L)] for t in range(T)]
        flows = [torch.empty(B, 2, H, W, device=dev) for _ in range(T)]

        mem0, sprev0 = [], []
        root = True
        ext = [False] * L
        for l in range(L):
            p = prev[l]
            if p is None:
                cache = cells[l].lif.mem
                mem0.append(cache if (cache is not None and tuple(cache.shape) == (B, C, H, W)
                                      and cache.device == dev) else None)
                sprev0.append(None)
            else:
                pn = as_nhwc_state(p)
                mem0.append(pn[0])
                sprev0.append(pn[1] if eng.rec[l] else None)
                ours = getattr(p.grad_fn, "eng", None) is eng
                if eng.rec[l] and p.requires_grad and ours:
                    root = False
                ext[l] = p.requires_grad and not ours
        mem_in = [mem0] + [[states[t - 1][l][0] for l in range(L)] for t in range(1, T)]
        s_prev = [sprev0] + [[states[t - 1][l][1] if eng.rec[l] else None for l in range(L)] for t in range(1, T)]
        neurons = eng.neurons()
        train = [bn.training or not bn.track_running_stats for bn in eng.bns]

        fuse = bool(eng.fuse_wgrad)

        bits_on = eng.spk_bits and C in (16, 32) and not fuse
        need_bits = [bits_on and l < L - 1 for l in range(L)]
        bits = (torch.empty(T, L, B * H * W * C // 8, dtype=torch.uint8, device=dev) if any(need_bits)
                else None)
        bptr = [[bits[t, l].data_ptr() if need_bits[l] else None for l in range(L)] for t in range(T)]

        def spk_skip(l, t):
            return t < T - 1 and not eng.keep_seq_states and ((fuse and not eng.rec[l]) or need_bits[l])
        for tasks in wavefront_slots(T, L + 1):
            convs, top = [], None
            for k, t in tasks:
                if k < L:
                    a = _fwd_conv_args(eng, k, B, H, W, cin0, xs[t], ys[t], stats[t], states[t], mem_in[t],
                                       s_prev[t], facc[t], neurons, train, wfwd, wbwd)
                    if k >= 1 and spk_skip(k - 1, t):
                        a.state_spk_skip = 1
                    if k >= 1 and need_bits[k - 1]:
                        a.prev_spk_bits = bptr[t][k - 1]
                    if eng.rec[k] and t >= 1 and need_bits[k]:
                        a.s_prev_bits, a.s_prev = bptr[t - 1][k], None
                    convs.append(a)
                else:
                    top = _fwd_top_args(eng, B, H, W, ys[t], stats[t], states[t], mem_in[t], facc[t], neurons,
                                        flows[t])
                    if spk_skip(L - 1, t):
                        top.state_spk_skip = 1
            arr = (_lib.ConvFwdArgs * max(len(convs), 1))(*convs)
            _lib.call("fwd_slot", lib.snnflow_fwd_slot, arr, len(convs), ctypes.byref(top) if top is not None else None,
                      s)
        _lib.timer_close()

        if eng.capture_states:
            eng.seq_debug = (ys, stats, facc)
        for l in range(L):
            cells[l].lif.mem = states[T - 1][l][0].detach()
        eng.seq_states = [[st.detach() for st in sts] for sts in states] if eng.keep_seq_states else None

        ctx.eng = eng
        ctx.T = T
        ctx.fuse = fuse
        ctx.bptr = bptr
        ctx.bits = bits
        ctx.root = root
        ctx.ext = ext
        ctx.shape = (B, H, W, cin0)
        ctx.has_prev = [p is not None for p in prev]
        ctx.has_mem = [m is not None for m in mem0]
        saved = xs + flows + [ys, stats, st_all]
        ctx.has_fin = fin is not None
        if fin is not None:
            saved.append(fin)
        saved += [m for m in mem0 if m is not None]
        saved += [sp for sp in sprev0 if sp is not None]
        ctx.save_for_backward(*saved)
        ctx.set_materialize_grads(False)
        return (*flows, *states[T - 1])

    @staticmethod
    def backward(ctx, *grads):
        eng, T = ctx.eng, ctx.T
        L, C = eng.L, eng.C
        B, H, W, cin0 = ctx.shape
        g_flows, g_final = list(grads[:T]), list(grads[T:T + L])
        saved = list(ctx.saved_tensors)
        xs, flows = saved[:T], saved[T:2 * T]
        ys, stats, st_all = saved[2 * T:2 * T + 3]
        rest = saved[2 * T + 3:]
        fin = rest.pop(0) if ctx.has_fin else None
        rows = _state_rows(st_all, fin, T)
        n1 = 2 * B * H * W * C
        states = [[rows[t][l * n1:(l + 1) * n1].as_strided((2, B, C, H, W), nhwc_state_strides(B, C, H, W))
                   for l in range(L)] for t in range(T)]
        mem0 = [rest.pop(0) if ctx.has_mem[l] else None for l in range(L)]
        sprev0 = [rest.pop(0) if (ctx.has_prev[l] and eng.rec[l]) else None for l in range(L)]
        mem_in = [mem0] + [[states[t - 1][l][0] for l in range(L)] for t in range(1, T)]
        s_prev = [sprev0] + [[states[t - 1][l][1] if eng.rec[l] else None for l in range(L)] for t in range(1, T)]

        dev = xs[0].device
        s = _lib.stream_ptr(dev)
        eng.drop_stale_chain()
        eng.workspace(B, H, W, dev)
        ws = eng.ws
        wfwd, wbwd = eng.prep_weights(s, refresh=False)
        fresh = not eng.bwd_open
        if fresh:
            eng.open_chain(dev)
        glayers, gpw, gpb = eng.grad_views()
        neurons = eng.neurons()
        bacc = ctx.bacc
        ctx.bacc = None
        if bacc is None:
            bacc = torch.zeros(T, L, _lib.acc_storage(_lib.bwd_acc_len(C)), dtype=torch.float64, device=dev)
        gcur = torch.empty(T, L, B, H, W, C, device=dev)
        bnc = torch.empty(T, L, 2, C, device=dev)

        g_into = [None] * T
        g_into[T - 1] = [as_nhwc_state(g) if g is not None else None for g in g_final]
        g_out = [None] * T
        for t in range(T - 1, 0, -1):
            g_out[t] = [empty_state(B, C, H, W, dev) if eng.rec[l] else None for l in range(L)]
            g_into[t - 1] = g_out[t]
        g0 = [None] * L
        for l in range(L):
            if not (ctx.has_prev[l] and ctx.needs_input_grad[2 + T + l]):
                continue
            if ctx.ext[l]:
                g0[l] = torch.zeros((2, B, C, H, W), device=dev).as_strided(
                    (2, B, C, H, W), (B * H * W * C, H * W * C, 1, W * C, C))
            elif eng.rec[l]:
                g0[l] = empty_state(B, C, H, W, dev)
        g_out[0] = g0
        ext = [list(ctx.ext)] + [[False] * L for _ in range(T - 1)]
        gmem = [[None] * L for _ in range(T)]
        gmem[0] = [g0[l] if (g0[l] is not None and ctx.ext[l]) else None for l in range(L)]
        gxs = [torch.empty_like(xs[t]) if ctx.needs_input_grad[2 + t] else None for t in range(T)]
        gfl = []
        for g in g_flows:
            if g is not None and (g.stride(3) != 1 or g.stride(2) != W or g.dtype != torch.float32):
                g = g.contiguous().float()
            gfl.append(g)

        fuse = ctx.fuse
        fuse_head = (bool(eng.fuse_head) and not eng.rec[0] and cin0 in (2, 4)
                     and all(x.dim() == 4 and x.dtype == torch.float32 for x in xs))
        bptr = ctx.bptr
        for t in range(T - 1, -1, -1):
            eng.pending.append((_Rows(gcur[t]), _Rows(bnc[t]), _Rows(ys[t]), _Rows(stats[t]), xs[t], states[t], s_prev[t],
                                (gcur, bnc, ys, stats, ctx.bits), (bptr[t], bptr[t - 1] if t >= 1 else [None] * L)))
            eng.pending_layers.append(tuple(l for l in range(L) if not ((fuse and l > 0) or (fuse_head and l == 0))))
        try:
            for tasks in wavefront_slots(T, L + 1):
                layers, top = [], None
                for j, tau in tasks:
                    t = T - 1 - tau
                    acc = 0 if (fresh and t == T - 1) else 1
                    if j == 0:
                        top = _bwd_top_args(eng, B, H, W, ys[t], stats[t], mem_in[t], neurons, g_into[t], gfl[t],
                                            flows[t], gcur[t], gmem[t], bacc[t])
                    else:
                        l = L - j
                        a = _bwd_layer_args(eng, l, B, H, W, cin0, ys[t], stats[t], mem_in[t], neurons,
                                            g_into[t], gcur[t], gmem[t], bacc[t], bnc[t], glayers, gpw, gpb,
                                            acc, wfwd, wbwd, g_out[t], ext[t], gxs[t] if l == 0 else None)
                        if t > 0:
                            a.zero_mem_half = 0
                        if fuse_head and l == 0:
                            a.x = xs[t].data_ptr()
                            a.xs_b, a.xs_c, a.xs_h, a.xs_w = _x_strides(xs[t])
                            a.wslab_ff = ws.slab_ff[0].data_ptr()
                            a.wslab_accumulate = 1 if eng.slab_live[0] else 0
                            eng.slab_live[0] = True
                        if fuse and l > 0:
                            a.wslab_ff = ws.slab_ff[l].data_ptr()
                            if eng.rec[l]:
                                a.wslab_rec = ws.slab_rec[l].data_ptr()
                                a.s_prev = _ptr_t(s_prev[t][l])
                            a.wslab_accumulate = 1 if eng.slab_live[l] else 0
                            eng.slab_live[l] = True
                        layers.append(a)
                arr = (_lib.LayerBwdArgs * max(len(layers), 1))(*layers)
                _lib.call("bwd_slot", lib.snnflow_bwd_slot, arr, len(layers),
                          ctypes.byref(top) if top is not None else None, s)
            _lib.timer_close()
            for l in range(L):
                for t in range(T):
                    theta_subtract(eng.cells[l], gcur[t][l], mem_in[t][l], B * H * W, glayers[l][2].threshold, s)
            if ctx.root:
                eng.flush_weight_grads(B, H, W, cin0, ws, glayers, s)
        except Exception:
            ws.reset_acc()
            eng.bwd_open = False
            eng.pending, eng.pending_layers = [], []
            eng.prep_stale = True
            raise

        pgrads = [None] * len(eng.flat_layout)
        if ctx.root:
            pgrads = [eng.flat[o:o + n].view(shp) for o, n, shp in eng.flat_layout]
            eng.flat_views = None
            eng.bwd_open = False
            eng.last_flat = eng.flat
            eng.prep_stale = True
        return (None, None, *gxs, *g0, *pgrads)


def eval_fused_ok(eng, xs, prev=()):
    import os
    x = xs[0]
    if os.environ.get("SNNFLOW_EVAL_FUSED", "1") == "0" or eng.C != 8 or not x.is_cuda or x.shape[1] not in (2, 4):
        return False
    if any(bn.training or not bn.track_running_stats for bn in eng.bns):
        return False
    if not torch.is_grad_enabled():
        return True
    return not (any(p.requires_grad for p in eng.param_list()) or any(t.requires_grad for t in xs)
                or any(p is not None and p.requires_grad for p in prev))


def eval_sequence(eng, xs, prev):
    L, C = eng.L, eng.C
    T = len(xs)
    B, cin0, H, W = xs[0].shape
    dev = xs[0].device
    for x in xs:
        _lib.require_device(x, "event tensor")
        if tuple(x.shape) != (B, cin0, H, W):
            raise _lib.SnnflowError("forward_sequence: every step's input must have the same shape")
    s = _lib.stream_ptr(dev)
    wfwd, wbwd = eng.prep_weights(s, refresh=eng.prep_stale)
    eng.prep_stale = False
    neurons = eng.neurons()
    n1 = 2 * B * H * W * C
    fin = eng.final_state_out
    eng.final_state_out = None
    if fin is not None:
        if (fin.device != dev or fin.dtype != torch.float32 or fin.numel() != L * n1 or not fin.is_contiguous()
                or any(p is not None and p.untyped_storage().data_ptr() == fin.untyped_storage().data_ptr()
                       for p in prev)):
            raise _lib.SnnflowError("final_state_out: a contiguous fp32 buffer of L*2*B*H*W*C floats on the "
                                    "input's device, not aliasing the initial states")
        fin = fin.view(L * n1)
    st_all = torch.empty(T - (fin is not None), L * n1, device=dev)
    rows = _state_rows(st_all, fin, T)
    sst = nhwc_state_strides(B, C, H, W)
    states = [[rows[t][l * n1:(l + 1) * n1].as_strided((2, B, C, H, W), sst) for l in range(L)] for t in range(T)]
    flows = [torch.empty(B, 2, H, W, device=dev) for _ in range(T)]
    half = 4 * (n1 // 2)
    keep, mem0, sp0 = [], [], []
    for l in range(L):
        p = prev[l]
        if p is None:
            cache = eng.lifs[l].mem
            ok = cache is not None and tuple(cache.shape) == (B, C, H, W) and cache.device == dev
            if ok and cache.stride() != (H * W * C, 1, W * C, C):
                cache = cache.permute(0, 2, 3, 1).contiguous().permute(0, 3, 1, 2)
            mem0.append(cache.data_ptr() if ok else None)
            sp0.append(None)
            keep.append(cache if ok else None)
        else:
            pn = as_nhwc_state(p.detach())
            mem0.append(pn.data_ptr())
            sp0.append(pn.data_ptr() + half if eng.rec[l] else None)
            keep.append(pn)
    base = [r.data_ptr() for r in rows]

    def targs(l, t):
        a = _lib.EvalFwdArgs()
        a.B, a.H, a.W, a.c = B, H, W, C
        if l == 0:
            x = xs[t]
            a.cin, a.x = cin0, x.data_ptr()
            a.xs_b, a.xs_c, a.xs_h, a.xs_w = _x_strides(x)
        else:
            a.cin, a.s_in = C, base[t] + 4 * (l - 1) * n1 + half
        a.mem_prev = mem0[l] if t == 0 else base[t - 1] + 4 * l * n1
        if eng.rec[l]:
            a.s_prev = sp0[l] if t == 0 else base[t - 1] + 4 * l * n1 + half
        a.wt_ff, a.wt_rec = ptr(wfwd[l][0]), _ptr_t(wfwd[l][1])
        a.wt_ff_t, a.wt_rec_t = ptr(wbwd[l][0]), _ptr_t(wbwd[l][1])
        a.n = neurons[l]
        a.state = base[t] + 4 * l * n1
        if l == L - 1:
            a.pred_w, a.pred_b, a.flow = ptr(eng.pred.weight), ptr(eng.pred.bias), flows[t].data_ptr()
        return a

    for d in range(T + L - 1):
        tasks = [(l, d - l) for l in range(L) if 0 <= d - l < T]
        for i0 in range(0, len(tasks), _lib.EVAL_MAX_TASKS):
            chunk = [targs(l, t) for l, t in tasks[i0:i0 + _lib.EVAL_MAX_TASKS]]
            _lib.call("eval_slot", lib.snnflow_eval_slot, (_lib.EvalFwdArgs * len(chunk))(*chunk), len(chunk), s)
    _lib.timer_close()
    del keep
    for l in range(L):
        eng.cells[l].lif.mem = states[T - 1][l][0]
    eng.seq_states = [list(sts) for sts in states] if eng.keep_seq_states else None
    return flows, states[T - 1]
```

Before: 65.70 million events/s.

## Chain recurrent and following feed-forward backward layer tasks in one block via LDS handoff

Adds a chained backward path in which a recurrent LIF layer's backward task at step t and the following feed-forward layer's task at step t-1 run back-to-back in the same thread block. The recurrent-state gradient is passed through LDS instead of a global g_state buffer. A new dependency-aware scheduler packs up to 7 tasks per launch instead of 4, and the kernel argument struct is compacted to fit. This removes a global round trip and reduces the number of wavefront launches, at the cost of serializing the two halves within a block and adding argument unpacking and extra syncs.

```diff
diff --git a/include/snnflow.h b/include/snnflow.h
--- a/include/snnflow.h
+++ b/include/snnflow.h
@@ -136,6 +136,9 @@
 int snnflow_bwd_slot(const snnflow_layer_bwd_args* layer, int nlayer, const snnflow_lif_bwd_args* lif,
                      void* stream);
 int snnflow_slot_supported(int c, int cin0);
+#define SNNFLOW_MAX_CHAIN_TASKS 7
+int snnflow_bwd_chain(const snnflow_layer_bwd_args* layer, int nlayer, const unsigned char* pair,
+                      const snnflow_lif_bwd_args* lif, void* stream);
 int snnflow_set_pipe(int fwd_tiles_per_block, int bwd_tiles_per_block);
 int snnflow_get_pipe(int which);
 
diff --git a/snn_event-based_optical_flow_amd/csrc/lif_layers.hip b/snn_event-based_optical_flow_amd/csrc/lif_layers.hip
--- a/snn_event-based_optical_flow_amd/csrc/lif_layers.hip
+++ b/snn_event-based_optical_flow_amd/csrc/lif_layers.hip
@@ -1183,7 +1183,7 @@
 constexpr int kPkRecOff = SNNFLOW_SWZ ? 16 : 0;
 
 __device__ void fused_wgrad_stage_pk(const float* G, float* wl_x, float* wl_r, const float (&xsp)[4], const float4& sp,
-                                     int pt, int ci0) {
+                                     int pt, int ci0, bool over_x = false) {
     constexpr int C = 8, PART = HN * C, XS = 16;
     static_assert(FragFloats<true, 8, 2 * NT>::v >= NT * XS / 2 && FragFloats<true, 8, 2 * NT>::v >= 2 * (kWgfR + kWgfP) + kPkRecOff,
                   "packed x|s tile in wl_x, both result sets in wl_r");
@@ -1217,6 +1217,7 @@
 #pragma unroll 2
     for (int row = 0; row < TH; ++row) kstep(wv, row, acc);
     kstep(8, wv, acc8);
+    if (over_x) __syncthreads();
     const int n = lane & 15;
     if (g4 < 2) {
         float* R = wl_r + (n < C ? 0 : kWgfR + kWgfP + kPkRecOff);
@@ -1383,7 +1384,7 @@
 };
 
 template <int CIN, int C, bool LIF_IN, bool REC, int SPLIT, bool BFG = false, bool WGF = false, bool HWG = false>
-__device__ void layer_bwd_body(const snnflow_layer_bwd_args& a, const Grid g, float* lds) {
+__device__ void layer_bwd_body(const snnflow_layer_bwd_args& a, const Grid g, float* lds, const int chain = 0) {
     using LB = LayerBwdLds<CIN, C, LIF_IN, REC, SPLIT, BFG>;
     static_assert(!HWG || (!LIF_IN && !REC && !kMfma<CIN, C>), "fused head weight gradient: feed-forward head tasks");
     static_assert(!WGF || (LIF_IN && C == 8 && CIN == 8 && SPLIT == 2 && LB::BF6 && LB::FR >= kWgfFloats),
@@ -1409,10 +1410,12 @@
     const Tile tl = block_tile(H, W, g);
     const double N = (double)a.B * H * W;
     const float nf = (float)N;
+    constexpr bool CHAIN2 = WGF && !REC && QI == 1;
     const int h = tl.h0 + ty, w = tl.w0 + tx;
     const bool in = (h < H) && (w < W);
     const int64_t pix = ((int64_t)tl.b * H + h) * W + w;
     const float4 z4 = make_float4(0.f, 0.f, 0.f, 0.f);
+    [[maybe_unused]] const bool has_gsp = REC && (a.g_state_prev != nullptr || (WGF && chain == 1));
     [[maybe_unused]] constexpr bool TR = LIF_IN && CIN == C && SNNFLOW_TRACE_LAYER;
     [[maybe_unused]] constexpr int TK = REC ? 3 : 2;
     TRACE_AT(TR, TK, 0);
@@ -1453,20 +1456,20 @@
     if constexpr (WL) {
         if (a.wt_bwd_ff) sw_x.load(a.wt_fwd_ff);
         if constexpr (REC) {
-            if (a.g_state_prev) sw_r.load(a.wt_fwd_rec);
+            if (has_gsp) sw_r.load(a.wt_fwd_rec);
         }
     }
     constexpr bool PKC = FLDS && REC && CIN == 8 && C == 8;
-    [[maybe_unused]] const bool pkr = PKC && a.wt_bwd_ff != nullptr && a.g_state_prev != nullptr;
+    [[maybe_unused]] const bool pkr = PKC && a.wt_bwd_ff != nullptr && has_gsp;
     if constexpr (FLDS) {
         if constexpr (PKC) {
             if (pkr) fs_x.load2(a.wt_fwd_ff, a.wt_fwd_rec);
             else if (a.wt_bwd_ff) fs_x.load(a.wt_fwd_ff);
-            if (!pkr && a.g_state_prev) fs_r.load(a.wt_fwd_rec);
+            if (!pkr && has_gsp) fs_r.load(a.wt_fwd_rec);
         } else {
             if (a.wt_bwd_ff) fs_x.load(a.wt_fwd_ff);
             if constexpr (REC) {
-                if (a.g_state_prev) fs_r.load(a.wt_fwd_rec);
+                if (has_gsp) fs_r.load(a.wt_fwd_rec);
             }
         }
     }
@@ -1518,6 +1521,10 @@
                 dm[q] = ld4_or_zero(pm4, py4, base + q);
                 dg[q] = ld4_or_zero(pg4 ? pg4 + plane4 : nullptr, py4, base + q);
             }
+            if constexpr (CHAIN2) {
+                if (chain == 2)
+                    dg[0] = *reinterpret_cast<const float4*>(wl_r + kPkRecOff + pt * 8 + 4 * pk_quad(pt, ci0 >> 2));
+            }
         }
         if constexpr (WGF && REC) {
             if (wgf && a.s_prev && a.wslab_rec && in) wsp = reinterpret_cast<const float4*>(a.s_prev)[pix * 2 + ci0 / 4];
@@ -1605,13 +1612,13 @@
     if constexpr (WL) {
         if (a.wt_bwd_ff) sw_x.store(wl_x);
         if constexpr (REC) {
-            if (a.g_state_prev) sw_r.store(wl_r);
+            if (has_gsp) sw_r.store(wl_r);
         }
     }
     if constexpr (FLDS) {
         if (a.wt_bwd_ff) fs_x.store(reinterpret_cast<__bf16*>(wl_x));
         if constexpr (REC) {
-            if (a.g_state_prev && !pkr) fs_r.store(reinterpret_cast<__bf16*>(wl_r));
+            if (has_gsp && !pkr) fs_r.store(reinterpret_cast<__bf16*>(wl_r));
         }
     }
     __syncthreads();
@@ -1623,7 +1630,7 @@
     if constexpr (kMfma<CIN, C>) {
         constexpr int NW = NTB / 64;
         const bool do_x = a.wt_bwd_ff != nullptr;
-        const bool do_r = REC && a.g_state_prev != nullptr;
+        const bool do_r = has_gsp;
         constexpr int NG = (C >= 32 && BF6) ? 2 : 1;
         MfmaAcc<C, CIN, NW, NG> ax;
         MfmaAcc<C, C, NW, NG> arr;
@@ -1670,7 +1677,8 @@
                 __syncthreads();
                 const float4 gv4 = *reinterpret_cast<const float4*>(wl_x + pt * 8 + 4 * pk_quad(pt, ci0 >> 2));
                 gx[0] = gv4.x; gx[1] = gv4.y; gx[2] = gv4.z; gx[3] = gv4.w;
-                if (in) {
+                if (WGF && chain == 1) {
+                } else if (in) {
                     const int64_t plane = (int64_t)a.B * H * W * C;
                     float* gsp = a.g_state_prev + pix * C + cr0;
                     if (a.zero_mem_half) *reinterpret_cast<float4*>(gsp) = z4;
@@ -1772,9 +1780,10 @@
         if constexpr (WGF) {
             if (wgf) {
                 if (REC && a.s_prev != nullptr && a.wslab_rec != nullptr) {
-                    fused_wgrad_stage_pk(G, wl_x, wl_r, xsp, wsp, pt, ci0);
+                    float* const res = chain == 1 ? wl_x : wl_r;
+                    fused_wgrad_stage_pk(G, wl_x, res, xsp, wsp, pt, ci0, chain == 1);
                     __syncthreads();
-                    fused_wgrad_store<REC>(a, g, wl_r, wl_r + kWgfR + kWgfP + kPkRecOff, wold);
+                    fused_wgrad_store<REC>(a, g, res, res + kWgfR + kWgfP + kPkRecOff, wold);
                 } else {
                     fused_wgrad_stage<REC>(a, G, wl_x, wl_r, xsp, wsp, pt, ci0);
                     __syncthreads();
@@ -2943,7 +2952,8 @@
     SK_PLAIN, SK_PLAIN_REC,
     SK_LIF, SK_LIF_REC,
     SK_TOP, SK_TOP_PRED,
-    SK_LIF_P, SK_LIF_REC_P
+    SK_LIF_P, SK_LIF_REC_P,
+    SK_CHAIN
 };
 
 struct FwdSlotParams {
@@ -2952,12 +2962,39 @@
     int kind[kSlotTasks], blk0[kSlotTasks], nblk[kSlotTasks];
     int ntask;
 };
+constexpr int kBwdTasks = SNNFLOW_MAX_CHAIN_TASKS, kBwdNodes = kBwdTasks + 1;
+struct ByteRange { int off, len; };
+constexpr int kNrnA0 = offsetof(snnflow_neuron, running_mean), kNrnA1 = offsetof(snnflow_neuron, beta);
+constexpr int kNrnB0 = offsetof(snnflow_neuron, momentum), kNrnB1 = offsetof(snnflow_neuron, bn_train);
+constexpr int kBwdOffN = offsetof(snnflow_layer_bwd_args, n), kBwdOffP = offsetof(snnflow_layer_bwd_args, prev);
+constexpr int kBwdKeepN = 5;
+constexpr ByteRange kBwdKeep[kBwdKeepN] = {
+    {0, kBwdOffN + kNrnA0},
+    {kBwdOffN + kNrnA1, kNrnB0 - kNrnA1},
+    {kBwdOffN + kNrnB1, kBwdOffP + kNrnA0 - (kBwdOffN + kNrnB1)},
+    {kBwdOffP + kNrnA1, kNrnB0 - kNrnA1},
+    {kBwdOffP + kNrnB1, (int)sizeof(snnflow_layer_bwd_args) - (kBwdOffP + kNrnB1)}};
+constexpr int bwd_keep_bytes(int n) { return n == 0 ? 0 : bwd_keep_bytes(n - 1) + kBwdKeep[n - 1].len; }
+constexpr bool bwd_keep_aligned(int n) {
+    return n == 0 || (kBwdKeep[n - 1].off % 8 == 0 && kBwdKeep[n - 1].len % 8 == 0 && kBwdKeep[n - 1].len > 0 && bwd_keep_aligned(n - 1));
+}
+constexpr int kBwdTaskBytes = bwd_keep_bytes(kBwdKeepN);
+static_assert(bwd_keep_aligned(kBwdKeepN), "8-byte pieces (pointers stay aligned)");
+struct BwdTask { int64_t w[kBwdTaskBytes / 8]; };
 struct BwdSlotParams {
-    snnflow_layer_bwd_args layer[kSlotTasks];
+    BwdTask layer[kBwdTasks];
     snnflow_lif_bwd_args lif;
-    int kind[kSlotTasks], blk0[kSlotTasks], nblk[kSlotTasks];
+    int kind[kBwdNodes], blk0[kBwdNodes], nblk[kBwdNodes], first[kBwdNodes];
     int ntask;
 };
+static_assert(sizeof(BwdSlotParams) + 256 <= 4096, "kernel arguments: 4 KB with the hidden ones");
+
+static void bwd_task_pack(const snnflow_layer_bwd_args& a, BwdTask& t) {
+    const int64_t* src = reinterpret_cast<const int64_t*>(&a);
+    int n = 0;
+    for (const ByteRange& r : kBwdKeep)
+        for (int i = 0; i < r.len / 8; ++i) t.w[n++] = src[r.off / 8 + i];
+}
 
 constexpr int cmax(int a, int b) { return a > b ? a : b; }
 
@@ -3061,12 +3098,27 @@
     return r;
 }
 
-template <typename P>
+__device__ inline snnflow_layer_bwd_args bwd_task_args(const __attribute__((address_space(4))) BwdTask* p) {
+    snnflow_layer_bwd_args r = {};
+    const __attribute__((address_space(4))) int* src = (const __attribute__((address_space(4))) int*)p;
+    int* dst = reinterpret_cast<int*>(&r);
+    int s = 0;
+#pragma unroll
+    for (int k = 0; k < kBwdKeepN; ++k) {
+#pragma unroll
+        for (int i = 0; i < kBwdKeep[k].len / 4; ++i) dst[kBwdKeep[k].off / 4 + i] = src[s + i];
+        s += kBwdKeep[k].len / 4;
+    }
+    globalize(r);
+    return r;
+}
+
+template <int NMAX = kSlotTasks, typename P>
 __device__ inline int slot_task(const __attribute__((address_space(4))) P* pp, Grid& g) {
     const int bid = blockIdx.x, nt = pp->ntask;
     int k = 0;
 #pragma unroll
-    for (int i = 1; i < kSlotTasks; ++i)
+    for (int i = 1; i < NMAX; ++i)
         if (i < nt && bid >= pp->blk0[i]) k = i;
     g.bid = bid - pp->blk0[k];
     g.nb = pp->nblk[k];
@@ -3656,14 +3708,28 @@
     typedef const __attribute__((address_space(4))) BwdSlotParams* cptr;
     const cptr pp = (cptr)__builtin_amdgcn_kernarg_segment_ptr();
     Grid g;
-    const int k = slot_task(pp, g);
+    const int k = slot_task<kBwdNodes>(pp, g);
     if (g.bid >= g.nb) return;
     __shared__ __attribute__((aligned(16))) float pool[SlotLds<C>::BWD];
-    switch (pp->kind[k]) {
+    int kind = pp->kind[k], ti = pp->first[k];
+    int chain = 0;
+    if (kind == SK_LIF_REC || kind == SK_CHAIN) {
+        const int ch1 = (C == 8 && kind == SK_CHAIN) ? 1 : 0;
+        {
+            const snnflow_layer_bwd_args a = bwd_task_args(&pp->layer[ti]);
+            layer_bwd_body<C, C, true, true, 2, SlotLds<C>::BFG, C == 8>(a, g, pool, ch1);
+        }
+        if (!ch1) return;
+        __syncthreads();
+        kind = SK_LIF;
+        ti += 1;
+        chain = 2;
+    }
+    switch (kind) {
 #define BWD_LAYER(ALL, KIND, ...)                             \
     case KIND: {                                              \
         if constexpr (ALL || kSlotAllKinds<C>) {              \
-            const snnflow_layer_bwd_args a = task_args(&pp->layer[k]);       \
+            const snnflow_layer_bwd_args a = bwd_task_args(&pp->layer[ti]);  \
             layer_bwd_body<__VA_ARGS__>(a, g, pool);          \
         }                                                     \
         break;                                                \
@@ -3672,9 +3738,12 @@
         BWD_LAYER(true, SK_HEAD4, 4, C, false, false, 2, false, false, true)
         BWD_LAYER(false, SK_PLAIN, C, C, false, false, 2)
         BWD_LAYER(false, SK_PLAIN_REC, C, C, false, true, 2)
-        BWD_LAYER(true, SK_LIF, C, C, true, false, 2, SlotLds<C>::BFG, C == 8)
-        BWD_LAYER(true, SK_LIF_REC, C, C, true, true, 2, SlotLds<C>::BFG, C == 8)
 #undef BWD_LAYER
+        case SK_LIF: {
+            const snnflow_layer_bwd_args a = bwd_task_args(&pp->layer[ti]);
+            layer_bwd_body<C, C, true, false, 2, SlotLds<C>::BFG, C == 8>(a, g, pool, chain);
+            break;
+        }
         case SK_TOP: {
             if constexpr (kSlotAllKinds<C>) {
                 const snnflow_lif_bwd_args a = task_args(&pp->lif);
@@ -4117,11 +4186,10 @@
     return 0;
 }
 
-int snnflow_bwd_slot(const snnflow_layer_bwd_args* layer, int nlayer, const snnflow_lif_bwd_args* lif,
-                     void* stream) {
-    const int nt = nlayer + (lif ? 1 : 0);
-    if (nlayer < 0 || nt <= 0 || nt > kSlotTasks || (nlayer && !layer)) SNN_FAIL(SNNFLOW_E_ARG, "bwd_slot: task count");
+static int bwd_launch(const snnflow_layer_bwd_args* layer, int nlayer, const unsigned char* pair,
+                      const snnflow_lif_bwd_args* lif, void* stream) {
     BwdSlotParams p = {};
+    int taskkind[kBwdTasks];
     const int c = nlayer ? layer[0].c : lif->c;
     const int B = nlayer ? layer[0].B : lif->B, H = nlayer ? layer[0].H : lif->H, W = nlayer ? layer[0].W : lif->W;
     if (!slot_c(c)) SNN_FAIL(SNNFLOW_E_CHANNELS, "bwd_slot: c must be 8, 16 or 32");
@@ -4150,9 +4218,17 @@
         const bool head_wg = (kind == SK_HEAD2 || kind == SK_HEAD4) && a.x != nullptr && !a.wslab_rec && !a.wt_bwd_rec;
         if ((a.wslab_ff || a.wslab_rec) && !(c == 8 && (kind == SK_LIF || kind == SK_LIF_REC)) && !head_wg)
             SNN_FAIL(SNNFLOW_E_ARG, "bwd_slot: wslab_ff / wslab_rec need a c = 8 LIF-fed task or a head task with x");
-        p.layer[i] = a;
-        p.kind[i] = kind;
-        p.nblk[i] = layer_bwd_blocks(a);
+        bwd_task_pack(a, p.layer[i]);
+        taskkind[i] = kind;
+    }
+    int nn = 0;
+    for (int i = 0; i < nlayer; ++i) {
+        const bool ch = pair && pair[i];
+        p.first[nn] = i;
+        p.kind[nn] = ch ? SK_CHAIN : taskkind[i];
+        p.nblk[nn] = layer_bwd_blocks(layer[i]);
+        ++nn;
+        if (ch) ++i;
     }
     if (lif) {
         if (const int e = lif_bwd_check(lif)) return e;
@@ -4161,22 +4237,60 @@
         if (lif->mem_grad_in) SNN_FAIL(SNNFLOW_E_ARG, "bwd_slot: mem_grad_in is a standalone-cell option");
         if (c != 8 && !lif->pred_w) SNN_FAIL(SNNFLOW_E_CHANNELS, "bwd_slot: c = 16 / 32 top task needs the prediction");
         p.lif = *lif;
-        p.kind[nlayer] = lif->pred_w ? SK_TOP_PRED : SK_TOP;
-        p.nblk[nlayer] = slot_top_blocks(c, B, H, W);
+        p.kind[nn] = lif->pred_w ? SK_TOP_PRED : SK_TOP;
+        p.nblk[nn] = slot_top_blocks(c, B, H, W);
     }
     if (c != 8) {
-        slot_sort(p.layer, p.kind, p.nblk, nlayer);
+        slot_sort(p.first, p.kind, p.nblk, nn);
+    } else if (pair) {
+        for (int i = 1; i < nn; ++i)
+            for (int j = i; j > 0 && p.kind[j] == SK_CHAIN && p.kind[j - 1] != SK_CHAIN; --j) {
+                const int tf = p.first[j]; p.first[j] = p.first[j - 1]; p.first[j - 1] = tf;
+                const int tk = p.kind[j]; p.kind[j] = p.kind[j - 1]; p.kind[j - 1] = tk;
+                const int tn = p.nblk[j]; p.nblk[j] = p.nblk[j - 1]; p.nblk[j - 1] = tn;
+            }
     } else if (SNNFLOW_SLOT_ORDER8) {
-        slot_sort(p.layer, p.kind, p.nblk, nlayer, SNNFLOW_SLOT_ORDER8 == 2);
-    }
-    p.ntask = nt;
-    const int nb = slot_ranges(p.nblk, nt, p.blk0);
+        slot_sort(p.first, p.kind, p.nblk, nn, SNNFLOW_SLOT_ORDER8 == 2);
+    }
+    p.ntask = nn + (lif ? 1 : 0);
+    const int nb = slot_ranges(p.nblk, p.ntask, p.blk0);
     const hipStream_t s = (hipStream_t)stream;
     if (c == 8) hipLaunchKernelGGL(k_bwd_slot<8>, dim3(nb), dim3(2 * NT), 0, s, p);
     else if (c == 16) hipLaunchKernelGGL(k_bwd_slot<16>, dim3(nb), dim3(2 * NT), 0, s, p);
     else hipLaunchKernelGGL(k_bwd_slot<32>, dim3(nb), dim3(2 * NT), 0, s, p);
     SNN_CHECK_LAUNCH();
     return 0;
+}
+
+int snnflow_bwd_slot(const snnflow_layer_bwd_args* layer, int nlayer, const snnflow_lif_bwd_args* lif,
+                     void* stream) {
+    const int nt = nlayer + (lif ? 1 : 0);
+    if (nlayer < 0 || nt <= 0 || nt > kSlotTasks || (nlayer && !layer)) SNN_FAIL(SNNFLOW_E_ARG, "bwd_slot: task count");
+    return bwd_launch(layer, nlayer, nullptr, lif, stream);
+}
+
+int snnflow_bwd_chain(const snnflow_layer_bwd_args* layer, int nlayer, const unsigned char* pair,
+                      const snnflow_lif_bwd_args* lif, void* stream) {
+    if (nlayer < 0 || nlayer > kBwdTasks || nlayer + (lif ? 1 : 0) <= 0 || (nlayer && !layer))
+        SNN_FAIL(SNNFLOW_E_ARG, "bwd_chain: task count");
+    for (int i = 0; pair && i < nlayer; ++i) {
+        if (!pair[i]) continue;
+        if (i + 1 >= nlayer || pair[i + 1]) SNN_FAIL(SNNFLOW_E_ARG, "bwd_chain: a pair is two consecutive tasks");
+        const snnflow_layer_bwd_args& r = layer[i];
+        const snnflow_layer_bwd_args& f = layer[i + 1];
+        if (r.c != 8 || r.cin != 8 || f.c != 8 || f.cin != 8 || !r.lif_in || !f.lif_in)
+            SNN_FAIL(SNNFLOW_E_CHANNELS, "bwd_chain: pairs are c = cin = 8 LIF-fed tasks");
+        if (r.B != f.B || r.H != f.H || r.W != f.W) SNN_FAIL(SNNFLOW_E_ARG, "bwd_chain: pair of different shapes");
+        if (!r.wt_bwd_rec || !r.wt_fwd_rec || f.wt_bwd_rec)
+            SNN_FAIL(SNNFLOW_E_ARG, "bwd_chain: a pair is (recurrent task, feed-forward task)");
+        if (!r.wslab_ff || !r.wslab_rec || !r.s_prev || !f.wslab_ff)
+            SNN_FAIL(SNNFLOW_E_ARG, "bwd_chain: both halves carry the fused weight gradients (wslab_*, s_prev)");
+        if (r.g_state_prev || f.prev_g_state || f.prev.bn_weight != r.n.bn_weight || f.prev.threshold != r.n.threshold)
+            SNN_FAIL(SNNFLOW_E_ARG, "bwd_chain: the first half's g_state_prev is handed to the second half's prev_g_state "
+                                    "(both NULL; second half's layer l-1 = first half's layer)");
+        ++i;
+    }
+    return bwd_launch(layer, nlayer, pair, lif, stream);
 }
 
 int snnflow_set_pipe(int fwd_tiles_per_block, int bwd_tiles_per_block) {
diff --git a/snn_event-based_optical_flow_amd/snnflow/_lib.py b/snn_event-based_optical_flow_amd/snnflow/_lib.py
--- a/snn_event-based_optical_flow_amd/snnflow/_lib.py
+++ b/snn_event-based_optical_flow_amd/snnflow/_lib.py
@@ -368,6 +368,8 @@
     "snnflow_count_nonzero": (I32, [P, P, I32, P, P]),
     "snnflow_fwd_slot": (I32, [ctypes.POINTER(ConvFwdArgs), I32, ctypes.POINTER(LifFwdArgs), P]),
     "snnflow_bwd_slot": (I32, [ctypes.POINTER(LayerBwdArgs), I32, ctypes.POINTER(LifBwdArgs), P]),
+    "snnflow_bwd_chain": (I32, [ctypes.POINTER(LayerBwdArgs), I32, ctypes.POINTER(ctypes.c_ubyte),
+                                ctypes.POINTER(LifBwdArgs), P]),
     "snnflow_slot_supported": (I32, [I32, I32]),
     "snnflow_set_pipe": (I32, [I32, I32]),
     "snnflow_get_pipe": (I32, [I32]),
@@ -399,6 +401,7 @@
     "snnflow_pointwise_bwd": (I32, [ctypes.POINTER(PointwiseArgs), P, I64, I64, P, P, P, P]),
 }
 MAX_SLOT_TASKS = 4
+MAX_CHAIN_TASKS = 7
 MAX_COUNT_TENSORS = 16
 
 
diff --git a/snn_event-based_optical_flow_amd/snnflow/engine.py b/snn_event-based_optical_flow_amd/snnflow/engine.py
--- a/snn_event-based_optical_flow_amd/snnflow/engine.py
+++ b/snn_event-based_optical_flow_amd/snnflow/engine.py
@@ -163,6 +163,8 @@
         self.fuse_wgrad = self.C == 8
         fh = os.environ.get("SNNFLOW_FUSE_HEAD")
         self.fuse_head = (self.C >= 16) if fh is None else fh != "0"
+        bc = os.environ.get("SNNFLOW_BWD_CHAIN")
+        self.bwd_chain = True if bc is None else bc != "0"
         self.spk_bits = os.environ.get("SNNFLOW_SPK_BITS", "1") != "0"
         self.defer_backward = os.environ.get("SNNFLOW_DEFER_BWD", "1") != "0"
         self.keep_seq_states = False
@@ -999,6 +1001,63 @@
     return slots
 
 
+def chainable_layers(rec):
+    L = len(rec)
+    return [r for r in range(1, L - 1) if rec[r] and not rec[r + 1]]
+
+
+def chained_bwd_slots(T, rec, chain=(), max_tasks=_lib.MAX_CHAIN_TASKS):
+    L = len(rec)
+    chain = set(chain)
+    if not all(1 <= r < L - 1 and rec[r] and not rec[r + 1] for r in chain):
+        raise ValueError("chained_bwd_slots: a chained layer is recurrent, LIF-fed and followed by a feed-forward layer")
+    node_of = {}
+    for k in range(L + 1):
+        for t in range(T):
+            if k in chain and t >= 1:
+                node = ((k, t), (k + 1, t - 1))
+            elif k - 1 in chain and t <= T - 2:
+                node = ((k - 1, t + 1), (k, t))
+            else:
+                node = ((k, t),)
+            node_of[(k, t)] = node
+
+    def deps(node):
+        out = set()
+        for k, t in node:
+            if k < L:
+                out.add((k + 1, t))
+            if t + 1 < T:
+                out.add((k, t + 1))
+                if k >= 1 and rec[k - 1]:
+                    out.add((k - 1, t + 1))
+        return {node_of[d] for d in out if d not in node}
+
+    level = {}
+
+    def lvl(node):
+        if node not in level:
+            level[node] = 1 + max((lvl(d) for d in deps(node)), default=-1)
+        return level[node]
+
+    nodes = sorted(set(node_of.values()), key=lambda n: (lvl(n), -n[0][0], -n[0][1]))
+    slot, fill, launches = {}, [], []
+    for n in nodes:
+        s = 1 + max((slot[d] for d in deps(n)), default=-1)
+        nl = sum(1 for k, _ in n if k < L)
+        while s < len(fill) and fill[s] + nl > max_tasks:
+            s += 1
+        while len(launches) <= s:
+            launches.append([])
+            fill.append(0)
+        slot[n] = s
+        fill[s] += nl
+        launches[s].append(n)
+    for la in launches:
+        la.sort(key=lambda n: -n[0][0])
+    return launches
+
+
 def _state_rows(st_all, fin, T):
     rows = [st_all[t] for t in range(st_all.shape[0])]
     return rows + [fin] if fin is not None else rows
@@ -1167,9 +1226,13 @@
 
         g_into = [None] * T
         g_into[T - 1] = [as_nhwc_state(g) if g is not None else None for g in g_final]
+        chained = bool(eng.bwd_chain) and C == 8 and bool(ctx.fuse) and L <= _lib.MAX_CHAIN_TASKS
+        chain = ([r for r in chainable_layers(eng.rec)
+                  if getattr(eng.cells[r], "detach", True) and getattr(eng.cells[r + 1], "detach", True)]
+                 if chained else [])
         g_out = [None] * T
         for t in range(T - 1, 0, -1):
-            g_out[t] = [empty_state(B, C, H, W, dev) if eng.rec[l] else None for l in range(L)]
+            g_out[t] = [empty_state(B, C, H, W, dev) if (eng.rec[l] and l not in chain) else None for l in range(L)]
             g_into[t - 1] = g_out[t]
         g0 = [None] * L
         for l in range(L):
@@ -1200,16 +1263,20 @@
                                 (gcur, bnc, ys, stats, ctx.bits), (bptr[t], bptr[t - 1] if t >= 1 else [None] * L)))
             eng.pending_layers.append(tuple(l for l in range(L) if not ((fuse and l > 0) or (fuse_head and l == 0))))
         try:
-            for tasks in wavefront_slots(T, L + 1):
-                layers, top = [], None
-                for j, tau in tasks:
-                    t = T - 1 - tau
+            if chained:
+                launches = [[(l, t, len(node) == 2 and i == 0) for node in la for i, (l, t) in enumerate(node)]
+                            for la in chained_bwd_slots(T, eng.rec, chain)]
+            else:
+                launches = [[(L - j, T - 1 - tau, False) for j, tau in tasks] for tasks in wavefront_slots(T, L + 1)]
+            for launch in launches:
+                layers, pairs, top = [], [], None
+                for l, t, first_half in launch:
                     acc = 0 if (fresh and t == T - 1) else 1
-                    if j == 0:
+                    if l == L:
                         top = _bwd_top_args(eng, B, H, W, ys[t], stats[t], mem_in[t], neurons, g_into[t], gfl[t],
                                             flows[t], gcur[t], gmem[t], bacc[t])
                     else:
-                        l = L - j
+                        pairs.append(1 if first_half else 0)
                         a = _bwd_layer_args(eng, l, B, H, W, cin0, ys[t], stats[t], mem_in[t], neurons,
                                             g_into[t], gcur[t], gmem[t], bacc[t], bnc[t], glayers, gpw, gpb,
                                             acc, wfwd, wbwd, g_out[t], ext[t], gxs[t] if l == 0 else None)
@@ -1230,8 +1297,13 @@
                             eng.slab_live[l] = True
                         layers.append(a)
                 arr = (_lib.LayerBwdArgs * max(len(layers), 1))(*layers)
-                _lib.call("bwd_slot", lib.snnflow_bwd_slot, arr, len(layers),
-                          ctypes.byref(top) if top is not None else None, s)
+                if chained:
+                    _lib.call("bwd_slot", lib.snnflow_bwd_chain, arr, len(layers),
+                              (ctypes.c_ubyte * max(len(pairs), 1))(*pairs),
+                              ctypes.byref(top) if top is not None else None, s)
+                else:
+                    _lib.call("bwd_slot", lib.snnflow_bwd_slot, arr, len(layers),
+                              ctypes.byref(top) if top is not None else None, s)
             _lib.timer_close()
             for l in range(L):
                 for t in range(T):
```

After: 68.96 million events/s, median of 6. +5.0%, better.
